# libraz/mygram-db

Hardware: AMD Instinct MI355X
Metric: queries/sec + p50 latency, 10M-doc bigram index, batch=1024 3-term AND (higher is better)
Workload: dtype u32 set algebra + f64 BM25

## Files before the change

mygram-db_amd/csrc/mgx_api.cpp:

```cpp
#include <hip/hip_runtime.h>

#include <dlfcn.h>
#include <pthread.h>

#include <algorithm>
#include <atomic>
#include <chrono>
#include <cmath>
#include <condition_variable>
#include <map>
#include <cstdio>
#include <cstdlib>
#include <cstring>
#include <memory>
#include <mutex>
#include <string>
#include <thread>
#include <tuple>
#include <unordered_map>
#include <vector>

#include "../../include/mygram_gpu.h"
#include "mgx_compile.hpp"
#include "mgx_highlight.hpp"
#include "mgx_host.hpp"
#include "mgx_internal.hpp"
#include "mgx_launch.hpp"
#include "mygram_tools.h"

namespace mgx {

static thread_local std::string g_last_error;
void SetError(const std::string& msg) { g_last_error = msg; }
int Fail(int code, const std::string& msg) {
  g_last_error = msg;
  return code;
}

#define MGX_HIP(expr)                                                                             \
  do {                                                                                            \
    hipError_t e__ = (expr);                                                                      \
    if (e__ != hipSuccess)                                                                        \
      return ::mgx::Fail(MGX_ERR_INTERNAL, std::string(#expr) + ": " + hipGetErrorString(e__));   \
  } while (0)
#define MGX_LAUNCH(expr)                                                                                    \
  do {                                                                                                      \
    int e__ = (expr);                                                                                       \
    if (e__ != 0)                                                                                           \
      return ::mgx::Fail(MGX_ERR_INTERNAL,                                                                  \
                         std::string(#expr) + ": " + hipGetErrorString(static_cast<hipError_t>(e__)));      \
  } while (0)

static std::atomic<int> g_fail_after{-1};
static std::atomic<int> g_fail_count{0};
static hipError_t DeviceMalloc(void** p, size_t n) {
  if (g_fail_after.load(std::memory_order_relaxed) >= 0) {
    if (g_fail_after.load() == 0) {
      if (g_fail_count.fetch_sub(1) > 0) {
        if (g_fail_count.load() <= 0) g_fail_after.store(-1);
        *p = nullptr;
        return hipErrorOutOfMemory;
      }
      g_fail_after.store(-1);
    } else {
      g_fail_after.fetch_sub(1);
    }
  }
  return hipMalloc(p, n);
}

struct Arena {
  struct Chunk {
    char* dev = nullptr;
    char* host = nullptr;
    size_t cap = 0, used = 0;
  };
  std::vector<Chunk> chunks;
  bool mirrored = false;
  size_t chunk_bytes = 4u << 20;
  explicit Arena(bool m) : mirrored(m) {}
  Arena(const Arena&) = delete;
  Arena& operator=(const Arena&) = delete;
  ~Arena() {
    for (Chunk& c : chunks) {
      if (c.dev) (void)hipFree(c.dev);
      if (c.host) (void)hipHostFree(c.host);
    }
  }
  void Reset() {
    for (Chunk& c : chunks) c.used = 0;
  }
  hipError_t Alloc(size_t n, void** dev, void** mirror) {
    n = (std::max<size_t>(n, 16) + 255) & ~static_cast<size_t>(255);
    for (Chunk& c : chunks) {
      if (c.cap - c.used >= n) {
        *dev = c.dev + c.used;
        if (mirror) *mirror = c.host ? c.host + c.used : nullptr;
        c.used += n;
        return hipSuccess;
      }
    }
    Chunk c;
    c.cap = std::max(n, chunk_bytes);
    hipError_t e = DeviceMalloc(reinterpret_cast<void**>(&c.dev), c.cap);
    if (e != hipSuccess) return e;
    if (mirrored) {
      e = hipHostMalloc(reinterpret_cast<void**>(&c.host), c.cap, hipHostMallocDefault);
      if (e != hipSuccess) {
        (void)hipFree(c.dev);
        return e;
      }
    }
    c.used = n;
    *dev = c.dev;
    if (mirror) *mirror = c.host;
    chunks.push_back(c);
    return hipSuccess;
  }
};

struct BatchResources {
  Arena upload{true}, out{false};
  bool uploaded = false;
  void* h_down[3] = {nullptr, nullptr, nullptr};
  size_t h_down_cap[3] = {0, 0, 0};
  hipEvent_t fork_ev = nullptr, join_ev = nullptr;
  hipStream_t stream = nullptr;
  hipEvent_t done_ev = nullptr;
  hipEvent_t main_ev = nullptr;
  bool copy_issued = false;
  void* xchg[4] = {nullptr, nullptr, nullptr, nullptr};
  size_t xchg_cap[4] = {0, 0, 0, 0};
  hipError_t Exchange(int which, size_t bytes, void** out_ptr) {
    if (xchg_cap[which] < bytes) {
      if (xchg[which]) (void)hipFree(xchg[which]);
      xchg[which] = nullptr;
      xchg_cap[which] = 0;
      const size_t cap = bytes + bytes / 4;
      hipError_t e = DeviceMalloc(&xchg[which], cap);
      if (e != hipSuccess) return e;
      xchg_cap[which] = cap;
    }
    *out_ptr = xchg[which];
    return hipSuccess;
  }
  void* cond = nullptr;
  size_t cond_cap = 0;
  hipError_t Conditions(size_t bytes, void** out_ptr) {
    if (cond_cap < bytes) {
      if (cond) (void)hipFree(cond);
      cond = nullptr;
      cond_cap = 0;
      hipError_t e = DeviceMalloc(&cond, bytes);
      if (e != hipSuccess) return e;
      cond_cap = bytes;
    }
    *out_ptr = cond;
    return hipSuccess;
  }
  ~BatchResources() {
    if (cond) (void)hipFree(cond);
    for (void* x : xchg)
      if (x) (void)hipFree(x);
    if (stream) (void)hipStreamDestroy(stream);
    if (done_ev) (void)hipEventDestroy(done_ev);
    if (main_ev) (void)hipEventDestroy(main_ev);
    for (void* h : h_down)
      if (h) (void)hipHostFree(h);
    if (fork_ev) (void)hipEventDestroy(fork_ev);
    if (join_ev) (void)hipEventDestroy(join_ev);
  }
  hipError_t Pinned(int which, size_t bytes, void** out_ptr) {
    if (h_down_cap[which] < bytes) {
      if (h_down[which]) (void)hipHostFree(h_down[which]);
      h_down[which] = nullptr;
      h_down_cap[which] = 0;
      const size_t cap = std::max<size_t>(bytes + bytes / 2, 1u << 16);
      hipError_t e = hipHostMalloc(&h_down[which], cap, hipHostMallocDefault);
      if (e != hipSuccess) return e;
      h_down_cap[which] = cap;
    }
    *out_ptr = h_down[which];
    return hipSuccess;
  }
  void Reset() {
    upload.Reset();
    out.Reset();
    uploaded = false;
    copy_issued = false;
  }
};
static thread_local BatchResources* tl_res = nullptr;
struct ResourceScope {
  BatchResources* prev;
  explicit ResourceScope(BatchResources* r) : prev(tl_res) { tl_res = r; }
  ~ResourceScope() { tl_res = prev; }
};

struct DevBuf {
  void* p = nullptr;
  size_t bytes = 0;
  bool owned = true;
  DevBuf() = default;
  DevBuf(const DevBuf&) = delete;
  DevBuf& operator=(const DevBuf&) = delete;
  DevBuf(DevBuf&& o) noexcept : p(o.p), bytes(o.bytes), owned(o.owned) { o.p = nullptr; o.bytes = 0; }
  DevBuf& operator=(DevBuf&& o) noexcept {
    if (this != &o) {
      Free();
      p = o.p;
      bytes = o.bytes;
      owned = o.owned;
      o.p = nullptr;
      o.bytes = 0;
    }
    return *this;
  }
  ~DevBuf() { Free(); }
  void Free() {
    if (p && owned) (void)hipFree(p);
    p = nullptr;
    bytes = 0;
    owned = true;
  }
  hipError_t Alloc(size_t n) {
    Free();
    bytes = n;
    if (tl_res) {
      owned = false;
      return tl_res->out.Alloc(n, &p, nullptr);
    }
    return DeviceMalloc(&p, n ? n : 16);
  }
  template <typename T>
  T* as() const { return static_cast<T*>(p); }
};

template <typename T>
static hipError_t Upload(DevBuf& b, const T* host, size_t count, size_t pad_count = 0) {
  if (tl_res) {
    b.Free();
    b.bytes = (count + pad_count) * sizeof(T);
    b.owned = false;
    void* mirror = nullptr;
    hipError_t e = tl_res->upload.Alloc(b.bytes, &b.p, &mirror);
    if (e != hipSuccess) return e;
    if (count) std::memcpy(mirror, host, count * sizeof(T));
    if (pad_count) std::memset(static_cast<char*>(mirror) + count * sizeof(T), 0xFF, pad_count * sizeof(T));
    return hipSuccess;
  }
  hipError_t e = b.Alloc((count + pad_count) * sizeof(T));
  if (e != hipSuccess) return e;
  if (pad_count) {
    e = hipMemset(static_cast<char*>(b.p) + count * sizeof(T), 0xFF, pad_count * sizeof(T));
    if (e != hipSuccess) return e;
  }
  if (count) e = hipMemcpy(b.p, host, count * sizeof(T), hipMemcpyHostToDevice);
  return e;
}

}

using mgx::DevBuf;


struct mgx_index {
  int device = 0;
  hipStream_t stream = nullptr;
  hipStream_t side_stream = nullptr;
  std::mutex mu;
  std::mutex pool_mu;
  std::vector<std::unique_ptr<mgx::BatchResources>> single_pool;
  mgx::DevIndex dev{};
  DevBuf d_offsets, d_docids, d_tf, d_doc_len, d_skip_row, d_tile_off, d_gram_bitmaps, d_filter_bitmaps;
  DevBuf d_text, d_text_off;
  uint32_t max_text_bytes = 0;
  DevBuf d_dl8, d_tfnib, d_tf_ovf_pos, d_tf_ovf_val;
  DevBuf d_dev_index;
  std::vector<uint64_t> h_offsets;
  std::vector<uint32_t> h_skip_row;
  std::vector<uint32_t> h_bm_row;
  uint32_t n_filter_rows = 0, filter_cap_rows = 0;
  struct FilterColumn {
    uint32_t value_class = 0, n_values = 0;
    DevBuf d_values, d_null, d_value_ids;
  };
  std::vector<std::unique_ptr<FilterColumn>> filter_columns;
  std::atomic<uint32_t> n_filter_columns{0};
  std::vector<DevBuf> retired_filter_pools;
  uint64_t n_grams = 0;
  bool can_score = false;
  uint64_t words_per_row = 0;
  uint64_t filter_row_stride = 0;
  struct TableKey {
    uint32_t row;
    uint64_t idf, k1, b, avg;
    bool operator==(const TableKey& o) const { return row == o.row && idf == o.idf && k1 == o.k1 && b == o.b && avg == o.avg; }
  };
  struct TableKeyHash {
    size_t operator()(const TableKey& k) const {
      uint64_t h = k.row * 0x9E3779B97F4A7C15ull;
      for (uint64_t v : {k.idf, k.k1, k.b, k.avg}) h = (h ^ v) * 0xFF51AFD7ED558CCDull + (h >> 29);
      return static_cast<size_t>(h);
    }
  };
  std::mutex table_mu;
  std::unordered_map<TableKey, uint32_t, TableKeyHash> table_slot;
  DevBuf d_table_pool;
  uint32_t table_cap = 0, table_used = 0, table_dl = 0;
  hipStream_t table_stream = nullptr;
  hipEvent_t table_ev = nullptr;
  mgx::TableJob* job_ring = nullptr;
  DevBuf d_job_ring;
  uint32_t job_ring_at = 0;
  std::vector<mgx::TableJob> pending_jobs;
  hipEvent_t chain_ev = nullptr;
  std::atomic<int> fifo{1};
  bool table_ev_recorded = false;
  static constexpr uint32_t kJobRing = 4096;
  size_t table_doubles() const { return static_cast<size_t>(mgx::kFastPoolTf + 1) * table_dl; }
  struct NormTable {
    uint64_t k1, b, avg;
    DevBuf d;
  };
  std::vector<std::unique_ptr<NormTable>> norm_tables;
  struct BlockMax {
    uint64_t k1, b, avg;
    double step;
    DevBuf d, d_fine;
  };
  std::vector<std::unique_ptr<BlockMax>> block_max;
  std::unordered_map<std::string, uint64_t> df_cache;
  uint32_t n_bitmap_rows = 0, n_fine_rows = 0;
  std::atomic<uint32_t> live_row{mgx::kNoRow};
  std::atomic<bool> bitmaps_clean{false};
  DevBuf d_doc_map;
  DevBuf d_fine_rows;
// ... 821 lines not shown
  }
}

int mgx_index_invalidate_statistics(mgx_index* idx) {
  if (!idx) return mgx::Fail(MGX_ERR_INVALID_ARGUMENT, "mgx_index_invalidate_statistics: null index");
  MGX_HIP(hipSetDevice(idx->device));
  MGX_HIP(hipDeviceSynchronize());
  std::lock_guard<std::mutex> lock(idx->table_mu);
  idx->table_slot.clear();
  idx->table_used = 0;
  idx->pending_jobs.clear();
  idx->norm_tables.clear();
  idx->block_max.clear();
  idx->df_cache.clear();
  return MGX_OK;
}

int mgx_index_synchronize(mgx_index* idx) {
  if (!idx) return mgx::Fail(MGX_ERR_INVALID_ARGUMENT, "mgx_index_synchronize: null index");
  MGX_HIP(hipSetDevice(idx->device));
  MGX_HIP(hipDeviceSynchronize());
  return MGX_OK;
}

}


struct mgx_batch {
  mgx_index* idx = nullptr;
  std::unique_ptr<mgx::BatchResources> res_owned;
  mgx::BatchResources* res = nullptr;
  uint32_t n_queries = 0;
  std::vector<mgx::QuerySpec> specs;
  struct RouteLaunch {
    mgx::DevBatch dev{};
    DevBuf d_items;
  };
  struct Group {
    std::vector<uint32_t> qids;
    mgx::DevBatch dev{};
    mgx::LdsPlan plan{};
    mgx::WavePlan wplan{};
    RouteLaunch block;
    uint32_t n_items_plain = 0;
    uint32_t n_items_fz = 0;
    RouteLaunch wave;
    DevBuf d_tables;
    mgx::WavePlan wplan_lists{};
    RouteLaunch wave_lists;
    mgx::FastPlan fplan{};
    RouteLaunch fast[mgx::kFastMaxScore];
    uint32_t n_seed_fast[mgx::kFastMaxScore] = {0, 0, 0, 0, 0};
    uint32_t seed_k = 0;
    uint64_t seed_table_docs = 0;
    DevBuf d_has_seed;
    DevBuf d_fast_queries;
    RouteLaunch cand;
    DevBuf d_cand_skip;
    uint32_t cand_leaves = 0, cand_instr = 0, cand_cap = 0;
    RouteLaunch merge;
    uint32_t merge_leaves = 0, merge_instr = 0, merge_ops = 0, merge_cap = 0;
    RouteLaunch page_wave, page_block;
    uint32_t n_page_fz = 0;
    DevBuf d_queries, d_leaves, d_prog, d_score, d_explicit, d_counters, d_ident, d_list_begin;
    std::vector<unsigned long long> h_counters;
  };
  Group score, bitmap;
  Group textdf;
  std::vector<mgx::QuerySpec> df_specs;
  DevBuf d_patterns, d_text_terms, d_text_idf, d_text_df, d_verify_terms, d_verify_prog;
  DevBuf d_text_df_local, d_text_df_known;
  std::vector<uint64_t> h_text_df, h_text_df_local, text_total_docs;
  std::vector<uint64_t> text_df_known;
  std::vector<std::string> text_df_key;
  std::vector<double> h_text_idf;
  DevBuf d_cond_groups, d_conds;
  uint32_t n_cond_groups = 0;
  uint64_t* cond_arena = nullptr;
  bool df_ready = false;
  DevBuf d_cand_keys, d_cand_docs, d_cand_n;
  DevBuf d_export;
  size_t ex_off32 = 0, ex_bytes = 0;
  uint64_t* ex_keys() const { return d_export.as<uint64_t>(); }
  uint64_t* ex_totals(size_t n) const { return d_export.as<uint64_t>() + n * top_stride; }
  uint32_t* ex_docs() const { return reinterpret_cast<uint32_t*>(static_cast<char*>(d_export.p) + ex_off32); }
  uint32_t* ex_counts(size_t n) const { return ex_docs() + n * top_stride; }
  DevBuf d_score_out;
  void* h_score_out = nullptr;
  size_t so_override = 0, so_scores = 0, so_docs = 0, so_n = 0, so_bytes = 0;
  unsigned long long* sc_counters() const { return d_score_out.as<unsigned long long>(); }
  uint64_t* sc_override() const { return reinterpret_cast<uint64_t*>(static_cast<char*>(d_score_out.p) + so_override); }
  double* sc_scores() const { return reinterpret_cast<double*>(static_cast<char*>(d_score_out.p) + so_scores); }
  uint32_t* sc_docs() const { return reinterpret_cast<uint32_t*>(static_cast<char*>(d_score_out.p) + so_docs); }
  uint32_t* sc_n() const { return reinterpret_cast<uint32_t*>(static_cast<char*>(d_score_out.p) + so_n); }
  uint32_t top_stride = 0, page_stride = 0;
  bool merged_shards = false;
  DevBuf d_rbits, d_tile_cnt, d_tile_start, d_totals, d_take, d_out_off, d_reverse;
  mgx_batch* merge_other = nullptr;
  bool merged_away = false;
  hipStream_t merge_stream = nullptr;
  DevBuf d_merge;
  Group page;
  DevBuf d_ptile_cnt, d_ptile_start, d_page_out, d_page_scratch;
  void* h_page_out = nullptr;
  size_t po_totals = 0, po_docs = 0, po_bytes = 0;
  uint32_t doc_page_stride = 0;
  struct Highlight {
    std::vector<mgx::DevHlQuery> queries;
    std::vector<int32_t> of_query;
    DevBuf d_queries, d_terms, d_patterns, d_arena;
    void* h_arena = nullptr;
    size_t bytes = 0;
    uint32_t n_entries = 0;
    bool defer = false;
    std::vector<mgx_highlight_entry> entries;
    bool on() const { return !queries.empty(); }
  };
  Highlight hl;
  bool fetched = false;
  std::vector<mgx_query_result> h_results;
  std::vector<uint32_t> h_docs;
  std::vector<double> h_scores;
  bool executed = false;
  hipStream_t last_stream = nullptr;
  bool timing = false;
  std::vector<std::pair<hipEvent_t, hipEvent_t>> events;
  uint64_t list_bytes = 0;
};

namespace mgx {

constexpr int kSections = 7;
static std::atomic<uint64_t> g_section_us[kSections];
static const char* const kSectionNames[kSections] = {"queries+leaves", "routes", "table uploads", "result blocks",
                                                      "items", "launch order", "descriptors+items"};
struct SectionTimer {
  static bool On() {
    static const bool on = std::getenv("MGX_TRACE_HOST") != nullptr;
    return on;
  }
  std::chrono::steady_clock::time_point t;
  SectionTimer() { if (On()) t = std::chrono::steady_clock::now(); }
  void Mark(int section) {
    if (!On()) return;
    const auto now = std::chrono::steady_clock::now();
    g_section_us[section] += std::chrono::duration_cast<std::chrono::nanoseconds>(now - t).count();
    t = now;
  }
};

using Group = mgx_batch::Group;
using RouteLaunch = mgx_batch::RouteLaunch;

enum class Route : uint8_t {
  kBlock,
  kWave,
  kWaveLists,
  kFast,
  kCand,
  kMerge,
};

static bool EnvZero(const char* name) { return std::getenv(name) && atoi(std::getenv(name)) == 0; }
struct PathSwitches {
  const bool wave = std::getenv("MGX_FORCE_BLOCK_KERNEL") == nullptr;
  const bool fast = wave && !EnvZero("MGX_FAST_PATH"), cand = wave && !EnvZero("MGX_CAND");
  const bool merge = wave && !EnvZero("MGX_MERGE");
};

struct GroupPlan {
  GroupPlan(uint32_t n_, uint32_t mode)
      : n(n_), score_mode(mode == kModeScore), df_mode(mode == kModeTextDf), page_mode(mode == kModeDocPage) {}
  const uint32_t n;
  const bool score_mode, df_mode, page_mode;
  std::vector<DevQuery> dq;
  std::vector<DevLeaf> leaves;
  std::vector<uint32_t> prog;
  std::vector<DevScoreTerm> score;
  std::vector<uint32_t> expl;
  uint32_t max_limit = 1, max_needed = 1;
  std::vector<Route> route;
  std::vector<DevFastQuery> fastq;
  std::vector<uint64_t> wave_tables;
  std::vector<uint32_t> cand_driver;
  std::vector<DevItem> items;
  std::vector<uint32_t> list_begin, item_begin;
  std::vector<DevItem> block, wave, wave_lists, fast[kFastMaxScore], cand, merge;
  std::vector<uint8_t> has_seed;
};

static int LayOutQueries(mgx_batch* b, Group& g, const std::vector<QuerySpec>& specs, GroupPlan& p) {
  std::vector<DevLeaf>& leaves = p.leaves;
  std::vector<uint32_t>& expl = p.expl;
  p.dq.resize(p.n);
  uint32_t max_leaves = 0, max_lds_leaves = 0, max_score = 0, max_stack = 0, max_instr = 0, max_cap = 64;
  for (uint32_t i = 0; i < p.n; ++i) {
    const QuerySpec& s = specs[g.qids[i]];
    DevQuery& q = p.dq[i];
    std::memset(&q, 0, sizeof(q));
    q.leaf_begin = static_cast<uint32_t>(leaves.size());
    q.n_leaves = static_cast<uint32_t>(s.leaves.size());
    q.prog_begin = static_cast<uint32_t>(p.prog.size());
    q.n_instr = static_cast<uint32_t>(s.prog.size());
    q.score_begin = static_cast<uint32_t>(p.score.size());
    q.n_score = static_cast<uint32_t>(s.score.size());
    q.mode = s.mode;
    q.limit = s.limit;
    q.offset = s.offset;
    q.needed = static_cast<uint32_t>(std::min<uint64_t>(static_cast<uint64_t>(s.offset) + s.limit, 0xFFFFFFFFull));
    uint32_t cap = 64;
    if (s.mode == kModeScore)
      while (cap < q.needed && cap < (1u << 30)) cap <<= 1;
    q.cap = cap;
    q.descending = s.reverse;
    q.stack_depth = s.stack_depth;
    q.out_slot = i;
    q.pat_off = s.pat_off;
    q.pat_len = s.pat_len;
    q.vt_begin = s.vt_begin;
    q.vt_count = static_cast<uint32_t>(s.verify_patterns.size());
    q.fz_distance = s.fz_distance;
    q.vp_begin = s.vp_begin;
    q.k1 = s.k1;
    q.b = s.b;
    q.one_minus_b = 1.0 - s.b;
    q.k1_plus_1 = s.k1 + 1.0;
    q.avgdl_clamped = std::max(s.avgdl, 1.0);
    const uint32_t ebase = static_cast<uint32_t>(expl.size());
    uint32_t n_lds = 0;
    for (size_t li = 0; li < s.leaves.size(); ++li) {
      DevLeaf lf = s.leaves[li];
      if (lf.kind == kLeafExplicit) lf.a += ebase;
      bool resident = lf.kind == kLeafList || lf.kind == kLeafExplicit;
      for (const DevScoreTerm& st : s.score) resident = resident || st.leaf == li;
      lf.lds = resident ? n_lds++ : kNoRow;
      leaves.push_back(lf);
    }
    if (n_lds > kMaxLdsLeaves)
      return Fail(MGX_ERR_NOT_IMPLEMENTED,
                  "query " + std::to_string(g.qids[i]) + ": more than 64 sorted-list / scored operands in one query");
    max_lds_leaves = std::max(max_lds_leaves, n_lds);
    p.prog.insert(p.prog.end(), s.prog.begin(), s.prog.end());
    p.score.insert(p.score.end(), s.score.begin(), s.score.end());
    expl.insert(expl.end(), s.explicit_ids.begin(), s.explicit_ids.end());
    while (expl.size() % 4) expl.push_back(0xFFFFFFFFu);
    max_leaves = std::max(max_leaves, q.n_leaves);
    max_score = std::max(max_score, q.n_score);
    max_stack = std::max(max_stack, q.stack_depth);
    max_instr = std::max(max_instr, q.n_instr);
    max_cap = std::max(max_cap, q.cap);
    p.max_limit = std::max(p.max_limit, q.limit);
    p.max_needed = std::max(p.max_needed, q.needed);
    if (!p.df_mode) b->list_bytes += 4 * s.list_postings;
  }
  g.plan = PlanLds(max_leaves, max_lds_leaves, max_score, max_stack, max_instr, max_cap, p.score_mode || p.df_mode);
  return MGX_OK;
}

static bool ResolveFast(mgx_index* idx, const uint64_t* cond_arena, const QuerySpec& s, const DevQuery& q, DevFastQuery* out) {
  DevFastQuery& f = *out;
  for (uint32_t ins : s.prog) {
    const uint32_t op = ins >> 24, arg = ins & 0xFFFFFFu;
    if (op == kOpCount) {
      if (f.n_ops == 0) return false;
      f.ops[f.n_ops - 1].code |= arg << 8;
      continue;
    }
    const DevLeaf& lf = s.leaves[arg];
    if (f.n_ops == static_cast<uint32_t>(kFastMaxOps) || (op == kOpLoad) != (f.n_ops == 0)) return false;
    FastOp o{};
    uint64_t stride = 0;
    if (lf.kind == kLeafGramBitmap) {
      o.base = reinterpret_cast<uint64_t>(idx->dev.gram_bitmaps + static_cast<uint64_t>(lf.b) * idx->dev.gb_row_stride);
      stride = idx->dev.gb_tile_stride * 8;
    } else if (lf.kind == kLeafFilterBitmap) {
      o.base = static_cast<uint64_t>(lf.b) * idx->dev.fb_row_stride * 8;
      stride = idx->dev.fb_tile_stride * 8;
      o.code |= 16u;
    } else if (lf.kind == kLeafCondBitmap) {
      o.base = reinterpret_cast<uint64_t>(cond_arena + static_cast<uint64_t>(lf.b) * idx->dev.fb_row_stride);
      stride = idx->dev.fb_tile_stride * 8;
    } else {
      return false;
    }
    if (stride > 0xFFFFFFFFull) return false;
    o.tile_stride = static_cast<uint32_t>(stride);
    o.code |= (op == kOpLoad || op == kOpOr) ? kFastOr : op == kOpAnd ? kFastAnd : kFastAndNot;
    f.ops[f.n_ops++] = o;
  }
  if (f.n_ops == 0) return false;
  for (size_t t = 0; t < s.score.size(); ++t) {
    const DevLeaf& lf = s.leaves[s.score[t].leaf];
    if (lf.kind != kLeafGramBitmap) return false;
    FastScore& fs = f.score[t];
    fs.nib = reinterpret_cast<uint64_t>(idx->dev.tfnib + static_cast<uint64_t>(lf.b) * idx->dev.nib_row_stride);
    fs.idf = s.score[t].idf;
    fs.gram = lf.a;
    fs.skip_row = lf.row;
  }
  if (s.reverse != 0) {
    double step = 0.0;
    f.blockmax = GetBlockMax(idx, s.k1, s.b, s.avgdl, &step, &f.blockmax_fine);
    if (f.blockmax) {
      f.bm_tile_stride = idx->n_bitmap_rows * 256u;
      f.bmf_tile_stride = idx->n_fine_rows * 1024u;
      double idf_max = 0.0;
      for (size_t t = 0; t < s.score.size(); ++t) idf_max = std::max(idf_max, s.score[t].idf);
      const double wunit = idf_max > 0.0 ? idf_max * (1.0 + 0x1p-40) / 255.0 : 1.0;
      f.bm_inv_unit = 1.0 / (wunit * step);
      f.bm_wpack = f.bm_w4 = f.bm_cint = 0;
      for (size_t t = 0; t < s.score.size(); ++t) {
        const uint32_t w = static_cast<uint32_t>(std::min(255.0, std::ceil(s.score[t].idf / wunit)));
        if (t < 4) f.bm_wpack |= w << (8 * t); else f.bm_w4 = w;
      }
      for (size_t t = 0; t < s.score.size(); ++t) {
        const DevLeaf& lf = s.leaves[s.score[t].leaf];
        FastScore& fs = f.score[t];
        const uint32_t frow = f.blockmax_fine ? idx->h_fine_map[lf.b] : kNoRow;
        fs.bm_mode = frow != kNoRow ? 2u : 1u;
        fs.bm_off = frow != kNoRow ? frow * 1024u : lf.b * 256u;
      }
    }
  }
  f.n_score = static_cast<uint32_t>(s.score.size());
  f.needed = q.needed;
  f.cap = q.cap;
  f.descending = q.descending;
  f.k1 = q.k1;
  f.b = q.b;
  f.one_minus_b = q.one_minus_b;
  f.k1_plus_1 = q.k1_plus_1;
  f.avgdl_clamped = q.avgdl_clamped;
  return true;
}

static void RouteCandMerge(mgx_batch* b, Group& g, const std::vector<QuerySpec>& specs, const PathSwitches& sw,
                           GroupPlan& p) {
  static const uint64_t kMaxPerTile = std::getenv("MGX_CAND_MAX_PER_TILE") ? static_cast<uint64_t>(atoll(std::getenv("MGX_CAND_MAX_PER_TILE"))) : 64ull;
  const mgx_index* idx = b->idx;
  for (uint32_t i = 0; sw.cand && i < p.n; ++i) {
    const QuerySpec& s = specs[g.qids[i]];
    if (p.route[i] == Route::kFast || !s.flat || s.prog.empty()) continue;
    if (p.score_mode && (!s.fast_score_ok || s.score.empty())) continue;
    bool ok = true, counted = false;
    uint32_t driver = kNoLeaf;
    uint64_t best = ~0ull, longest_list = 0;
    for (size_t pc = 0; ok && pc < s.prog.size(); ++pc) {
      const uint32_t op = s.prog[pc] >> 24, arg = s.prog[pc] & 0xFFFFFFu;
      if (op == kOpCount) {
        counted = true;
        continue;
      }
      if ((op == kOpLoad) != (pc == 0) || (op != kOpLoad && op != kOpAnd && op != kOpAndNot)) { ok = false; break; }
      const DevLeaf& lf = s.leaves[arg];
      if (lf.kind != kLeafList && lf.kind != kLeafGramBitmap && !IsFilterKind(lf.kind)) { ok = false; break; }
      if (lf.kind == kLeafList) longest_list = std::max<uint64_t>(longest_list, idx->h_offsets[lf.a + 1] - idx->h_offsets[lf.a]);
      if (op == kOpAndNot || IsFilterKind(lf.kind) || counted) continue;
      const uint64_t sz = idx->h_offsets[lf.a + 1] - idx->h_offsets[lf.a];
      if (sz < best) {
        best = sz;
        driver = arg;
      }
    }
    if (!ok || driver == kNoLeaf || s.leaves[driver].kind != kLeafList) continue;
    for (uint32_t ins : s.prog)
      if ((ins >> 24) == kOpAndNot && (ins & 0xFFFFFFu) == driver) ok = false;
    if (p.score_mode)
      for (const DevScoreTerm& st : s.score)
        ok = ok && st.leaf != kNoLeaf && (s.leaves[st.leaf].kind == kLeafList || s.leaves[st.leaf].kind == kLeafGramBitmap);
    if (!ok) continue;
    DevQuery& q = p.dq[i];
    const bool long_probe = longest_list > 8 * kMaxPerTile * idx->dev.n_tiles;
    if (best > kMaxPerTile * idx->dev.n_tiles || long_probe) {
      uint32_t staged = 0;
      for (size_t li = 0; li < s.leaves.size(); ++li) staged += li != driver ? 1u : 0u;
      if (!p.score_mode || !sw.merge || staged > kMergeMaxOps || q.cap > 256) continue;
      q.pat_off = driver;
      p.route[i] = Route::kMerge;
      g.merge_leaves = std::max(g.merge_leaves, q.n_leaves);
      g.merge_instr = std::max(g.merge_instr, q.n_instr);
      g.merge_ops = std::max(g.merge_ops, staged);
      g.merge_cap = std::max(g.merge_cap, q.cap);
      continue;
    }
    if (p.cand_driver.empty()) p.cand_driver.assign(p.n, kNoLeaf);
    p.cand_driver[i] = driver;
    p.route[i] = Route::kCand;
    g.cand_leaves = std::max(g.cand_leaves, q.n_leaves);
    g.cand_instr = std::max(g.cand_instr, q.n_instr);
    g.cand_cap = std::max(g.cand_cap, q.cap);
  }
  if (CandLdsBytes(g.cand_leaves, g.cand_instr, p.score_mode ? g.cand_cap : 0) > 150 * 1024) {
    for (Route& r : p.route)
      if (r == Route::kCand) r = Route::kBlock;
    p.cand_driver.clear();
  }
  if (MergeLdsBytes(g.merge_leaves, g.merge_instr, g.merge_ops, g.merge_cap) > 150 * 1024)
    for (Route& r : p.route)
      if (r == Route::kMerge) r = Route::kBlock;
}

static int ChooseRoutes(mgx_batch* b, Group& g, const std::vector<QuerySpec>& specs, const PathSwitches& sw,
                        GroupPlan& p) {
  mgx_index* idx = b->idx;
  p.route.assign(p.n, Route::kBlock);
  if (p.score_mode) {
    uint32_t fcap = 64;
    bool have_params = false;
    double pk1 = 0, pb = 0, pavg = 0;
    for (uint32_t i = 0; sw.fast && i < p.n; ++i) {
      const QuerySpec& s = specs[g.qids[i]];
      if (!s.flat || !s.fast_score_ok || s.score.empty() || s.score.size() > static_cast<size_t>(kFastMaxScore)) continue;
      if (p.dq[i].cap > 128) continue;
      if (have_params && (Bits(s.k1) != Bits(pk1) || Bits(s.b) != Bits(pb) || Bits(s.avgdl) != Bits(pavg))) continue;
      DevFastQuery f{};
      if (!ResolveFast(idx, b->cond_arena, s, p.dq[i], &f)) continue;
      if (!have_params) {
        pk1 = s.k1;
        pb = s.b;
        pavg = s.avgdl;
        have_params = true;
      }
      if (p.fastq.empty()) p.fastq.resize(p.n);
      p.fastq[i] = f;
      p.route[i] = Route::kFast;
      fcap = std::max(fcap, f.cap);
    }
    if (have_params) {
      const double* ktab = GetLengthNormTable(idx, pk1, pb, pavg);
      g.fplan = PlanFast(fcap, ktab);
      if (ktab == nullptr || g.fplan.bytes > 64 * 1024)
        for (Route& r : p.route) r = Route::kBlock;
    }

    uint32_t wl = 0, wsc = 0, wi = 0, wc = 64;
    for (uint32_t i = 0; i < p.n; ++i) {
      if (p.route[i] == Route::kFast) continue;
      const QuerySpec& s = specs[g.qids[i]];
      bool ok = sw.wave && s.wave_ok;
      for (const DevScoreTerm& st : s.score)
        ok = ok && (s.leaves[st.leaf].kind == kLeafGramBitmap || s.leaves[st.leaf].kind == kLeafList);
      if (!ok) continue;
      uint64_t tabs[kWaveScoreSlots] = {0, 0, 0};
      for (size_t t = 0; ok && t < s.score.size(); ++t) {
        const DevLeaf& lf = s.leaves[s.score[t].leaf];
        const uint32_t key = lf.kind == kLeafGramBitmap ? lf.b : 0x80000000u | lf.a;
        tabs[t] = GetContributionTable(idx, key, s.score[t].idf, s.k1, s.b, s.avgdl);
        ok = tabs[t] != 0;
      }
      if (!ok) continue;
      if (p.wave_tables.empty()) p.wave_tables.assign(static_cast<size_t>(p.n) * kWaveScoreSlots, 0);
      for (int t = 0; t < kWaveScoreSlots; ++t) p.wave_tables[static_cast<size_t>(i) * kWaveScoreSlots + t] = tabs[t];
      bool lists = false;
      for (const DevLeaf& lf : s.leaves) lists = lists || lf.kind == kLeafList || lf.kind == kLeafExplicit;
      p.route[i] = lists ? Route::kWaveLists : Route::kWave;
      wl = std::max<uint32_t>(wl, p.dq[i].n_leaves);
      wsc = std::max<uint32_t>(wsc, p.dq[i].n_score);
      wi = std::max<uint32_t>(wi, p.dq[i].n_instr);
      wc = std::max<uint32_t>(wc, p.dq[i].cap);
    }
    g.wplan = PlanWave(wl, wsc, wi, wc, idx->dev.max_doc_len, false);
    g.wplan_lists = PlanWave(wl, wsc, wi, wc, idx->dev.max_doc_len, true);
    if (g.wplan_lists.bytes > 160 * 1024)
      for (Route& r : p.route)
        if (r != Route::kFast) r = Route::kBlock;
  }
  if (p.page_mode || p.df_mode) {
    uint32_t wl = 1, wi = 1;
    bool has_list = false;
    for (uint32_t i = 0; i < p.n; ++i) {
      const QuerySpec& s = specs[g.qids[i]];
      if (!(sw.wave && s.wave_ok)) continue;
      p.route[i] = Route::kWave;
      for (const DevLeaf& lf : s.leaves) has_list = has_list || lf.kind == kLeafList || lf.kind == kLeafExplicit;
      wl = std::max<uint32_t>(wl, p.dq[i].n_leaves);
      wi = std::max<uint32_t>(wi, p.dq[i].n_instr);
    }
    g.wplan = WavePlan{wl, 0, wi, 0, 0, has_list ? 1u : 0u, 0};
  }
  g.cand_leaves = g.cand_instr = g.cand_cap = 0;
  g.merge_leaves = g.merge_instr = g.merge_ops = g.merge_cap = 0;
  if (p.score_mode || p.page_mode) RouteCandMerge(b, g, specs, sw, p);
  if (g.plan.bytes > 160 * 1024)
    return Fail(MGX_ERR_NOT_IMPLEMENTED, "query shape exceeds the 160 KiB LDS of a CU");
  for (uint32_t i = 0; i < p.n; ++i)
    if (specs[g.qids[i]].fz_op && g.plan.bytes + kFzLdsBytes > 160 * 1024)
      return Fail(MGX_ERR_NOT_IMPLEMENTED, "query shape with the fuzzy text filter exceeds the 160 KiB LDS of a CU");
  return MGX_OK;
}

static int UploadTables(mgx_batch* b, Group& g, const GroupPlan& p, SectionTimer& sec) {
  const uint32_t n = p.n;
  MGX_HIP(Upload(g.d_queries, p.dq.data(), p.dq.size()));
  MGX_HIP(Upload(g.d_leaves, p.leaves.data(), p.leaves.size()));
  MGX_HIP(Upload(g.d_prog, p.prog.data(), p.prog.size()));
  MGX_HIP(Upload(g.d_score, p.score.data(), p.score.size()));
  MGX_HIP(Upload(g.d_explicit, p.expl.data(), p.expl.size(), 4));
  sec.Mark(2);
  if (p.score_mode) {
    const size_t max_limit = p.max_limit;
    b->so_override = static_cast<size_t>(n) * 9 * 8;
    b->so_scores = b->so_override + static_cast<size_t>(n) * 8;
    b->so_docs = b->so_scores + static_cast<size_t>(n) * max_limit * 8;
    b->so_n = b->so_docs + static_cast<size_t>(n) * max_limit * 4;
    b->so_bytes = b->so_n + static_cast<size_t>(n) * 4;
    MGX_HIP(b->d_score_out.Alloc(b->so_bytes));
    MGX_HIP(b->res->Pinned(0, b->so_bytes, &b->h_score_out));
  } else if (p.page_mode) {
    const size_t max_limit = p.max_limit;
    b->doc_page_stride = p.max_limit;
    b->po_totals = static_cast<size_t>(n) * 8 * 8;
    b->po_docs = b->po_totals + static_cast<size_t>(n) * 8;
    b->po_bytes = b->po_docs + static_cast<size_t>(n) * max_limit * 4;
    MGX_HIP(b->d_page_out.Alloc(b->po_bytes));
    MGX_HIP(b->res->Pinned(1, b->po_bytes, &b->h_page_out));
    const size_t tiles = b->idx->dev.n_tiles;
    MGX_HIP(b->d_ptile_cnt.Alloc(static_cast<size_t>(n) * tiles * 4));
    MGX_HIP(b->d_ptile_start.Alloc(static_cast<size_t>(n) * tiles * 8));
  } else {
    MGX_HIP(g.d_counters.Alloc(static_cast<size_t>(n) * 9 * sizeof(unsigned long long)));
  }
  g.h_counters.assign(static_cast<size_t>(n) * 8, 0);
  std::vector<uint32_t> ident(n);
  for (uint32_t i = 0; i < n; ++i) ident[i] = i;
  MGX_HIP(Upload(g.d_ident, ident.data(), n));
  return MGX_OK;
}

static void CutItems(const mgx_batch* b, const Group& g, const std::vector<QuerySpec>& specs, GroupPlan& p) {
  static const double kMatchesPerUnit = std::getenv("MGX_ITEM_MATCHES") ? atof(std::getenv("MGX_ITEM_MATCHES")) : 256.0;
  static const double kItemCost = std::getenv("MGX_ITEM_COST") ? atof(std::getenv("MGX_ITEM_COST")) : 192.0;
  static const uint32_t kMaxTiles = std::getenv("MGX_MAX_ITEM_TILES") ? static_cast<uint32_t>(atoi(std::getenv("MGX_MAX_ITEM_TILES"))) : static_cast<uint32_t>(kMaxTilesPerItem);
  static const uint64_t want_items = std::getenv("MGX_WANT_ITEMS") ? static_cast<uint64_t>(atoll(std::getenv("MGX_WANT_ITEMS"))) : 4ull * 768ull;
  static const uint32_t kSeedTiles = std::getenv("MGX_SEED_TILES") ? static_cast<uint32_t>(atoi(std::getenv("MGX_SEED_TILES"))) : 16u;
  const uint32_t n = p.n, n_tiles = b->idx->dev.n_tiles;
  p.list_begin.assign(n + 1, 0);
  p.item_begin.assign(n + 1, 0);
  uint32_t n_lists = 0;
  for (uint32_t i = 0; i < n; ++i) {
    const QuerySpec& s = specs[g.qids[i]];
    const Route route = p.route[i];
    p.item_begin[i] = static_cast<uint32_t>(p.items.size());
    const bool fast = route == Route::kFast;
    const double per_tile = 1.0 + (p.score_mode || p.df_mode ? s.est_density * kTileDocs / (fast ? kMatchesPerUnit / 2 : kMatchesPerUnit) : 0.0);
    const double fast_scale = std::min(4.0, std::max(2.0, static_cast<double>(n_tiles) / 150.0));
    uint32_t tiles = static_cast<uint32_t>((fast ? fast_scale * kItemCost : kItemCost) / per_tile);
    tiles = std::max<uint32_t>(8, std::min<uint32_t>(tiles, fast ? 2 * kMaxTiles : kMaxTiles)) & ~7u;
    if (p.score_mode) {
      const uint64_t cap = std::max<uint64_t>(8, (static_cast<uint64_t>(n_tiles) * n / want_items + 7) & ~7ull);
      tiles = static_cast<uint32_t>(std::min<uint64_t>(tiles, cap));
    }
    if (p.score_mode && route == Route::kBlock) tiles = 8;
    p.list_begin[i] = n_lists;
    if (route == Route::kCand) {
      p.items.push_back(DevItem{i, p.cand_driver[i], 0, n_lists++});
      continue;
    }
    uint32_t t0 = 0;
    const uint32_t seed_tiles = std::min<uint32_t>(kSeedTiles, (n_tiles / 8) & ~7u);
    if (fast && seed_tiles && n_tiles > 4 * seed_tiles) {
      p.items.push_back(DevItem{i, 0, seed_tiles, n_lists++});
      t0 = seed_tiles;
    }
    for (uint32_t t = t0; t < n_tiles; t += tiles) {
      DevItem it{i, t, std::min(tiles, n_tiles - t), n_lists++};
      p.items.push_back(it);
    }
  }
  p.list_begin[n] = n_lists;
  p.item_begin[n] = static_cast<uint32_t>(p.items.size());
}

static int ScheduleItems(const mgx_batch* b, Group& g, const std::vector<QuerySpec>& specs, GroupPlan& p) {
  static const uint32_t kSortTiles = std::getenv("MGX_SORT_TILES") ? static_cast<uint32_t>(atoi(std::getenv("MGX_SORT_TILES"))) : 16u;
  static const bool kXcdAffinity = std::getenv("MGX_XCD_AFFINITY") ? atoi(std::getenv("MGX_XCD_AFFINITY")) != 0 : true;
  static const double kHeavyDensity = std::getenv("MGX_HEAVY_DENSITY") ? atof(std::getenv("MGX_HEAVY_DENSITY")) : 0.05;
  static const double kSqueezeEnv = std::getenv("MGX_HEAVY_SQUEEZE") ? atof(std::getenv("MGX_HEAVY_SQUEEZE")) : -1.0;
  const uint32_t n = p.n, n_tiles = b->idx->dev.n_tiles;
  const bool deal = kXcdAffinity && p.score_mode;
  std::vector<uint32_t> order(n);
  for (uint32_t i = 0; i < n; ++i) order[i] = i;
  if (deal) {
    std::vector<uint32_t> heavy(n, 0);
    for (uint32_t i = 0; i < n; ++i) {
      uint64_t best = 0;
      for (const DevLeaf& lf : specs[g.qids[i]].leaves) {
        if (lf.kind != kLeafGramBitmap && lf.kind != kLeafList) continue;
        const uint64_t sz = b->idx->h_offsets[lf.a + 1] - b->idx->h_offsets[lf.a];
        if (sz > best) {
          best = sz;
          heavy[i] = lf.a;
        }
      }
    }
    std::stable_sort(order.begin(), order.end(), [&](uint32_t x, uint32_t y) { return heavy[x] < heavy[y]; });
  }
  const uint32_t n_bands = n_tiles / kSortTiles + 1;
  const double kHeavySqueeze = kSqueezeEnv >= 0.0 ? kSqueezeEnv : 0.6 + 0.4 * std::min(1.0, n_tiles / 600.0);
  auto band_of = [&](const DevItem& it) {
    const Route route = p.route[it.query];
    if (route == Route::kCand) return 0u;
    const uint32_t band = it.tile_begin / kSortTiles;
    if (p.score_mode && route == Route::kFast && specs[g.qids[it.query]].est_density >= kHeavyDensity)
      return static_cast<uint32_t>(band * kHeavySqueeze);
    return band;
  };
  std::vector<uint32_t> band_at(n_bands + 1, 0);
  for (const DevItem& it : p.items) band_at[band_of(it) + 1]++;
  for (uint32_t k = 0; k < n_bands; ++k) band_at[k + 1] += band_at[k];
  std::vector<DevItem> sorted(p.items.size());
  {
    std::vector<uint32_t> cur(band_at.begin(), band_at.end() - 1);
    for (uint32_t oi = 0; oi < n; ++oi) {
      const uint32_t i = order[oi];
      for (uint32_t k = p.item_begin[i]; k < p.item_begin[i + 1]; ++k) sorted[cur[band_of(p.items[k])]++] = p.items[k];
    }
  }
  if (deal) {
    for (uint32_t k = 0; k < n_bands; ++k) {
      const size_t lo = band_at[k], m = band_at[k + 1] - lo, per = (m + 7) / 8;
      size_t w = lo;
      for (size_t r = 0; r < per; ++r)
        for (size_t x = 0; x < 8; ++x)
          if (x * per + r < m) p.items[w++] = sorted[lo + x * per + r];
    }
  } else {
    p.items.swap(sorted);
  }
  p.has_seed.assign(n, 0);
  for (int pass = 0; pass < 2; ++pass) {
    for (const DevItem& it : p.items) {
      const Route route = p.route[it.query];
      const bool seed = route == Route::kFast && it.list == p.list_begin[it.query] && it.tile_begin == 0 &&
                        p.list_begin[it.query + 1] - p.list_begin[it.query] > 1 && it.n_tiles <= 16;
      if (seed != (pass == 0)) continue;
      switch (route) {
        case Route::kBlock: p.block.push_back(it); break;
        case Route::kWave: p.wave.push_back(it); break;
        case Route::kWaveLists: p.wave_lists.push_back(it); break;
        case Route::kFast: p.fast[p.fastq[it.query].n_score - 1].push_back(it); break;
        case Route::kCand: p.cand.push_back(it); break;
        case Route::kMerge: p.merge.push_back(it); break;
      }
      if (seed && p.fastq[it.query].blockmax != 0) p.has_seed[it.query] = 1;
    }
    if (pass == 0)
      for (int t = 0; t < kFastMaxScore; ++t) g.n_seed_fast[t] = static_cast<uint32_t>(p.fast[t].size());
  }
  g.seed_k = 0;
  g.seed_table_docs = 0;
  for (uint32_t i = 0; p.score_mode && i < n; ++i) {
    const QuerySpec& sp = specs[g.qids[i]];
    if (sp.reverse != 0 && p.dq[i].needed != 0 && p.dq[i].needed <= 128u) {
      g.seed_k = std::max(g.seed_k, p.dq[i].needed);
      g.seed_table_docs = std::max<uint64_t>(g.seed_table_docs, sp.total_docs);
    }
  }
  if (g.seed_k) MGX_HIP(Upload(g.d_has_seed, p.has_seed.data(), p.has_seed.size()));
  return MGX_OK;
}

static hipError_t MakeRoute(RouteLaunch& r, const DevBatch& base, const std::vector<DevItem>& items) {
  r.dev = base;
  r.dev.n_items = static_cast<uint32_t>(items.size());
  const hipError_t e = Upload(r.d_items, items.data(), items.size());
  r.dev.items = r.d_items.as<DevItem>();
  return e;
}

static int UploadItems(mgx_batch* b, Group& g, const std::vector<QuerySpec>& specs, GroupPlan& p) {
  const uint32_t n = p.n;
  std::vector<uint8_t> listlike(n, 0);
  for (uint32_t i = 0; i < n; ++i) {
    for (const DevLeaf& lf : specs[g.qids[i]].leaves)
      if (lf.kind == kLeafList || lf.kind == kLeafExplicit || lf.kind == kLeafRange) listlike[i] = 1;
    if (specs[g.qids[i]].fz_op) listlike[i] = 2;
  }
  std::stable_partition(p.block.begin(), p.block.end(), [&](const DevItem& it) { return listlike[it.query] == 0; });
  if (std::find(listlike.begin(), listlike.end(), 2) != listlike.end())
    std::stable_partition(p.block.begin(), p.block.end(), [&](const DevItem& it) { return listlike[it.query] != 2; });
  g.n_items_plain = g.n_items_fz = 0;
  for (const DevItem& it : p.block) {
    g.n_items_plain += listlike[it.query] == 0 ? 1u : 0u;
    g.n_items_fz += listlike[it.query] == 2 ? 1u : 0u;
  }
  DevBatch& d = g.dev;
  d.queries = g.d_queries.as<DevQuery>();
  d.leaves = g.d_leaves.as<DevLeaf>();
  d.prog = g.d_prog.as<uint32_t>();
  d.score_terms = g.d_score.as<DevScoreTerm>();
  d.explicit_pool = g.d_explicit.as<uint32_t>();
  d.patterns = b->d_patterns.as<uint8_t>();
  d.text_terms = b->d_text_terms.as<DevTextTerm>();
  d.text_idf = b->d_text_idf.as<double>();
  d.verify_terms = b->d_verify_terms.as<DevTextTerm>();
  d.verify_prog = b->d_verify_prog.as<uint32_t>();
  d.n_queries = n;
  d.counters = p.score_mode  ? b->sc_counters()
               : p.page_mode ? b->d_page_out.as<unsigned long long>()
                             : g.d_counters.as<unsigned long long>();
  if (p.page_mode) {
    d.tile_cnt = b->d_ptile_cnt.as<uint32_t>();
    d.tile_start = b->d_ptile_start.as<uint64_t>();
    d.totals = reinterpret_cast<const uint64_t*>(static_cast<const char*>(b->d_page_out.p) + b->po_totals);
    d.page_docs = reinterpret_cast<uint32_t*>(static_cast<char*>(b->d_page_out.p) + b->po_docs);
    d.page_stride = b->doc_page_stride;
  }
  d.bounds = p.score_mode ? d.counters + static_cast<size_t>(n) * 8 : nullptr;
#ifdef MGX_ABLATION
  d.debug_skip = std::getenv("MGX_DEBUG_SKIP") ? static_cast<uint32_t>(atoi(std::getenv("MGX_DEBUG_SKIP"))) : 0u;
#endif
  if (p.score_mode) {
    const size_t n_lists = p.list_begin[n], max_needed = p.max_needed;
    d.cand_stride = b->top_stride = p.max_needed;
    b->page_stride = p.max_limit;
    MGX_HIP(b->d_cand_keys.Alloc(n_lists * max_needed * 8));
    MGX_HIP(b->d_cand_docs.Alloc(n_lists * max_needed * 4));
    MGX_HIP(b->d_cand_n.Alloc(n_lists * 4));
    {
      const size_t elems = static_cast<size_t>(n) * max_needed + n;
      b->ex_off32 = elems * 8;
      b->ex_bytes = (elems * 12 + 7) / 8 * 8;
      MGX_HIP(b->d_export.Alloc(b->ex_bytes));
    }
    d.cand_keys = b->d_cand_keys.as<uint64_t>();
    d.cand_docs = b->d_cand_docs.as<uint32_t>();
    d.cand_n = b->d_cand_n.as<uint32_t>();
  } else if (!p.df_mode && !p.page_mode) {
    const size_t tiles = b->idx->dev.n_tiles;
    MGX_HIP(b->d_rbits.Alloc(static_cast<size_t>(n) * tiles * kWordsPerTile * 8));
    MGX_HIP(b->d_tile_cnt.Alloc(static_cast<size_t>(n) * tiles * 4));
    MGX_HIP(b->d_tile_start.Alloc(static_cast<size_t>(n) * tiles * 8));
    MGX_HIP(b->d_totals.Alloc(static_cast<size_t>(n) * 8));
    MGX_HIP(b->d_take.Alloc(static_cast<size_t>(n) * 8));
    MGX_HIP(b->d_out_off.Alloc(static_cast<size_t>(n) * 8));
    std::vector<uint32_t> rev(n);
    for (uint32_t i = 0; i < n; ++i) rev[i] = specs[g.qids[i]].deep_score ? 0u : specs[g.qids[i]].reverse;
    MGX_HIP(Upload(b->d_reverse, rev.data(), n));
    d.rbits = b->d_rbits.as<uint64_t>();
    d.tile_cnt = b->d_tile_cnt.as<uint32_t>();
  }
  if (p.score_mode && !p.wave_tables.empty()) {
    MGX_HIP(Upload(g.d_tables, p.wave_tables.data(), p.wave_tables.size()));
    d.wave_tables = g.d_tables.as<uint64_t>();
  }
  if (!p.fastq.empty()) MGX_HIP(Upload(g.d_fast_queries, p.fastq.data(), p.fastq.size()));
  d.fast_queries = g.d_fast_queries.as<DevFastQuery>();
  d.dev_index = b->idx->d_dev_index.as<DevIndex>();
  d.cond_bitmaps = b->cond_arena;
  for (int t = 0; t < kFastMaxScore; ++t) MGX_HIP(MakeRoute(g.fast[t], d, p.fast[t]));
  MGX_HIP(MakeRoute(g.wave_lists, d, p.wave_lists));
  MGX_HIP(MakeRoute(g.cand, d, p.cand));
  MGX_HIP(MakeRoute(g.merge, d, p.merge));
  if (p.page_mode && !p.cand.empty()) {
    std::vector<uint8_t> skip(n, 0);
    for (uint32_t i = 0; i < n; ++i) skip[i] = p.route[i] == Route::kCand ? 1 : 0;
    MGX_HIP(Upload(g.d_cand_skip, skip.data(), skip.size()));
  }
  MGX_HIP(MakeRoute(g.block, d, p.block));
  MGX_HIP(MakeRoute(g.wave, d, p.wave));
  MGX_HIP(Upload(g.d_list_begin, p.list_begin.data(), p.list_begin.size()));
  if (p.page_mode) {
    std::vector<DevItem> pw, pb;
    for (uint32_t i = 0; i < n; ++i)
      if (p.route[i] != Route::kCand && !specs[g.qids[i]].fz_op)
        (p.route[i] == Route::kWave ? pw : pb).push_back(DevItem{i, 0, 0, 0});
    g.n_page_fz = 0;
    for (uint32_t i = 0; i < n; ++i)
      if (specs[g.qids[i]].fz_op) {
        pb.push_back(DevItem{i, 0, 0, 0});
        ++g.n_page_fz;
      }
    MGX_HIP(MakeRoute(g.page_wave, d, pw));
    MGX_HIP(MakeRoute(g.page_block, d, pb));
  }
  return MGX_OK;
}

static int UploadGroup(mgx_batch* b, Group& g, uint32_t mode, const std::vector<QuerySpec>& specs) {
  GroupPlan p(static_cast<uint32_t>(g.qids.size()), mode);
  if (p.n == 0) return MGX_OK;
  const PathSwitches sw;
  SectionTimer sec;
  if (const int rc = LayOutQueries(b, g, specs, p)) return rc;
  sec.Mark(0);
  if (const int rc = ChooseRoutes(b, g, specs, sw, p)) return rc;
  sec.Mark(1);
  if (const int rc = UploadTables(b, g, p, sec)) return rc;
  sec.Mark(3);
  CutItems(b, g, specs, p);
  sec.Mark(4);
  if (const int rc = ScheduleItems(b, g, specs, p)) return rc;
  sec.Mark(5);
  if (const int rc = UploadItems(b, g, specs, p)) return rc;
  sec.Mark(6);
  if (std::getenv("MGX_VERBOSE")) {
    size_t fast_queries = 0;
    for (Route r : p.route) fast_queries += r == Route::kFast ? 1 : 0;
    fprintf(stderr,
            "[mgx] %s group: %u queries; fast path %zu items (%zu queries, lds %u B, ring %u), wave kernel %zu items "
            "(lds %u B, lists %zu), block kernel %zu items (lds %u B), candidate-driven %zu queries, list merge %zu "
            "items\n",
            p.score_mode ? "score" : p.page_mode ? "docid-page" : p.df_mode ? "df" : "bitmap", p.n,
            p.fast[0].size() + p.fast[1].size() + p.fast[2].size() + p.fast[3].size() + p.fast[4].size(), fast_queries,
            g.fplan.bytes, g.fplan.ring, p.wave.size() + p.wave_lists.size(), g.wplan.bytes, p.wave_lists.size(),
            p.block.size(), g.plan.bytes, p.cand.size(), p.merge.size());
  }
  return MGX_OK;
}

static CompileView ViewOf(const mgx_index* idx) {
  CompileView v;
  v.offsets = idx->h_offsets.data();
  v.skip_row = idx->h_skip_row.data();
  v.bm_row = idx->h_bm_row.data();
  v.n_grams = idx->n_grams;
  v.n_docs = idx->dev.n_docs;
  v.first_doc_id = idx->dev.first_doc_id;
  v.has_text = idx->dev.text != nullptr;
  v.can_score = idx->can_score;
  v.n_filter_rows = idx->n_filter_rows;
  v.n_filter_columns = idx->n_filter_columns.load(std::memory_order_acquire);
  v.live_row = idx->live_row.load(std::memory_order_relaxed);
  v.bitmaps_clean = idx->bitmaps_clean.load(std::memory_order_relaxed);
  return v;
}

static int CompileRange(const CompileView& view, const mgx_query* queries, std::vector<QuerySpec>* specs, uint32_t a, uint32_t b) {
  for (uint32_t i = a; i < b; ++i) {
    (*specs)[i].Clear();
    if (const int rc = CompileQuery(view, queries[i], &(*specs)[i])) return Fail(rc, "query " + std::to_string(i) + ": " + g_last_error);
  }
  return MGX_OK;
}

struct CompilePool {
  std::mutex mu, gate;
  std::condition_variable cv_work, cv_done;
  std::vector<std::thread> helpers;
  const CompileView* view = nullptr;
  const mgx_query* queries = nullptr;
  std::vector<QuerySpec>* specs = nullptr;
  uint32_t next = 0, end = 0, pending = 0;
  int rc = MGX_OK;
  std::string error;
  bool stop = false;
  static constexpr uint32_t kChunk = 64;

  void Run(std::unique_lock<std::mutex>& lock) {
    while (next < end) {
      const uint32_t a = next, b = std::min(end, a + kChunk);
      next = b;
      lock.unlock();
      const int local = CompileRange(*view, queries, specs, a, b);
      lock.lock();
      if (local && rc == MGX_OK) {
        rc = local;
        error = g_last_error;
      }
      pending -= b - a;
    }
  }
  void Helper() {
    std::unique_lock<std::mutex> lock(mu);
    for (;;) {
      cv_work.wait(lock, [&] { return stop || next < end; });
      if (stop) return;
      Run(lock);
      if (pending == 0) cv_done.notify_all();
    }
  }
  CompilePool() {
    const int n = std::getenv("MGX_COMPILE_THREADS") ? atoi(std::getenv("MGX_COMPILE_THREADS")) : 3;
    for (int i = 0; i < n; ++i)
      helpers.emplace_back([this] {
        pthread_setname_np(pthread_self(), "mgx-compile");
        Helper();
      });
  }
  ~CompilePool() {
    {
      std::lock_guard<std::mutex> lock(mu);
      stop = true;
    }
    cv_work.notify_all();
    for (auto& t : helpers) t.join();
  }
};

static int CompileAll(const mgx_index* idx, const mgx_query* queries, uint32_t n, std::vector<QuerySpec>* specs) {
  static thread_local CompilePool pool;
  const CompileView view = ViewOf(idx);
  std::unique_lock<std::mutex> gate(pool.gate, std::try_to_lock);
  if (n < 4 * CompilePool::kChunk || pool.helpers.empty() || !gate.owns_lock()) return CompileRange(view, queries, specs, 0, n);
  std::unique_lock<std::mutex> lock(pool.mu);
  pool.view = &view;
  pool.queries = queries;
  pool.specs = specs;
  pool.next = 0;
  pool.end = pool.pending = n;
  pool.rc = MGX_OK;
  pool.cv_work.notify_all();
  pool.Run(lock);
  pool.cv_done.wait(lock, [&] { return pool.pending == 0; });
  pool.end = 0;
  if (pool.rc) SetError(pool.error);
  return pool.rc;
}

static int LayOutConditions(mgx_batch* b) {
  mgx_index* idx = b->idx;
  size_t n_refs = 0;
  for (const QuerySpec& s : b->specs) n_refs += s.conds.size();
  if (n_refs == 0) return MGX_OK;
  using Key = std::tuple<uint32_t, uint32_t, uint64_t, uint64_t, uint32_t, uint32_t>;
  std::map<Key, uint32_t> rows;
  for (QuerySpec& s : b->specs)
    for (DevLeaf& lf : s.leaves) {
      if (lf.kind != kLeafCondBitmap) continue;
      const mgx_condition& c = s.conds[lf.a];
      const Key key{c.column_id, c.op, c.literal_bits, Bits(c.eq_epsilon), c.null_matches ? 1u : 0u, c.never_matches ? 1u : 0u};
      lf.b = rows.emplace(key, static_cast<uint32_t>(rows.size())).first->second;
      lf.a = 0;
    }
  const uint64_t row_bytes = idx->dev.fb_row_stride * sizeof(uint64_t);
  if (idx->dev.fb_row_stride % kCondBlockWords != 0)
    return Fail(MGX_ERR_INTERNAL, "filter row stride is not a multiple of the condition pass's block");
  if (rows.size() * row_bytes > MGX_CONDITION_ARENA_MAX_BYTES)
    return Fail(MGX_ERR_OUT_OF_RANGE, "the batch holds " + std::to_string(rows.size()) + " distinct conditions of " +
                                          std::to_string(row_bytes) + " bytes each: more than the " +
                                          std::to_string(MGX_CONDITION_ARENA_MAX_BYTES) +
                                          " bytes (MGX_CONDITION_ARENA_MAX_BYTES) a batch's condition arena may take");
  void* arena = nullptr;
  MGX_HIP(b->res->Conditions(rows.size() * row_bytes, &arena));
  b->cond_arena = static_cast<uint64_t*>(arena);
  std::vector<DevCondition> conds;
  std::vector<DevCondGroup> groups;
  conds.reserve(rows.size());
  {
    std::lock_guard<std::mutex> lock(idx->mu);
    uint32_t last_column = 0;
    for (const auto& kv : rows) {
      const uint32_t column = std::get<0>(kv.first);
      if (groups.empty() || column != last_column) {
        last_column = column;
        const mgx_index::FilterColumn& col = *idx->filter_columns[column];
        DevCondGroup g{};
        g.values = col.d_values.as<uint64_t>();
        g.is_null = col.d_null.as<uint8_t>();
        g.value_class = col.value_class;
        g.cond_begin = g.cond_end = static_cast<uint32_t>(conds.size());
        groups.push_back(g);
      }
      DevCondition d{};
      d.literal = std::get<2>(kv.first);
      __builtin_memcpy(&d.eq_epsilon, &std::get<3>(kv.first), 8);
      d.op = std::get<1>(kv.first);
      d.null_matches = std::get<4>(kv.first);
      d.never_matches = std::get<5>(kv.first);
      d.row = kv.second;
      conds.push_back(d);
      groups.back().cond_end = static_cast<uint32_t>(conds.size());
    }
  }
  if (groups.size() > 65535) return Fail(MGX_ERR_OUT_OF_RANGE, "conditions on more than 65535 columns in one batch");
  MGX_HIP(Upload(b->d_conds, conds.data(), conds.size()));
  MGX_HIP(Upload(b->d_cond_groups, groups.data(), groups.size()));
  b->n_cond_groups = static_cast<uint32_t>(groups.size());
  return MGX_OK;
}

static int NumberTextTerms(mgx_batch* b, std::string* pool, std::vector<DevTextTerm>* tts) {
  mgx_index* idx = b->idx;
  const CompileView view = ViewOf(idx);
  std::map<std::pair<std::string, uint64_t>, uint32_t> seen;
  for (QuerySpec& s : b->specs) {
    for (const QuerySpec::TextTerm& tt : s.text_terms) {
      const auto ins = seen.emplace(std::make_pair(tt.pattern, s.total_docs), static_cast<uint32_t>(tts->size()));
      const uint32_t id = ins.first->second;
      if (s.deep_score) s.deep_grams[tt.score_index] = kDeepText | id;
      else s.score[tt.score_index].text_term = id;
      if (!ins.second) continue;
      const DevTextTerm d{static_cast<uint32_t>(pool->size()), static_cast<uint32_t>(tt.pattern.size())};
      *pool += tt.pattern;
      tts->push_back(d);
      b->text_total_docs.push_back(s.total_docs);
      std::string ckey = tt.pattern + '\0' + std::to_string(s.total_docs);
      uint64_t known = ~0ull;
      {
        std::lock_guard<std::mutex> lock(idx->table_mu);
        const auto hit = idx->df_cache.find(ckey);
        if (hit != idx->df_cache.end()) known = hit->second;
      }
      b->text_df_known.push_back(tt.grams.empty() ? 0ull : known);
      b->text_df_key.push_back(std::move(ckey));
      QuerySpec ds;
      if (const int rc = CompileTextDf(view, tt.grams, tt.grams.empty() || known != ~0ull, d.pat_off, d.pat_len, &ds)) return rc;
      b->df_specs.push_back(std::move(ds));
    }
  }
  return MGX_OK;
}

static void PoolVerifyPatterns(mgx_batch* b, std::string* pool, std::vector<DevTextTerm>* vts, std::vector<uint32_t>* vprog) {
  for (QuerySpec& s : b->specs) {
    s.vt_begin = static_cast<uint32_t>(vts->size());
    s.vp_begin = static_cast<uint32_t>(vprog->size());
    vprog->insert(vprog->end(), s.verify_prog.begin(), s.verify_prog.end());
    for (const std::string& pat : s.verify_patterns) {
      vts->push_back(DevTextTerm{static_cast<uint32_t>(pool->size()), static_cast<uint32_t>(pat.size())});
      *pool += pat;
    }
  }
}

static int PrepareInto(mgx_batch* b, mgx_index* idx, std::vector<QuerySpec>&& specs) {
  ResourceScope scope(b->res);
  b->idx = idx;
  b->n_queries = static_cast<uint32_t>(specs.size());
  b->specs = std::move(specs);
  for (uint32_t i = 0; i < b->n_queries; ++i) {
    const uint32_t m = b->specs[i].mode;
    (m == kModeScore ? b->score : m == kModeDocPage ? b->page : b->bitmap).qids.push_back(i);
  }
  MGX_HIP(hipSetDevice(idx->device));
  if (const int rc = LayOutConditions(b)) return rc;
  std::string pool;
  std::vector<DevTextTerm> tts, vts;
  std::vector<uint32_t> vprog;
  if (const int rc = NumberTextTerms(b, &pool, &tts)) return rc;
  PoolVerifyPatterns(b, &pool, &vts, &vprog);
  if (!vprog.empty()) MGX_HIP(Upload(b->d_verify_prog, vprog.data(), vprog.size()));
  if (!vts.empty()) MGX_HIP(Upload(b->d_verify_terms, vts.data(), vts.size()));
  if (!pool.empty()) MGX_HIP(Upload(b->d_patterns, reinterpret_cast<const uint8_t*>(pool.data()), pool.size(), 16));
  const uint32_t n_tt = static_cast<uint32_t>(tts.size());
  if (n_tt != 0) {
    MGX_HIP(Upload(b->d_text_terms, tts.data(), tts.size()));
    MGX_HIP(b->d_text_idf.Alloc(static_cast<size_t>(n_tt) * sizeof(double)));
    MGX_HIP(b->d_text_df.Alloc(static_cast<size_t>(n_tt) * sizeof(uint64_t)));
    MGX_HIP(b->d_text_df_local.Alloc(static_cast<size_t>(n_tt) * sizeof(uint64_t)));
    MGX_HIP(Upload(b->d_text_df_known, b->text_df_known.data(), b->text_df_known.size()));
    b->h_text_df.assign(n_tt, 0);
    b->h_text_df_local.assign(n_tt, 0);
    b->h_text_idf.assign(n_tt, 0.0);
    for (uint32_t i = 0; i < n_tt; ++i) b->textdf.qids.push_back(i);
  }
  int rc = UploadGroup(b, b->score, kModeScore, b->specs);
  if (rc) return rc;
  rc = UploadGroup(b, b->bitmap, kModeBitmap, b->specs);
  if (rc) return rc;
  rc = UploadGroup(b, b->textdf, kModeTextDf, b->df_specs);
  if (rc) return rc;
  rc = UploadGroup(b, b->page, kModeDocPage, b->specs);
  if (rc) return rc;
  b->h_results.assign(b->n_queries, mgx_query_result{});
  return MGX_OK;
}

static int PrepareFromSpecs(mgx_index* idx, std::vector<QuerySpec>&& specs, mgx_batch** out) {
  auto b = std::make_unique<mgx_batch>();
  b->res_owned = std::make_unique<BatchResources>();
  b->res = b->res_owned.get();
  int rc = PrepareInto(b.get(), idx, std::move(specs));
  if (rc) return rc;
  *out = b.release();
  return MGX_OK;
}

static void ResetBatch(mgx_batch* b) {
  std::unique_ptr<BatchResources> owned = std::move(b->res_owned);
  BatchResources* res = b->res;
  for (auto& ev : b->events) {
    (void)hipEventDestroy(ev.first);
    (void)hipEventDestroy(ev.second);
  }
  const bool timing = b->timing;
  b->~mgx_batch();
  new (b) mgx_batch();
  b->res_owned = std::move(owned);
  b->res = res;
  b->timing = timing;
  if (res) res->Reset();
}

static int IssueResultCopy(mgx_batch* b, hipStream_t s) {
  if (!b->res) return MGX_OK;
  if (!b->page.qids.empty())
    MGX_HIP(hipMemcpyAsync(b->h_page_out, b->d_page_out.p, b->po_bytes, hipMemcpyDeviceToHost, s));
  if (!b->score.qids.empty())
    MGX_HIP(hipMemcpyAsync(b->h_score_out, b->d_score_out.p, b->so_bytes, hipMemcpyDeviceToHost, s));
  if (!b->res->done_ev) {
    MGX_HIP(hipEventCreateWithFlags(&b->res->done_ev, hipEventDisableTiming));
  }
  MGX_HIP(hipEventRecord(b->res->done_ev, s));
  b->res->copy_issued = true;
  return MGX_OK;
}

static int BatchStream(mgx_batch* b, void* hip_stream, hipStream_t* out) {
  (void)b;
  *out = static_cast<hipStream_t>(hip_stream);
  return MGX_OK;
}

static int EnsureUploaded(mgx_batch* b, hipStream_t s) {
  if (!b->res || b->res->uploaded) return MGX_OK;
  for (const Arena::Chunk& c : b->res->upload.chunks)
    if (c.used) MGX_HIP(hipMemcpyAsync(c.dev, c.host, c.used, hipMemcpyHostToDevice, s));
  b->res->uploaded = true;
  return MGX_OK;
}

static int CountDfImpl(mgx_batch* b, hipStream_t s) {
  mgx_index* idx = b->idx;
  mgx_batch::Group& g = b->textdf;
  if (g.qids.empty()) return MGX_OK;
  MGX_HIP(hipSetDevice(idx->device));
  {
    int rc = EnsureUploaded(b, s);
    if (rc) return rc;
  }
  MGX_HIP(hipMemsetAsync(g.d_counters.p, 0, g.d_counters.bytes, s));
  MGX_LAUNCH(LaunchWaveCount(idx->dev, g.wave.dev, g.wplan, true, s));
  MGX_LAUNCH(LaunchTileEval(kModeTextDf, idx->dev, g.block.dev, g.plan, s, g.n_items_plain));
  MGX_LAUNCH(LaunchGatherDf(g.d_counters.as<unsigned long long>(), b->d_text_df_known.as<uint64_t>(),
                            static_cast<uint32_t>(g.qids.size()), b->d_text_df_local.as<uint64_t>(),
                            b->d_text_df.as<uint64_t>(), s));
  return MGX_OK;
}

struct SeedGather {
  int world = 1;
  mgx_gather_fn fn = nullptr;
  void* user = nullptr;
};
static int SeedBoundExchange(mgx_batch* b, mgx_batch::Group& g, const SeedGather& sg, hipStream_t s);

static int ForkSide(mgx_batch* b, hipStream_t s) {
  if (!b->res->fork_ev) {
    MGX_HIP(hipEventCreateWithFlags(&b->res->fork_ev, hipEventDisableTiming));
    MGX_HIP(hipEventCreateWithFlags(&b->res->join_ev, hipEventDisableTiming));
  }
  MGX_HIP(hipEventRecord(b->res->fork_ev, s));
  MGX_HIP(hipStreamWaitEvent(b->idx->side_stream, b->res->fork_ev, 0));
  return MGX_OK;
}

static int RunHighlight(mgx_batch* b, hipStream_t s, bool merged, const mgx_index* mapped, const mgx_index* plain) {
  mgx_batch::Highlight& h = b->hl;
  DevHlBatch hb{};
  hb.queries = h.d_queries.as<DevHlQuery>();
  hb.n_queries = static_cast<uint32_t>(h.queries.size());
  hb.n_entries = h.n_entries;
  hb.terms = h.d_terms.as<DevHlTerm>();
  hb.patterns = h.d_patterns.as<uint8_t>();
  hb.arena = h.d_arena.as<uint8_t>();
  auto source = [](const mgx_index* ix, bool with_map) {
    DevHlSource src{};
    if (!ix) return src;
    src.text = ix->dev.text;
    src.text_off = ix->dev.text_off;
    src.doc_map = with_map ? ix->d_doc_map.as<uint32_t>() : nullptr;
    src.first_doc_id = ix->dev.first_doc_id;
    src.n_docs = ix->dev.n_docs;
    return src;
  };
  hb.mapped = source(mapped, true);
  hb.plain = source(plain, false);
  hb.merged = merged ? 1u : 0u;
  MGX_LAUNCH(LaunchHighlight(hb, s));
  MGX_HIP(hipMemcpyAsync(h.h_arena, h.d_arena.p, h.bytes, hipMemcpyDeviceToHost, s));
  return MGX_OK;
}

static int ExecuteImpl(mgx_batch* b, hipStream_t s, const SeedGather* sg = nullptr) {
  mgx_index* idx = b->idx;
  MGX_HIP(hipSetDevice(idx->device));
  {
    int rc = EnsureUploaded(b, s);
    if (rc) return rc;
  }
  MGX_LAUNCH(LaunchFilterCompareBatch(b->d_cond_groups.as<DevCondGroup>(), b->n_cond_groups, b->d_conds.as<DevCondition>(),
                                      idx->dev.n_docs, idx->dev.fb_row_stride, b->cond_arena, s));
  b->merged_shards = false;
  b->merge_other = nullptr;
  b->merged_away = false;
  {
    std::lock_guard<std::mutex> lock(idx->table_mu);
    MGX_HIP(FlushTableJobs(idx));
    if (idx->table_ev_recorded) MGX_HIP(hipStreamWaitEvent(s, idx->table_ev, 0));
  }
  hipEvent_t ev0 = nullptr, ev1 = nullptr;
  if (b->timing) {
    MGX_HIP(hipEventCreate(&ev0));
    MGX_HIP(hipEventCreate(&ev1));
  }
  bool timed = false;
  if (!b->textdf.qids.empty()) {
    if (!b->df_ready) {
      int rc = CountDfImpl(b, s);
      if (rc) return rc;
    }
    b->df_ready = false;
    const size_t n_tt = b->h_text_df.size();
    MGX_HIP(hipMemcpyAsync(b->h_text_df.data(), b->d_text_df.p, n_tt * sizeof(uint64_t), hipMemcpyDeviceToHost, s));
    MGX_HIP(hipMemcpyAsync(b->h_text_df_local.data(), b->d_text_df_local.p, n_tt * sizeof(uint64_t),
                           hipMemcpyDeviceToHost, s));
    MGX_HIP(hipStreamSynchronize(s));
    {
      std::lock_guard<std::mutex> lock(idx->table_mu);
      for (size_t i = 0; i < n_tt; ++i)
        if (b->text_df_known[i] == ~0ull && idx->df_cache.size() < (1u << 20))
          idx->df_cache.emplace(b->text_df_key[i], b->h_text_df_local[i]);
    }
    for (size_t i = 0; i < n_tt; ++i) {
      const uint64_t total = b->text_total_docs[i];
      const uint64_t dfc = std::min<uint64_t>(b->h_text_df[i], total);
      const double nn = static_cast<double>(total), df = static_cast<double>(dfc);
      b->h_text_idf[i] = total == 0 ? 0.0 : std::log((nn - df + 0.5) / (df + 0.5) + 1.0);
    }
    MGX_HIP(hipMemcpyAsync(b->d_text_idf.p, b->h_text_idf.data(), n_tt * sizeof(double), hipMemcpyHostToDevice, s));
  }
  if (!b->score.qids.empty()) {
    mgx_batch::Group& g = b->score;
    size_t clear_bytes = b->so_override;
#ifdef MGX_ABLATION
    if (std::getenv("MGX_KEEP_BOUNDS")) clear_bytes = b->score.qids.size() * 8 * 8;
#endif
    MGX_HIP(hipMemsetAsync(b->d_score_out.p, 0, clear_bytes, s));
    if (b->timing) {
      MGX_HIP(hipEventRecord(ev0, s));
    }
    static const bool kChainEnv = !(std::getenv("MGX_CHAIN") && atoi(std::getenv("MGX_CHAIN")) == 0);
    const bool kChain = kChainEnv && idx->fifo.load(std::memory_order_relaxed) != 0;
    if (kChain && b->res_owned) {
      if (!b->res->main_ev) MGX_HIP(hipEventCreateWithFlags(&b->res->main_ev, hipEventDisableTiming));
      std::lock_guard<std::mutex> lock(idx->table_mu);
      if (idx->chain_ev && idx->chain_ev != b->res->main_ev) MGX_HIP(hipStreamWaitEvent(s, idx->chain_ev, 0));
    }
    uint32_t n_fast = 0;
    for (int t = 0; t < kFastMaxScore; ++t) n_fast += g.fast[t].dev.n_items;
    const bool main_work = n_fast != 0 || g.wave.dev.n_items != 0 || g.merge.dev.n_items != 0;
    const bool side_work = g.block.dev.n_items != 0 || g.wave_lists.dev.n_items != 0 || g.cand.dev.n_items != 0;
    hipStream_t side = s;
    if (main_work && side_work) {
      if (const int rc = ForkSide(b, s)) return rc;
      side = idx->side_stream;
// ... 151 lines not shown
  m->page_off.resize(n);
  m->page_n.resize(n);
  std::vector<uint64_t> take[2], off[2], soff[2], koff[2], n2[2], toff[2];
  for (int k = 0; k < 2; ++k) {
    take[k].assign(n, 0);
    off[k].assign(n, 0);
    soff[k].assign(n, 0);
    koff[k].assign(n, 0);
    n2[k].assign(n, 0);
    toff[k].assign(n, 0);
  }
  std::vector<DevMergeRun> runs(n);
  std::vector<uint64_t> run_start(n + 1);
  std::vector<uint32_t> terms;
  std::vector<double> idfs;
  uint64_t at[2] = {0, 0}, n_scores = 0, n_keys = 0, pages = 0, elems = 0;
  for (size_t i = 0; i < n; ++i) {
    const QuerySpec& sp = a->specs[g.qids[i]];
    const uint64_t t = a->merged_away ? 0 : tot[0][i] + tot[1][i];
    uint64_t lo = 0, hi = 0;
    if (sp.deep_score) {
      lo = std::min<uint64_t>(sp.offset, t);
      hi = sp.limit == 0 ? t : std::min<uint64_t>(lo + sp.limit, t);
    } else {
      hi = sp.limit == 0 ? t : std::min<uint64_t>(t, sp.limit);
    }
    m->total[i] = n_side == 2 ? t : g.h_counters[i * 8 + 4];
    m->page_off[i] = pages;
    m->page_n[i] = hi - lo;
    pages += hi - lo;
    DevMergeRun& r = runs[i];
    r.kind = sp.deep_score ? kMergeScore : sp.reverse ? kMergeDocDesc : kMergeDocAsc;
    r.descending = sp.reverse ? 1u : 0u;
    r.lo = static_cast<uint32_t>(lo);
    r.hi = static_cast<uint32_t>(hi);
    r.out_off = m->page_off[i];
    for (int k = 0; k < n_side; ++k) {
      take[k][i] = hi == lo ? 0 : sp.deep_score ? tot[k][i] : std::min<uint64_t>(tot[k][i], hi);
      off[k][i] = at[k];
      at[k] += take[k][i];
      if (sp.deep_score && take[k][i] != 0) {
        const QuerySpec& ks = side[k]->specs[g.qids[i]];
        soff[k][i] = n_scores;
        n_scores += take[k][i];
        n2[k][i] = 2048;
        while (n2[k][i] < take[k][i]) n2[k][i] <<= 1;
        koff[k][i] = n_keys;
        n_keys += n2[k][i];
        toff[k][i] = terms.size();
        const std::vector<double> ki = DeepIdfs(side[k], ks);
        terms.insert(terms.end(), ks.deep_grams.begin(), ks.deep_grams.end());
        idfs.insert(idfs.end(), ki.begin(), ki.end());
      }
    }
    r.a_n = static_cast<uint32_t>(take[0][i]);
    r.b_n = static_cast<uint32_t>(take[1][i]);
    run_start[i] = elems;
    elems += take[0][i] + take[1][i];
  }
  run_start[n] = elems;
  if (elems == 0) return MGX_OK;
  if (elems > 0xFFFFFFFFull || pages > 0xFFFFFFFFull || n_keys > 0xFFFFFFFFull)
    return Fail(MGX_ERR_OUT_OF_RANGE, "batch result exceeds 2^32 doc ids");
  for (size_t i = 0; i < n; ++i) {
    DevMergeRun& r = runs[i];
    r.a_off = r.kind == kMergeScore ? koff[0][i] : off[0][i];
    r.b_off = r.kind == kMergeScore ? koff[1][i] : at[0] + off[1][i];
  }
  const uint64_t o_start = Align8(n * sizeof(DevMergeRun));
  const uint64_t o_terms = o_start + (n + 1) * 8;
  const uint64_t o_idfs = Align8(o_terms + terms.size() * 4);
  const uint64_t up_bytes = o_idfs + idfs.size() * 8;
  const uint64_t o_docs = Align8(up_bytes);
  const uint64_t o_scores = Align8(o_docs + (at[0] + at[1]) * 4);
  const uint64_t o_keys = o_scores + n_scores * 8;
  const uint64_t o_dprime = o_keys + n_keys * 8;
  const uint64_t o_pdocs = Align8(o_dprime + n_keys * 4);
  const uint64_t o_pscores = Align8(o_pdocs + pages * 4);
  const uint64_t bytes = o_pscores + pages * 8;
  if (a->d_merge.bytes < bytes) MGX_HIP(a->d_merge.Alloc(bytes));
  char* base = static_cast<char*>(a->d_merge.p);
  std::vector<char> up(up_bytes);
  std::memcpy(up.data(), runs.data(), n * sizeof(DevMergeRun));
  std::memcpy(up.data() + o_start, run_start.data(), (n + 1) * 8);
  if (!terms.empty()) std::memcpy(up.data() + o_terms, terms.data(), terms.size() * 4);
  if (!idfs.empty()) std::memcpy(up.data() + o_idfs, idfs.data(), idfs.size() * 8);
  MGX_HIP(hipMemcpyAsync(base, up.data(), up_bytes, hipMemcpyHostToDevice, s));
  uint32_t* docs = reinterpret_cast<uint32_t*>(base + o_docs);
  double* scores = reinterpret_cast<double*>(base + o_scores);
  uint64_t* keys = reinterpret_cast<uint64_t*>(base + o_keys);
  uint32_t* dprime = reinterpret_cast<uint32_t*>(base + o_dprime);
  uint32_t* pdocs = reinterpret_cast<uint32_t*>(base + o_pdocs);
  double* pscores = reinterpret_cast<double*>(base + o_pscores);
  std::vector<uint64_t> out_off[2];
  for (int k = 0; k < n_side; ++k) {
    mgx_batch* x = side[k];
    out_off[k] = off[k];
    if (k == 1)
      for (uint64_t& o : out_off[k]) o += at[0];
    MGX_HIP(hipMemcpyAsync(x->d_take.p, take[k].data(), n * 8, hipMemcpyHostToDevice, s));
    MGX_HIP(hipMemcpyAsync(x->d_out_off.p, out_off[k].data(), n * 8, hipMemcpyHostToDevice, s));
    if (at[k])
      MGX_LAUNCH(LaunchExpand(x->bitmap.dev.rbits, x->d_tile_start.as<uint64_t>(), x->d_totals.as<uint64_t>(),
                              x->d_take.as<uint64_t>(), x->d_out_off.as<uint64_t>(), x->d_reverse.as<uint32_t>(),
                              static_cast<uint32_t>(n), x->idx->dev.n_tiles, x->idx->dev.first_doc_id, docs, s));
  }
  const uint32_t* d_terms = reinterpret_cast<const uint32_t*>(base + o_terms);
  const double* d_idfs = reinterpret_cast<const double*>(base + o_idfs);
  for (size_t i = 0; i < n; ++i)
    for (int k = 0; k < n_side; ++k) {
      if (n2[k][i] == 0) continue;
      mgx_batch* x = side[k];
      const QuerySpec& ks = x->specs[g.qids[i]];
      MGX_LAUNCH(LaunchScoreCandidatesMixed(x->idx->dev, docs + out_off[k][i], take[k][i], d_terms + toff[k][i],
                                            d_idfs + toff[k][i], static_cast<uint32_t>(ks.deep_grams.size()),
                                            x->d_patterns.as<uint8_t>(), x->d_text_terms.as<DevTextTerm>(), ks.k1,
                                            ks.b, ks.avgdl, scores + soff[k][i], s));
    }
  if (n_side == 2)
    for (int k = 0; k < 2; ++k) {
      const mgx_index* ix = side[k]->idx;
      if (ix->d_doc_map.p && at[k])
        MGX_LAUNCH(LaunchRemapDocs(docs + (k == 0 ? 0 : at[0]), at[k], ix->d_doc_map.as<uint32_t>(), ix->dev.first_doc_id,
                                   ix->dev.n_docs, s));
    }
  for (size_t i = 0; i < n; ++i)
    for (int k = 0; k < n_side; ++k) {
      if (n2[k][i] == 0) continue;
      const int rc = SortRun(docs + out_off[k][i], scores + soff[k][i], take[k][i], n2[k][i], runs[i].descending,
                             keys + koff[k][i], dprime + koff[k][i], s);
      if (rc) return rc;
    }
  MGX_LAUNCH(LaunchRankMerge(reinterpret_cast<const DevMergeRun*>(base), reinterpret_cast<const uint64_t*>(base + o_start),
                             static_cast<uint32_t>(n), elems, docs, keys, dprime, pdocs, pscores, s));
  m->docs.resize(pages);
  if (pages) MGX_HIP(hipMemcpyAsync(m->docs.data(), pdocs, pages * 4, hipMemcpyDeviceToHost, s));
  if (pages && n_keys) {
    m->scores.resize(pages);
    MGX_HIP(hipMemcpyAsync(m->scores.data(), pscores, pages * 8, hipMemcpyDeviceToHost, s));
  }
  MGX_HIP(hipStreamSynchronize(s));
  return MGX_OK;
}

static int FetchImpl(mgx_batch* b, mgx_result_view* out) {
  mgx_index* idx = b->idx;
  MGX_HIP(hipSetDevice(idx->device));
  hipStream_t s = b->last_stream;
  const uint32_t* page_n = nullptr;
  const uint32_t* page_docs = nullptr;
  const double* page_scores = nullptr;
  const unsigned long long* override_tot = nullptr;
  if (b->res && b->res->copy_issued) {
    static const bool spin = std::getenv("MGX_WAIT_POLICY") != nullptr && std::string(std::getenv("MGX_WAIT_POLICY")) == "spin";
    if (spin) {
      MGX_HIP(hipEventSynchronize(b->res->done_ev));
    } else {
      for (;;) {
        const hipError_t q = hipEventQuery(b->res->done_ev);
        if (q == hipSuccess) break;
        if (q != hipErrorNotReady) return Fail(MGX_ERR_INTERNAL, std::string("hipEventQuery: ") + hipGetErrorString(q));
        std::this_thread::sleep_for(std::chrono::microseconds(20));
      }
    }
  } else {
    if (!b->page.qids.empty())
      MGX_HIP(hipMemcpyAsync(b->h_page_out, b->d_page_out.p, b->po_bytes, hipMemcpyDeviceToHost, s));
    if (!b->score.qids.empty())
      MGX_HIP(hipMemcpyAsync(b->h_score_out, b->d_score_out.p, b->so_bytes, hipMemcpyDeviceToHost, s));
    MGX_HIP(hipStreamSynchronize(s));
  }
  if (!b->score.qids.empty()) {
    mgx_batch::Group& g = b->score;
    const size_t n = g.qids.size();
    const char* h = static_cast<const char*>(b->h_score_out);
    const unsigned long long* hc = reinterpret_cast<const unsigned long long*>(h);
    for (size_t i = 0; i < n * 8; ++i) g.h_counters[i] = hc[i];
    override_tot = reinterpret_cast<const unsigned long long*>(h + b->so_override);
    page_scores = reinterpret_cast<const double*>(h + b->so_scores);
    page_docs = reinterpret_cast<const uint32_t*>(h + b->so_docs);
    page_n = reinterpret_cast<const uint32_t*>(h + b->so_n);
  }
  BitmapPages bm;
  if (!b->bitmap.qids.empty()) {
    int rc = FetchBitmapPages(b, &bm);
    if (rc) return rc;
  }
  const uint32_t* dp_docs = nullptr;
  const unsigned long long* dp_totals = nullptr;
  if (!b->page.qids.empty()) {
    const char* h = static_cast<const char*>(b->h_page_out);
    const unsigned long long* hc = reinterpret_cast<const unsigned long long*>(h);
    for (size_t i = 0; i < b->page.qids.size() * 8; ++i) b->page.h_counters[i] = hc[i];
    dp_docs = reinterpret_cast<const uint32_t*>(h + b->po_docs);
    dp_totals = reinterpret_cast<const unsigned long long*>(h + b->po_totals);
  }
  std::vector<uint32_t> pos_in_group(b->n_queries, 0);
  for (size_t i = 0; i < b->score.qids.size(); ++i) pos_in_group[b->score.qids[i]] = static_cast<uint32_t>(i);
  for (size_t i = 0; i < b->bitmap.qids.size(); ++i) pos_in_group[b->bitmap.qids[i]] = static_cast<uint32_t>(i);
  for (size_t i = 0; i < b->page.qids.size(); ++i) pos_in_group[b->page.qids[i]] = static_cast<uint32_t>(i);
  uint64_t n_out = 0;
  for (uint32_t qi = 0; qi < b->n_queries; ++qi) {
    mgx_query_result& r = b->h_results[qi];
    const uint32_t gi = pos_in_group[qi];
    const bool sc = b->specs[qi].mode == kModeScore, pg = b->specs[qi].mode == kModeDocPage;
    const unsigned long long* c =
        (sc ? b->score : pg ? b->page : b->bitmap).h_counters.data() + static_cast<size_t>(gi) * 8;
    r.total_candidates = c[0];
    r.after_intersection = c[1];
    r.after_not = c[2];
    r.after_filters = c[3];
    r.total = c[4];
    if (sc && b->merged_shards) r.total = override_tot[gi];
    if (pg && b->merged_shards) r.total = dp_totals[gi];
    if (!sc && !pg) r.total = bm.total[gi];
    r.n_docs = sc   ? page_n[gi]
               : pg ? static_cast<uint32_t>(std::min<uint64_t>(r.total, b->specs[qi].limit))
                    : static_cast<uint32_t>(bm.page_n[gi]);
    r.docs_begin = static_cast<uint32_t>(n_out);
    n_out += r.n_docs;
  }
  if (n_out > 0xFFFFFFFFull) return Fail(MGX_ERR_OUT_OF_RANGE, "batch result exceeds 2^32 doc ids");
  b->h_docs.resize(n_out);
  b->h_scores.assign(n_out, 0.0);
  for (uint32_t qi = 0; qi < b->n_queries; ++qi) {
    const mgx_query_result& r = b->h_results[qi];
    if (r.n_docs == 0) continue;
    const uint32_t gi = pos_in_group[qi];
    const uint32_t mode = b->specs[qi].mode;
    uint32_t* dst = b->h_docs.data() + r.docs_begin;
    if (mode == kModeScore) {
      std::memcpy(dst, page_docs + static_cast<size_t>(gi) * b->page_stride, r.n_docs * sizeof(uint32_t));
      std::memcpy(b->h_scores.data() + r.docs_begin, page_scores + static_cast<size_t>(gi) * b->page_stride,
                  r.n_docs * sizeof(double));
    } else if (mode == kModeDocPage) {
      std::memcpy(dst, dp_docs + static_cast<size_t>(gi) * b->doc_page_stride, r.n_docs * sizeof(uint32_t));
    } else {
      std::memcpy(dst, bm.docs.data() + bm.page_off[gi], r.n_docs * sizeof(uint32_t));
      if (b->specs[qi].deep_score)
        std::memcpy(b->h_scores.data() + r.docs_begin, bm.scores.data() + bm.page_off[gi], r.n_docs * sizeof(double));
    }
  }
  out->n_queries = b->n_queries;
  out->queries = b->h_results.data();
  out->docs = b->h_docs.data();
  out->scores = b->h_scores.data();
  b->fetched = true;
  return MGX_OK;
}

}

extern "C" {

int mgx_batch_prepare(mgx_index* idx, const mgx_query* queries, uint32_t n_queries, mgx_batch** out) {
  if (out) *out = nullptr;
  if (!idx || !out || (n_queries && !queries))
    return mgx::Fail(MGX_ERR_INVALID_ARGUMENT, "mgx_batch_prepare: null argument");
  try {
    std::vector<mgx::QuerySpec> specs(n_queries);
    const int rc = mgx::CompileAll(idx, queries, n_queries, &specs);
    if (rc) return rc;
    return mgx::PrepareFromSpecs(idx, std::move(specs), out);
  } catch (const std::exception& e) {
    return mgx::Fail(MGX_ERR_INTERNAL, std::string("mgx_batch_prepare: ") + e.what());
  }
}

int mgx_batch_reset(mgx_batch* batch, const mgx_query* queries, uint32_t n_queries) {
  if (!batch || (n_queries && !queries)) return mgx::Fail(MGX_ERR_INVALID_ARGUMENT, "mgx_batch_reset: null argument");
  try {
    mgx_index* idx = batch->idx;
    std::vector<mgx::QuerySpec> specs = std::move(batch->specs);
    specs.resize(n_queries);
    int rc = MGX_OK;
    static const bool kTrace = std::getenv("MGX_TRACE_HOST") != nullptr;
    const auto t0 = std::chrono::steady_clock::now();
    rc = mgx::CompileAll(idx, queries, n_queries, &specs);
    const auto t1 = std::chrono::steady_clock::now();
    MGX_HIP(hipSetDevice(idx->device));
    mgx::ResetBatch(batch);
    if (rc) return rc;
    rc = mgx::PrepareInto(batch, idx, std::move(specs));
    if (kTrace) {
      static std::atomic<uint64_t> n{0};
      static std::atomic<uint64_t> us_compile{0}, us_into{0};
      const auto t2 = std::chrono::steady_clock::now();
      us_compile += std::chrono::duration_cast<std::chrono::microseconds>(t1 - t0).count();
      us_into += std::chrono::duration_cast<std::chrono::microseconds>(t2 - t1).count();
      static const uint64_t period = std::max(1, atoi(std::getenv("MGX_TRACE_HOST")) > 1 ? atoi(std::getenv("MGX_TRACE_HOST")) : 64);
      if (++n % period == 0) {
        const double per = static_cast<double>(period);
        fprintf(stderr, "[mgx] reset x%llu: CompileQuery loop %.3f ms, reset + PrepareInto %.3f ms per batch\n",
                static_cast<unsigned long long>(period), us_compile.exchange(0) / (per * 1e3), us_into.exchange(0) / (per * 1e3));
        for (int k = 0; k < mgx::kSections; ++k)
          fprintf(stderr, "[mgx]   %-24s %.3f ms\n", mgx::kSectionNames[k], mgx::g_section_us[k].exchange(0) / (per * 1e6));
      }
    }
    return rc;
  } catch (const std::exception& e) {
    return mgx::Fail(MGX_ERR_INTERNAL, std::string("mgx_batch_reset: ") + e.what());
  }
}

int mgx_batch_stream(mgx_batch* batch, void** hip_stream) {
  if (hip_stream) *hip_stream = nullptr;
  if (!batch || !hip_stream || !batch->res) return mgx::Fail(MGX_ERR_INVALID_ARGUMENT, "mgx_batch_stream: null argument");
  if (!batch->res->stream) {
    MGX_HIP(hipSetDevice(batch->idx->device));
    MGX_HIP(hipStreamCreateWithFlags(&batch->res->stream, hipStreamNonBlocking));
  }
  *hip_stream = batch->res->stream;
  return MGX_OK;
}

int mgx_batch_execute(mgx_batch* batch, void* hip_stream) {
// ... 1182 lines not shown
```

mygram-db_amd/csrc/shim/mygram_shim.cpp:

```cpp
#include "mygram_shim.hpp"

#include "../mgx_highlight.hpp"
#include "../mgx_text.hpp"

#include <algorithm>
#include <atomic>
#include <charconv>
#include <chrono>
#include <cstring>
#include <cmath>
#include <cstdio>
#include <cstdlib>
#include <condition_variable>
#include <deque>
#include <functional>
#include <future>
#include <iterator>
#include <map>
#include <mutex>
#include <thread>
#include <unordered_map>

#include <pthread.h>

// ... 2507 lines not shown
    return out;
  }
  mgx_batch* batch = nullptr;
  int rc = mgx_batch_prepare(im->dev, mq.data(), static_cast<uint32_t>(mq.size()), &batch);
  if (rc != MGX_OK) return MakeUnexpected(MakeError(static_cast<ErrorCode>(rc), mgx_last_error()));
  std::unique_ptr<mgx_batch, void (*)(mgx_batch*)> guard(batch, mgx_batch_destroy);
  HighlightRequests hreq;
  {
    const Error he = AttachHighlight(index, delta.get(), queries, plans, batch, &hreq);
    if (he.code() != ErrorCode::kSuccess) return MakeUnexpected(he);
  }
  if (delta) {
    mgx_batch* dbatch = nullptr;
    rc = mgx_batch_prepare(delta->impl()->dev, dq.data(), static_cast<uint32_t>(dq.size()), &dbatch);
    if (rc != MGX_OK) return MakeUnexpected(MakeError(static_cast<ErrorCode>(rc), mgx_last_error()));
    std::unique_ptr<mgx_batch, void (*)(mgx_batch*)> dguard(dbatch, mgx_batch_destroy);
    void* stream = nullptr;
    rc = mgx_batch_stream(batch, &stream);
    if (rc == MGX_OK) rc = RunWithDelta(batch, dbatch, stream);
    if (rc != MGX_OK) return MakeUnexpected(MakeError(static_cast<ErrorCode>(rc), mgx_last_error()));
    mgx_result_view dv{};
    rc = mgx_batch_fetch(batch, &v);
    if (rc == MGX_OK) rc = mgx_batch_fetch(dbatch, &dv);
    if (rc != MGX_OK) return MakeUnexpected(MakeError(static_cast<ErrorCode>(rc), mgx_last_error()));
    Collect(plans, v, &out, &dv);
    rc = CollectSnippets(queries, plans, batch, v, &out);
    if (rc != MGX_OK) return MakeUnexpected(MakeError(static_cast<ErrorCode>(rc), mgx_last_error()));
    return out;
  }
  rc = mgx_batch_execute(batch, nullptr);
  if (rc != MGX_OK) return MakeUnexpected(MakeError(static_cast<ErrorCode>(rc), mgx_last_error()));
  rc = mgx_batch_fetch(batch, &v);
  if (rc != MGX_OK) return MakeUnexpected(MakeError(static_cast<ErrorCode>(rc), mgx_last_error()));
  Collect(plans, v, &out);
  rc = CollectSnippets(queries, plans, batch, v, &out);
  if (rc != MGX_OK) return MakeUnexpected(MakeError(static_cast<ErrorCode>(rc), mgx_last_error()));
  return out;
}

namespace {
Error FacetOne(const index::Index& index, const BatchQuery& query, const std::string& column, bool* found,
               std::vector<storage::FilterValue>* dict, std::vector<uint64_t>* counts, uint64_t* matched) {
  index.FlushPendingFilterColumns();
  index::Index::Impl* im = index.impl();
  uint32_t device_column = 0;
  *found = false;
  *matched = 0;
  {
    std::lock_guard<std::mutex> lock(im->filter_mu);
    const index::Index::Impl::FilterColumn* col = im->ResolveColumn(column);
    if (col != nullptr) {
      *found = true;
      device_column = col->device_id;
      *dict = col->dict;
    }
  }
  BatchQuery q = query;
  q.sort_by_score = false;
  q.limit = 0;
  q.offset = 0;
  if (q.terms.empty() && !q.ast) {
    auto all = std::make_shared<query::QueryNode>(query::NodeType::NOT);
    all->children.push_back(std::make_unique<query::QueryNode>(std::string()));
    q.ast = std::move(all);
  }
  PlannedQuery plan;
  PlanQuery(index, q, index.Bm25DocCount(), index.Bm25AvgDocLength(), &plan);
  if (plan.error != ErrorCode::kSuccess) return MakeError(plan.error, plan.error_message);
  counts->assign(std::max<size_t>(dict->size(), 1), 0);
  if (plan.on_device && *found) {
    if (mgx_facet_counts(im->dev, &plan.q, device_column, counts->data(), matched) != MGX_OK)
      return MakeError(ErrorCode::kInternalError, mgx_last_error());
  }
  return Error{ErrorCode::kSuccess, ""};
}
}

Expected<FacetOutput, Error> ExecuteFacet(const index::Index& index, const BatchQuery& query, const std::string& column) {
  index.Finalize();
  index::Index::Impl* im = index.impl();
  if (!im->dev) return MakeUnexpected(MakeError(ErrorCode::kInternalError, im->last_error));
  {
    const std::string merr = index.ApplyMutations();
    if (!merr.empty()) return MakeUnexpected(MakeError(ErrorCode::kInternalError, merr));
  }
  const std::shared_ptr<index::Index> delta = DeltaOf(index);
  if (delta && !query.filters.empty())
    return MakeUnexpected(MakeError(ErrorCode::kNotImplemented,
                                    "BatchQuery::filters (raw bitmap ids) belong to one device index: a table with a delta takes filter_conditions"));
  bool found = false, dfound = false;
  std::vector<storage::FilterValue> dict, ddict;
  std::vector<uint64_t> counts, dcounts;
  FacetOutput out;
  Error e = FacetOne(index, query, column, &found, &dict, &counts, &out.matched_documents);
  if (e.code() != ErrorCode::kSuccess) return MakeUnexpected(e);
  if (delta) {
    uint64_t dmatched = 0;
    e = FacetOne(*delta, query, column, &dfound, &ddict, &dcounts, &dmatched);
    if (e.code() != ErrorCode::kSuccess) return MakeUnexpected(e);
    out.matched_documents += dmatched;
    if (dfound) {
      std::vector<storage::FilterValue> merged;
      std::vector<uint64_t> mcounts;
      size_t i = 0, j = 0;
      const size_t ni = found ? dict.size() : 0;
      while (i < ni || j < ddict.size()) {
        if (j == ddict.size() || (i < ni && dict[i] < ddict[j])) {
          merged.push_back(dict[i]);
          mcounts.push_back(counts[i]);
          ++i;
        } else if (i == ni || ddict[j] < dict[i]) {
          merged.push_back(ddict[j]);
          mcounts.push_back(dcounts[j]);
          ++j;
        } else {
          merged.push_back(dict[i]);
          mcounts.push_back(counts[i] + dcounts[j]);
          ++i;
          ++j;
        }
      }
      dict.swap(merged);
      counts.swap(mcounts);
      found = true;
    }
  }
  if (!found)
    return MakeUnexpected(MakeError(ErrorCode::kIndexNotFound, "Facet column \"" + column + "\" not found"));
  std::vector<size_t> order;
  for (size_t v = 0; v < dict.size(); ++v)
    if (counts[v] > 0) order.push_back(v);
  std::stable_sort(order.begin(), order.end(), [&](size_t a, size_t b) { return counts[a] > counts[b]; });
  out.total_values = order.size();
  const size_t first = std::min<size_t>(query.offset, order.size());
  const size_t last = std::min<size_t>(order.size(), first + static_cast<size_t>(query.limit));
  for (size_t k = first; k < last; ++k) {
    out.value_counts.emplace_back(storage::SerializeFilterValue(dict[order[k]]), counts[order[k]]);
    out.display.push_back(storage::FilterValueToDisplayString(dict[order[k]]));
  }
  return out;
}


struct BatchExecutor::Impl {
  using clock = std::chrono::steady_clock;
  const index::Index& index;
  Options opt;
  uint64_t total_docs = 0;
  double avgdl = 0.0;
  enum State { kFree, kFilling, kPlanning, kPlanned, kCompiling, kCompiled, kEnqueued, kFailed };
  struct Slot {
    mgx_batch* batch = nullptr;
    std::vector<BatchQuery> queries;
    std::vector<PlannedQuery> plans;
    std::vector<mgx_query> mq;
    std::shared_ptr<index::Index::Impl::Handles> handles;
    std::shared_ptr<index::Index> delta, dbatch_index;
    std::vector<PlannedQuery> dplans;
    std::vector<mgx_query> dq;
    HighlightRequests hreq;
    mgx_batch* dbatch = nullptr;
    uint64_t total_docs = 0;
    double avgdl = 0.0;
    uint64_t ticket = 0;
    State state = kFree;
    size_t chunks_left = 0;
    Error error{ErrorCode::kSuccess, ""};
    Timing timing;
    clock::time_point t_submit, t_planned, t_compiled;
  };
  struct Chunk {
    Slot* slot;
    size_t begin, end;
  };
  static constexpr size_t kChunk = 64;
  std::vector<Slot> slots;
  uint64_t next_ticket = 1, next_compile = 1, next_enqueue = 1;
  std::vector<std::thread> workers;
  std::vector<std::thread> dispatchers;
  std::mutex mu;
  std::condition_variable cv_work, cv_state;
  std::deque<Chunk> chunks;
  bool stop = false;
  bool enqueuing = false;
  bool comm_poisoned = false;
  std::string poison_message;

  Impl(const index::Index& ix, Options o) : index(ix), opt(o) {}

  Slot* ByTicket(uint64_t ticket) {
    for (auto& s : slots)
      if (s.state != kFree && s.state != kFilling && s.ticket == ticket) return &s;
    return nullptr;
  }

  void Compile(Slot* slot) {
    index::Index::Impl* im = index.impl();
    static const bool kTrace = std::getenv("MGX_TRACE_HOST") != nullptr;
    const auto t_in = clock::now();
    slot->mq.clear();
    for (const auto& p : slot->plans) {
      if (p.error != ErrorCode::kSuccess) {
        slot->error = MakeError(p.error, p.error_message);
        return;
      }
      if (p.on_device) slot->mq.push_back(p.q);
    }
    slot->timing.device_queries = static_cast<uint32_t>(slot->mq.size());
    slot->dq.clear();
    if (slot->delta) {
      for (const auto& p : slot->dplans) {
        if (p.error != ErrorCode::kSuccess) {
          slot->error = MakeError(p.error, p.error_message);
          return;
        }
        if (p.on_device) slot->dq.push_back(p.q);
      }
    }
    if (slot->mq.empty()) return;
    if (kTrace) {
      static std::atomic<uint64_t> n{0}, us{0};
      us += std::chrono::duration_cast<std::chrono::microseconds>(clock::now() - t_in).count();
      if (++n % 64 == 0) fprintf(stderr, "[shim] gather of the planned queries: %.3f ms per batch\n", us.exchange(0) / 64e3);
    }
    int rc;
    {
      std::shared_ptr<index::Index::Impl::Handles> cur;
      {
        std::lock_guard<std::mutex> il(im->mu);
        cur = im->handles;
      }
      if (slot->batch && slot->handles != cur) {
        mgx_batch_destroy(slot->batch);
        slot->batch = nullptr;
      }
      slot->handles = std::move(cur);
    }
    if (!slot->batch)
      rc = mgx_batch_prepare(im->dev, slot->mq.data(), static_cast<uint32_t>(slot->mq.size()), &slot->batch);
    else
      rc = mgx_batch_reset(slot->batch, slot->mq.data(), static_cast<uint32_t>(slot->mq.size()));
    if (rc != MGX_OK) {
      slot->error = MakeError(static_cast<ErrorCode>(rc), mgx_last_error());
      return;
    }
    slot->error = AttachHighlight(index, slot->delta.get(), slot->queries, slot->plans, slot->batch, &slot->hreq);
    if (slot->error.code() != ErrorCode::kSuccess) return;
    if (slot->dbatch && slot->dbatch_index != slot->delta) {
      mgx_batch_destroy(slot->dbatch);
      slot->dbatch = nullptr;
      slot->dbatch_index.reset();
    }
    if (!slot->delta) return;
    if (!slot->dbatch) {
      rc = mgx_batch_prepare(slot->delta->impl()->dev, slot->dq.data(), static_cast<uint32_t>(slot->dq.size()), &slot->dbatch);
      if (rc == MGX_OK) slot->dbatch_index = slot->delta;
    } else {
      rc = mgx_batch_reset(slot->dbatch, slot->dq.data(), static_cast<uint32_t>(slot->dq.size()));
    }
    if (rc != MGX_OK) slot->error = MakeError(static_cast<ErrorCode>(rc), mgx_last_error());
  }

  void EnqueueReady(std::unique_lock<std::mutex>& lock) {
    if (enqueuing) return;
    enqueuing = true;
    for (;;) {
      Slot* slot = ByTicket(next_enqueue);
      if (!slot || (slot->state != kCompiled && slot->state != kFailed)) break;
      if (opt.comm && comm_poisoned && slot->state == kCompiled) {
        slot->error = MakeError(ErrorCode::kInternalError, "the table's communicator was aborted after an earlier failure: " + poison_message);
        slot->state = kFailed;
      } else if (opt.comm && slot->state == kFailed && !comm_poisoned) {
        comm_poisoned = true;
        poison_message = slot->error.message();
        (void)mgx_comm_abort(opt.comm);
      }
      if (slot->state == kCompiled && !slot->mq.empty()) {
        lock.unlock();
        const auto t0 = clock::now();
        void* stream = nullptr;
        int rc = mgx_batch_stream(slot->batch, &stream);
        mgx_comm* comm = opt.comm;
        if (rc == MGX_OK && slot->delta) {
          rc = RunWithDelta(slot->batch, slot->dbatch, stream);
        } else {
          static const bool kTrace = std::getenv("MGX_TRACE_HOST") != nullptr;
          const auto e0 = clock::now();
          if (rc == MGX_OK && comm) rc = mgx_batch_exchange_df(slot->batch, comm, stream);
          const auto e1 = clock::now();
          if (rc == MGX_OK)
            rc = comm ? mgx_batch_execute_sharded(slot->batch, comm, stream) : mgx_batch_execute(slot->batch, stream);
          const auto e2 = clock::now();
          if (rc == MGX_OK && comm) rc = mgx_batch_exchange(slot->batch, comm, stream);
          if (kTrace) {
            static std::atomic<uint64_t> n{0}, a{0}, b{0}, c{0};
            a += std::chrono::duration_cast<std::chrono::nanoseconds>(e1 - e0).count();
            b += std::chrono::duration_cast<std::chrono::nanoseconds>(e2 - e1).count();
            c += std::chrono::duration_cast<std::chrono::nanoseconds>(clock::now() - e2).count();
            if (++n % 64 == 0)
              fprintf(stderr, "[shim] enqueue per batch: exchange_df %.1f us, execute %.1f us, exchange %.1f us\n",
                      a.exchange(0) / 64e3, b.exchange(0) / 64e3, c.exchange(0) / 64e3);
          }
        }
        if (rc != MGX_OK) slot->error = MakeError(static_cast<ErrorCode>(rc), mgx_last_error());
        slot->timing.enqueue_ms = std::chrono::duration<double, std::milli>(clock::now() - t0).count();
        lock.lock();
        if (rc != MGX_OK && comm && !comm_poisoned) {
          comm_poisoned = true;
          poison_message = slot->error.message();
          (void)mgx_comm_abort(comm);
        }
      }
      slot->state = slot->error.code() == ErrorCode::kSuccess && slot->state == kCompiled ? kEnqueued : kFailed;
      ++next_enqueue;
      cv_state.notify_all();
    }
    enqueuing = false;
  }

  void Work() {
    std::unique_lock<std::mutex> lock(mu);
    for (;;) {
      cv_work.wait(lock, [&] { return stop || !chunks.empty(); });
      if (stop) return;
      const Chunk c = chunks.front();
      chunks.pop_front();
      lock.unlock();
      for (size_t i = c.begin; i < c.end; ++i) {
        c.slot->plans[i].Reset();
        PlanQuery(index, c.slot->queries[i], c.slot->total_docs, c.slot->avgdl, &c.slot->plans[i]);
        if (c.slot->delta) {
          c.slot->dplans[i].Reset();
          if (c.slot->plans[i].error == ErrorCode::kSuccess)
            PlanForDelta(*c.slot->delta, c.slot->queries[i], c.slot->total_docs, c.slot->avgdl, c.slot->plans[i],
                         &c.slot->dplans[i]);
        }
      }
      lock.lock();
      if (--c.slot->chunks_left != 0) continue;
      c.slot->t_planned = clock::now();
      c.slot->state = kPlanned;
      cv_state.notify_all();
    }
  }

  void Dispatch() {
    std::unique_lock<std::mutex> lock(mu);
    for (;;) {
      Slot* slot = nullptr;
      cv_state.wait(lock, [&] {
        slot = ByTicket(next_compile);
        return stop || (slot && slot->state == kPlanned);
      });
      if (stop) return;
      slot->state = kCompiling;
      ++next_compile;
      lock.unlock();
      const auto t_begin = clock::now();
      Compile(slot);
      slot->t_compiled = clock::now();
      slot->timing.plan_ms = std::chrono::duration<double, std::milli>(slot->t_planned - slot->t_submit).count();
      slot->timing.compile_ms = std::chrono::duration<double, std::milli>(slot->t_compiled - t_begin).count();
      lock.lock();
      slot->state = slot->error.code() == ErrorCode::kSuccess ? kCompiled : kFailed;
      EnqueueReady(lock);
    }
  }
};

BatchExecutor::BatchExecutor(const index::Index& index, Options options) : impl_(std::make_unique<Impl>(index, options)) {
  index.Finalize();
  impl_->total_docs = index.Bm25DocCount();
  impl_->avgdl = index.Bm25AvgDocLength();
  impl_->slots.resize(static_cast<size_t>(std::max(1, options.depth)));
  for (int t = 0; t < std::max(1, options.planner_threads); ++t)
    impl_->workers.emplace_back([this] {
      pthread_setname_np(pthread_self(), "mgx-plan");
      impl_->Work();
    });
  static const int kDispatchers = std::getenv("MGX_DISPATCHERS") ? atoi(std::getenv("MGX_DISPATCHERS")) : 3;
  const int n_dispatchers = std::max(1, std::min(kDispatchers, std::max(1, options.depth)));
  for (int t = 0; t < n_dispatchers; ++t)
    impl_->dispatchers.emplace_back([this] {
      pthread_setname_np(pthread_self(), "mgx-dispatch");
      impl_->Dispatch();
    });
}

BatchExecutor::~BatchExecutor() {
  {
    std::unique_lock<std::mutex> lock(impl_->mu);
    impl_->cv_state.wait(lock, [&] {
      for (auto& s : impl_->slots)
        if (s.state == Impl::kPlanning || s.state == Impl::kPlanned || s.state == Impl::kCompiling ||
            s.state == Impl::kCompiled)
          return false;
      return true;
    });
    impl_->stop = true;
  }
  impl_->cv_work.notify_all();
  impl_->cv_state.notify_all();
  for (auto& w : impl_->workers) w.join();
  for (auto& d : impl_->dispatchers) d.join();
  for (auto& s : impl_->slots) {
    if (s.state == Impl::kEnqueued && s.batch && !s.mq.empty()) {
      mgx_result_view v{};
      (void)mgx_batch_fetch(s.batch, &v);
    }
    if (s.dbatch) mgx_batch_destroy(s.dbatch);
    if (s.batch) mgx_batch_destroy(s.batch);
  }
}

Expected<uint64_t, Error> BatchExecutor::Submit(std::vector<BatchQuery>&& queries) {
  index::Index::Impl* im = impl_->index.impl();
  if (!im->dev) return MakeUnexpected(MakeError(ErrorCode::kInternalError, im->last_error));
  index::MutationStep step;
  bool mutable_table = false;
  {
    std::lock_guard<std::mutex> il(im->mu);
    step = index::NextMutationStep(im->mut, false);
    mutable_table = im->mut.active;
  }
  if (step == index::MutationStep::kInstall) {
    if (impl_->opt.comm)
      return MakeUnexpected(MakeError(ErrorCode::kNotImplemented, "a sharded table (Options::comm) is static"));
    std::unique_lock<std::mutex> lock(impl_->mu);
    impl_->cv_state.wait(lock, [&] {
      for (auto& s : impl_->slots)
        if (s.state == Impl::kPlanning || s.state == Impl::kPlanned || s.state == Impl::kCompiling || s.state == Impl::kCompiled)
          return false;
      return true;
    });
  }
  if (step != index::MutationStep::kNothing) {
    const std::string merr = impl_->index.ApplyMutations();
    if (!merr.empty()) return MakeUnexpected(MakeError(ErrorCode::kInternalError, merr));
  }
  if (mutable_table) {
    impl_->total_docs = impl_->index.Bm25DocCount();
    impl_->avgdl = impl_->index.Bm25AvgDocLength();
  }
  if (impl_->opt.comm && AnyHighlight(queries))
    return MakeUnexpected(MakeError(ErrorCode::kNotImplemented,
                                    "highlight on a sharded table (Options::comm) is not implemented: the page's texts "
                                    "live on other ranks"));
  Impl::Slot* slot = nullptr;
  {
    std::lock_guard<std::mutex> lock(impl_->mu);
    for (auto& s : impl_->slots)
      if (s.state == Impl::kFree) {
        slot = &s;
        break;
      }
    if (!slot)
      return MakeUnexpected(MakeError(ErrorCode::kInvalidArgument,
                                      "BatchExecutor: every slot holds an unfetched batch (Wait for one first)"));
    slot->state = Impl::kFilling;
  }
  slot->queries.swap(queries);
  slot->plans.resize(slot->queries.size());
  slot->total_docs = impl_->total_docs;
  slot->avgdl = impl_->avgdl;
  slot->delta = DeltaOf(impl_->index);
  if (slot->delta) slot->dplans.resize(slot->queries.size());
  slot->error = Error{ErrorCode::kSuccess, ""};
  slot->timing = Timing{};
  slot->t_submit = Impl::clock::now();
  const size_t n = slot->queries.size();
  std::lock_guard<std::mutex> lock(impl_->mu);
  slot->ticket = impl_->next_ticket++;
  slot->state = Impl::kPlanning;
  slot->chunks_left = std::max<size_t>(1, (n + Impl::kChunk - 1) / Impl::kChunk);
  if (n == 0) impl_->chunks.push_back(Impl::Chunk{slot, 0, 0});
  for (size_t a = 0; a < n; a += Impl::kChunk) impl_->chunks.push_back(Impl::Chunk{slot, a, std::min(n, a + Impl::kChunk)});
  impl_->cv_work.notify_all();
  return slot->ticket;
}

Expected<uint64_t, Error> BatchExecutor::Submit(const std::vector<BatchQuery>& queries) {
  return Submit(std::vector<BatchQuery>(queries));
}

Expected<std::vector<BatchResult>, Error> BatchExecutor::Wait(uint64_t ticket, Timing* timing) {
  std::vector<BatchResult> out;
  const Error e = WaitInto(ticket, &out, timing);
  if (e.code() != ErrorCode::kSuccess) return MakeUnexpected(e);
  return out;
}

Error BatchExecutor::Warm(const std::vector<BatchQuery>& sample, int rounds) {
  const size_t depth = impl_->slots.size();
  std::vector<uint64_t> tickets;
  std::vector<BatchResult> sink;
  for (int r = 0; r < std::max(1, rounds); ++r) {
    tickets.clear();
    for (size_t k = 0; k < depth; ++k) {
      auto t = Submit(sample);
      if (!t) return t.error();
      tickets.push_back(*t);
    }
    for (uint64_t t : tickets) {
      const Error e = WaitInto(t, &sink);
      if (e.code() != ErrorCode::kSuccess) return e;
    }
  }
  return Error{ErrorCode::kSuccess, ""};
}

Error BatchExecutor::WaitInto(uint64_t ticket, std::vector<BatchResult>* results, Timing* timing) {
  std::vector<BatchResult>& out = *results;
  std::unique_lock<std::mutex> lock(impl_->mu);
  Impl::Slot* s = ticket ? impl_->ByTicket(ticket) : nullptr;
  if (!s) return MakeError(ErrorCode::kInvalidArgument, "BatchExecutor::Wait: unknown ticket");
  impl_->cv_state.wait(lock, [&] { return s->state == Impl::kEnqueued || s->state == Impl::kFailed; });
  if (s->state == Impl::kFailed) {
    const Error e = s->error;
    s->state = Impl::kFree;
    return e;
  }
  lock.unlock();
  mgx_result_view v{}, dv{};
  const auto t0 = Impl::clock::now();
  if (!s->mq.empty()) {
    int rc = mgx_batch_fetch(s->batch, &v);
    if (rc == MGX_OK && s->delta) rc = mgx_batch_fetch(s->dbatch, &dv);
    if (rc != MGX_OK) {
      const Error e = MakeError(static_cast<ErrorCode>(rc), mgx_last_error());
      lock.lock();
      s->state = Impl::kFree;
      return e;
    }
  }
  Collect(s->plans, v, &out, s->delta ? &dv : nullptr);
  if (!s->mq.empty()) {
    const int rc = CollectSnippets(s->queries, s->plans, s->batch, v, &out);
    if (rc != MGX_OK) {
      const Error e = MakeError(static_cast<ErrorCode>(rc), mgx_last_error());
      lock.lock();
      s->state = Impl::kFree;
      return e;
    }
  }
  s->timing.wait_ms = std::chrono::duration<double, std::milli>(Impl::clock::now() - t0).count();
  if (timing) *timing = s->timing;
  lock.lock();
  s->state = Impl::kFree;
  return Error{ErrorCode::kSuccess, ""};
}


struct MicroBatcher::Impl {
  using clock = std::chrono::steady_clock;
  struct Waiter {
    std::mutex mu;
    std::condition_variable cv;
    bool done = false;
    Expected<BatchResult, Error> result{MakeUnexpected(MakeError(ErrorCode::kInternalError, "unanswered"))};
  };
  struct InFlight {
    uint64_t ticket = 0;
    std::vector<Waiter*> waiters;
    Error submit_error{ErrorCode::kSuccess, ""};
  };
  Options opt;
  BatchExecutor executor;
  std::mutex mu;
  std::condition_variable cv_pending, cv_inflight, cv_room;
  std::vector<BatchQuery> pending;
  std::vector<Waiter*> pending_waiters;
  clock::time_point first_arrival;
  std::deque<InFlight> inflight;
  Stats stats;
  bool stop = false;
  std::thread former, completer;

  Impl(const index::Index& index, Options o) : opt(o), executor(index, o.executor) {}

  static void Answer(Waiter* w, Expected<BatchResult, Error>&& r) {
    std::lock_guard<std::mutex> lock(w->mu);
    w->result = std::move(r);
    w->done = true;
    w->cv.notify_one();
  }

  void Form() {
    std::unique_lock<std::mutex> lock(mu);
    for (;;) {
      cv_pending.wait(lock, [&] { return stop || !pending.empty(); });
      if (pending.empty()) return;
      const auto deadline = first_arrival + opt.max_delay;
      const bool full = cv_pending.wait_until(lock, deadline, [&] { return stop || pending.size() >= opt.max_batch; });
      cv_room.wait(lock, [&] { return inflight.size() < static_cast<size_t>(std::max(1, opt.executor.depth)); });
      InFlight f;
      std::vector<BatchQuery> batch;
      const size_t take = std::min(pending.size(), opt.max_batch);
      batch.assign(std::make_move_iterator(pending.begin()), std::make_move_iterator(pending.begin() + take));
      f.waiters.assign(pending_waiters.begin(), pending_waiters.begin() + take);
      pending.erase(pending.begin(), pending.begin() + take);
      pending_waiters.erase(pending_waiters.begin(), pending_waiters.begin() + take);
      if (!pending.empty()) first_arrival = clock::now();
      ++stats.batches;
      stats.queries += take;
      ++(full && take == opt.max_batch ? stats.closed_full : stats.closed_by_delay);
      lock.unlock();
      auto t = executor.Submit(std::move(batch));
      lock.lock();
      if (t) f.ticket = *t; else f.submit_error = t.error();
      inflight.push_back(std::move(f));
      cv_inflight.notify_one();
    }
  }

// ... 69 lines not shown
```

mygram-db_amd/csrc/shim/mygram_shim.hpp:

```cpp
#pragma once

#include <chrono>
#include <cstdint>
#include <memory>
#include <optional>
#include <string>
#include <unordered_map>
#include <string_view>
#include <utility>
#include <variant>
#include <vector>

#include "../../../include/mygram_gpu.h"

namespace mygram::utils {

enum class ErrorCode : std::uint16_t {
  kSuccess = 0,
  kInvalidArgument = 2,
  kOutOfRange = 3,
  kNotImplemented = 4,
  kInternalError = 5,
  kQueryInvalidSort = 3007,
  kIndexNotFound = 4000,
// ... 162 lines not shown
}

namespace mygramdb::storage {
class DocumentStore {
 public:
  explicit DocumentStore(const index::Index& index) : index_(&index) {}
  [[nodiscard]] const index::Index& index() const { return *index_; }
  [[nodiscard]] bool IsStoreTextsEnabled() const { return true; }
  [[nodiscard]] size_t Size() const;

 private:
  const index::Index* index_;
};
}

namespace mygramdb::index {

struct BM25Params {
  double k1 = 1.2;
  double b = 0.75;
};

struct ScoredDoc {
  DocId doc_id;
  double score;
};

class BM25Scorer {
 public:
  static double ComputeIDF(uint64_t total_docs, uint64_t doc_freq);
  static mygram::utils::Expected<std::vector<ScoredDoc>, mygram::utils::Error> ScoreDocuments(
      const std::vector<DocId>& candidates, const std::vector<std::string>& search_terms,
      const std::vector<uint64_t>& term_doc_freqs, const Index& index, uint64_t total_docs, double avg_doc_length,
      const BM25Params& params);
  static mygram::utils::Expected<std::vector<ScoredDoc>, mygram::utils::Error> ScoreDocuments(
      const std::vector<DocId>& candidates, const std::vector<std::string>& search_terms,
      const std::vector<uint64_t>& term_doc_freqs, const storage::DocumentStore& doc_store, uint64_t total_docs,
      double avg_doc_length, const BM25Params& params) {
    return ScoreDocuments(candidates, search_terms, term_doc_freqs, doc_store.index(), total_docs, avg_doc_length, params);
  }
};

}

namespace mygramdb::query {

using DocId = storage::DocId;
enum class SortOrder : uint8_t { ASC, DESC };
enum class FilterOp : uint8_t { EQ, NE, GT, GTE, LT, LTE };
struct FilterCondition {
  std::string column;
  FilterOp op = FilterOp::EQ;
  std::string value;
};

enum class NodeType : uint8_t { AND, OR, NOT, TERM };
struct QueryNode {
  NodeType type;
  std::string term;
  std::vector<std::unique_ptr<QueryNode>> children;
  explicit QueryNode(std::string term_value) : type(NodeType::TERM), term(std::move(term_value)) {}
  explicit QueryNode(NodeType node_type) : type(node_type) {}
};

struct HighlightOptions {
  std::string open_tag = "<em>";
  std::string close_tag = "</em>";
  uint32_t snippet_length = 100;
  uint32_t max_fragments = 3;
};
struct HighlightResult {
  std::string snippet;
};
class Highlighter {
 public:
  static HighlightResult Generate(std::string_view normalized_text, const std::vector<std::string>& search_terms,
                                  const HighlightOptions& options);
  static std::vector<std::pair<uint32_t, uint32_t>> FindMatchPositions(std::string_view normalized_text,
                                                                       const std::vector<std::string>& search_terms);
};

class ResultSorter {
 public:
  static std::vector<DocId> SortByScore(const index::Index& index, const std::vector<DocId>& results,
                                        const std::vector<double>& scores, SortOrder order, uint32_t limit,
                                        uint32_t offset);
  static std::vector<DocId> SortByScore(const std::vector<DocId>& results, const std::vector<double>& scores,
                                        SortOrder order, uint32_t limit, uint32_t offset);
};

}

namespace mygramdb::search_pipeline {

using DocId = storage::DocId;

struct BatchQuery {
  std::vector<std::string> terms;
  std::shared_ptr<const query::QueryNode> ast;
  std::vector<std::string> not_terms;
  std::vector<std::pair<uint32_t, bool>> filters;
  std::vector<query::FilterCondition> filter_conditions;
  uint32_t fuzzy_max_distance = 0;
  bool sort_by_score = false;
  bool verify_text = false;
  query::SortOrder order = query::SortOrder::DESC;
  uint32_t limit = 100;
  uint32_t offset = 0;
  index::BM25Params bm25;
  std::optional<query::HighlightOptions> highlight;
};

std::vector<std::string> BuildHighlightTerms(const std::vector<std::string>& search_terms, const index::Index* index);

struct BatchResult {
  std::vector<DocId> results;
  std::vector<double> scores;
  uint64_t total = 0;
  size_t total_candidates = 0, after_intersection = 0, after_not = 0, after_filters = 0;
  bool empty_term_detected = false;
  std::vector<std::string> snippets;
};

mygram::utils::Expected<std::vector<BatchResult>, mygram::utils::Error> ExecuteBatch(
    const index::Index& index, const std::vector<BatchQuery>& queries);

struct FacetOutput {
  uint64_t matched_documents = 0;
  uint64_t total_values = 0;
  std::vector<std::pair<std::string, uint64_t>> value_counts;
  std::vector<std::string> display;
};
mygram::utils::Expected<FacetOutput, mygram::utils::Error> ExecuteFacet(const index::Index& index, const BatchQuery& query,
                                                                        const std::string& column);

class BatchExecutor {
 public:
  struct Options {
    int depth = 2;
    int planner_threads = 4;
    mgx_comm* comm = nullptr;
  };
  struct Timing {
    double plan_ms = 0, compile_ms = 0, enqueue_ms = 0, wait_ms = 0;
    uint32_t device_queries = 0;
  };
  BatchExecutor(const index::Index& index, Options options);
  explicit BatchExecutor(const index::Index& index) : BatchExecutor(index, Options{}) {}
  ~BatchExecutor();
  BatchExecutor(const BatchExecutor&) = delete;
  BatchExecutor& operator=(const BatchExecutor&) = delete;
  mygram::utils::Expected<uint64_t, mygram::utils::Error> Submit(const std::vector<BatchQuery>& queries);
  mygram::utils::Expected<uint64_t, mygram::utils::Error> Submit(std::vector<BatchQuery>&& queries);
  mygram::utils::Expected<std::vector<BatchResult>, mygram::utils::Error> Wait(uint64_t ticket, Timing* timing = nullptr);
  mygram::utils::Error Warm(const std::vector<BatchQuery>& sample, int rounds = 2);
  mygram::utils::Error WaitInto(uint64_t ticket, std::vector<BatchResult>* results, Timing* timing = nullptr);

 private:
  struct Impl;
  std::unique_ptr<Impl> impl_;
};

class MicroBatcher {
 public:
  struct Options {
    size_t max_batch = 1024;
    std::chrono::microseconds max_delay{200};
    BatchExecutor::Options executor;
  };
  struct Stats {
    uint64_t batches = 0, queries = 0;
    uint64_t closed_full = 0, closed_by_delay = 0;
  };
  MicroBatcher(const index::Index& index, Options options);
  ~MicroBatcher();
  MicroBatcher(const MicroBatcher&) = delete;
  MicroBatcher& operator=(const MicroBatcher&) = delete;
  [[nodiscard]] mygram::utils::Expected<BatchResult, mygram::utils::Error> Search(BatchQuery query);
  [[nodiscard]] Stats GetStats() const;

 private:
  struct Impl;
  std::unique_ptr<Impl> impl_;
};

}
```

mygram-db_amd/csrc/shim/shim_capi.cpp:

```cpp
#include <algorithm>
#include <chrono>
#include <cstring>
#include <memory>
#include <mutex>
#include <string>
#include <unordered_map>
#include <vector>

#include "../../../include/mygram_shim_c.h"
#include "mygram_shim.hpp"

using mygramdb::index::Index;
using mygramdb::search_pipeline::BatchExecutor;
using mygramdb::search_pipeline::BatchQuery;
using mygramdb::search_pipeline::MicroBatcher;

struct mgxs_table {
  std::unique_ptr<Index> index;
};
struct mgxs_executor {
  std::unique_ptr<BatchExecutor> ex;
  std::vector<BatchQuery> queries;
  std::vector<mygramdb::search_pipeline::BatchResult> results;
  std::mutex limits_mu;
  std::unordered_map<uint64_t, uint32_t> limits;
};

struct mgxs_batcher {
  std::unique_ptr<MicroBatcher> mb;
};

namespace {
thread_local std::string g_err;
int Fail(int code, const std::string& msg) {
  g_err = msg;
  return code;
}
}

extern "C" {

const char* mgxs_last_error(void) { return g_err.c_str(); }

int mgxs_table_adopt(mgx_columns* columns, mgx_index* device_index, int ngram_size, int kanji_ngram_size,
                     int cross_boundary_ngrams, mgxs_table** out) {
  if (out) *out = nullptr;
  if (!columns || !device_index || !out) return Fail(MGX_ERR_INVALID_ARGUMENT, "mgxs_table_adopt: null argument");
  try {
    auto t = std::make_unique<mgxs_table>();
    t->index = Index::Adopt(columns, device_index, ngram_size, kanji_ngram_size, cross_boundary_ngrams != 0);
    if (!t->index->LastError().empty()) return Fail(MGX_ERR_INTERNAL, t->index->LastError());
    *out = t.release();
    return MGX_OK;
  } catch (const std::exception& e) {
    return Fail(MGX_ERR_INTERNAL, e.what());
  }
}

int mgxs_table_from_dump(const uint8_t* data, uint64_t len, const char* table_name, int device, mgxs_table** out) {
  if (out) *out = nullptr;
  if (!data || !out) return Fail(MGX_ERR_INVALID_ARGUMENT, "mgxs_table_from_dump: null argument");
  try {
    std::string err;
    auto t = std::make_unique<mgxs_table>();
    t->index = Index::FromDump(data, len, table_name ? table_name : "", &err, device);
    if (!t->index) return Fail(MGX_ERR_INVALID_ARGUMENT, err);
    *out = t.release();
    return MGX_OK;
  } catch (const std::exception& e) {
    return Fail(MGX_ERR_INTERNAL, e.what());
  }
}

int mgxs_table_set_global_stats(mgxs_table* table, uint64_t total_docs, double avg_doc_length,
                                const uint64_t* global_posting_sizes, uint64_t n_grams) {
  if (!table || (n_grams && !global_posting_sizes))
    return Fail(MGX_ERR_INVALID_ARGUMENT, "mgxs_table_set_global_stats: null argument");
  try {
    const std::string err = table->index->SetGlobalStats(
        total_docs, avg_doc_length, std::vector<uint64_t>(global_posting_sizes, global_posting_sizes + n_grams));
    return err.empty() ? MGX_OK : Fail(MGX_ERR_INVALID_ARGUMENT, err);
  } catch (const std::exception& e) {
    return Fail(MGX_ERR_INTERNAL, e.what());
  }
}

int mgxs_table_set_normalization(mgxs_table* table, int nfkc, const char* width, int lower) {
  if (!table || !width) return Fail(MGX_ERR_INVALID_ARGUMENT, "mgxs_table_set_normalization: null argument");
  try {
    table->index->SetNormalization(nfkc != 0, width, lower != 0);
    return MGX_OK;
  } catch (const std::exception& e) {
    return Fail(MGX_ERR_INTERNAL, e.what());
  }
}

int mgxs_normalize_uses_icu(void) { return mygram::utils::NormalizeTextUsesIcu() ? 1 : 0; }

int mgxs_normalize_text(const char* text, size_t len, int nfkc, const char* width, int lower, char* out, size_t cap,
                        size_t* out_len) {
  if ((len && !text) || !width || !out_len || (cap && !out))
    return Fail(MGX_ERR_INVALID_ARGUMENT, "mgxs_normalize_text: null argument");
  try {
    const std::string r = mygram::utils::NormalizeText(std::string_view(text ? text : "", len), nfkc != 0, width, lower != 0);
    *out_len = r.size();
    if (r.size() > cap) return Fail(MGX_ERR_OUT_OF_RANGE, "mgxs_normalize_text: output buffer too small (*out_len holds the size)");
    if (!r.empty()) std::memcpy(out, r.data(), r.size());
    return MGX_OK;
  } catch (const std::exception& e) {
    return Fail(MGX_ERR_INTERNAL, e.what());
  }
}

int mgxs_table_set_absent_grams(mgxs_table* table, uint64_t n, const char* const* grams, const uint64_t* sizes) {
  if (!table || (n && (!grams || !sizes))) return Fail(MGX_ERR_INVALID_ARGUMENT, "mgxs_table_set_absent_grams: null argument");
  try {
    std::unordered_map<std::string, uint64_t> m;
    for (uint64_t i = 0; i < n; ++i) m.emplace(grams[i], sizes[i]);
    table->index->SetAbsentGrams(std::move(m));
    return MGX_OK;
  } catch (const std::exception& e) {
    return Fail(MGX_ERR_INTERNAL, e.what());
  }
}

void mgxs_table_destroy(mgxs_table* table) { delete table; }

int mgxs_executor_create_sharded(mgxs_table* table, int depth, int planner_threads, mgx_comm* comm, mgxs_executor** out) {
  if (out) *out = nullptr;
  if (!table || !out) return Fail(MGX_ERR_INVALID_ARGUMENT, "mgxs_executor_create_sharded: null argument");
  try {
    auto e = std::make_unique<mgxs_executor>();
    BatchExecutor::Options o;
    o.depth = depth > 0 ? depth : 2;
    o.planner_threads = planner_threads > 0 ? planner_threads : 1;
    o.comm = comm;
    e->ex = std::make_unique<BatchExecutor>(*table->index, o);
    *out = e.release();
    return MGX_OK;
  } catch (const std::exception& e) {
    return Fail(MGX_ERR_INTERNAL, e.what());
  }
}

int mgxs_executor_create(mgxs_table* table, int depth, int planner_threads, mgxs_executor** out) {
  return mgxs_executor_create_sharded(table, depth, planner_threads, nullptr, out);
}

void mgxs_executor_destroy(mgxs_executor* ex) { delete ex; }

namespace {
void FillQueries(std::vector<BatchQuery>* out, uint32_t n_queries, const uint32_t* n_terms, const char* const* terms,
                 uint32_t limit, uint32_t offset, int sort_by_score, int descending) {
  out->resize(n_queries);
  size_t at = 0;
  for (uint32_t i = 0; i < n_queries; ++i) {
    BatchQuery& q = (*out)[i];
    q.terms.resize(n_terms[i]);
    for (uint32_t t = 0; t < n_terms[i]; ++t) q.terms[t].assign(terms[at++]);
    q.ast.reset();
    q.not_terms.clear();
    q.filters.clear();
    q.fuzzy_max_distance = 0;
    q.verify_text = false;
    q.bm25 = mygramdb::index::BM25Params{};
    q.sort_by_score = sort_by_score != 0;
    q.order = descending ? mygramdb::query::SortOrder::DESC : mygramdb::query::SortOrder::ASC;
    q.limit = limit;
    q.offset = offset;
  }
}
}

int mgxs_executor_warm(mgxs_executor* ex, uint32_t n_queries, const uint32_t* n_terms, const char* const* terms,
                       uint32_t limit, uint32_t offset, int sort_by_score, int descending, int rounds) {
  if (!ex || (n_queries && (!n_terms || !terms))) return Fail(MGX_ERR_INVALID_ARGUMENT, "mgxs_executor_warm: null argument");
  try {
    std::vector<BatchQuery> sample;
    FillQueries(&sample, n_queries, n_terms, terms, limit, offset, sort_by_score, descending);
    const auto e = ex->ex->Warm(sample, rounds);
    if (e.code() != mygram::utils::ErrorCode::kSuccess) return Fail(static_cast<int>(e.code()), e.message());
    return MGX_OK;
  } catch (const std::exception& e) {
    return Fail(MGX_ERR_INTERNAL, e.what());
  }
}

int mgxs_submit(mgxs_executor* ex, uint32_t n_queries, const uint32_t* n_terms, const char* const* terms,
                uint32_t limit, uint32_t offset, int sort_by_score, int descending, uint64_t* ticket) {
  if (ticket) *ticket = 0;
  if (!ex || !ticket || (n_queries && (!n_terms || !terms)))
    return Fail(MGX_ERR_INVALID_ARGUMENT, "mgxs_submit: null argument");
  try {
    FillQueries(&ex->queries, n_queries, n_terms, terms, limit, offset, sort_by_score, descending);
    auto r = ex->ex->Submit(std::move(ex->queries));
    if (!r) return Fail(static_cast<int>(r.error().code()), r.error().message());
    *ticket = *r;
    {
      std::lock_guard<std::mutex> lock(ex->limits_mu);
      ex->limits[*r] = limit;
    }
    return MGX_OK;
  } catch (const std::exception& e) {
    return Fail(MGX_ERR_INTERNAL, e.what());
  }
}

int mgxs_wait(mgxs_executor* ex, uint64_t ticket, uint64_t* totals, uint32_t* n_docs, uint32_t* docs, double* scores,
              double* timing_ms) {
  if (!ex || !totals || !n_docs || !docs) return Fail(MGX_ERR_INVALID_ARGUMENT, "mgxs_wait: null argument");
  try {
    BatchExecutor::Timing tm;
    uint32_t limit = 0;
    {
      std::lock_guard<std::mutex> lock(ex->limits_mu);
      const auto lim = ex->limits.find(ticket);
      if (lim != ex->limits.end()) {
        limit = lim->second;
        ex->limits.erase(lim);
      }
    }
    const auto err = ex->ex->WaitInto(ticket, &ex->results, &tm);
    if (err.code() != mygram::utils::ErrorCode::kSuccess) return Fail(static_cast<int>(err.code()), err.message());
    const auto& res = ex->results;
    for (size_t i = 0; i < res.size(); ++i) {
      totals[i] = res[i].total;
      const size_t n = res[i].results.size();
      n_docs[i] = static_cast<uint32_t>(n);
      for (size_t k = 0; k < n && k < limit; ++k) {
        docs[i * limit + k] = res[i].results[k];
        if (scores) scores[i * limit + k] = k < res[i].scores.size() ? res[i].scores[k] : 0.0;
      }
    }
    if (timing_ms) {
      timing_ms[0] = tm.plan_ms;
      timing_ms[1] = tm.compile_ms;
      timing_ms[2] = tm.enqueue_ms;
      timing_ms[3] = tm.wait_ms;
      timing_ms[4] = static_cast<double>(tm.device_queries);
    }
    return MGX_OK;
  } catch (const std::exception& e) {
    return Fail(MGX_ERR_INTERNAL, e.what());
  }
}

namespace {
using mygramdb::query::FilterCondition;
using mygramdb::query::FilterOp;
using mygramdb::storage::FilterValue;

BatchQuery MakeQuery(uint32_t n_terms, const char* const* terms, uint32_t n_not, const char* const* not_terms,
                     uint32_t n_cond, const char* const* cond_columns, const uint32_t* cond_ops,
                     const char* const* cond_values, int sort_by_score, int descending, uint32_t limit, uint32_t offset) {
  BatchQuery q;
  for (uint32_t t = 0; t < n_terms; ++t) q.terms.emplace_back(terms[t]);
  for (uint32_t t = 0; t < n_not; ++t) q.not_terms.emplace_back(not_terms[t]);
  for (uint32_t c = 0; c < n_cond; ++c)
    q.filter_conditions.push_back(FilterCondition{cond_columns[c], static_cast<FilterOp>(cond_ops[c]), cond_values[c]});
  q.sort_by_score = sort_by_score != 0;
  q.order = descending ? mygramdb::query::SortOrder::DESC : mygramdb::query::SortOrder::ASC;
  q.limit = limit;
  q.offset = offset;
  return q;
}
}

int mgxs_table_add_filter_column(mgxs_table* table, const char* name, int value_type, uint64_t n, const void* values,
                                 const char* const* strings, const uint8_t* is_null) {
  if (!table || !name || (n && !values && !strings)) return Fail(MGX_ERR_INVALID_ARGUMENT, "mgxs_table_add_filter_column: null argument");
  if (value_type < 1 || value_type > 12) return Fail(MGX_ERR_INVALID_ARGUMENT, "mgxs_table_add_filter_column: value_type is 1..12");
  try {
    std::vector<FilterValue> v(n);
    const int64_t* si = static_cast<const int64_t*>(values);
    const uint64_t* ui = static_cast<const uint64_t*>(values);
    const double* di = static_cast<const double*>(values);
    for (uint64_t i = 0; i < n; ++i) {
      if (is_null && is_null[i]) continue;
      switch (value_type) {
        case 1: v[i] = si[i] != 0; break;
        case 2: v[i] = static_cast<int8_t>(si[i]); break;
        case 3: v[i] = static_cast<uint8_t>(ui[i]); break;
        case 4: v[i] = static_cast<int16_t>(si[i]); break;
        case 5: v[i] = static_cast<uint16_t>(ui[i]); break;
        case 6: v[i] = static_cast<int32_t>(si[i]); break;
        case 7: v[i] = static_cast<uint32_t>(ui[i]); break;
        case 8: v[i] = static_cast<int64_t>(si[i]); break;
        case 9: v[i] = static_cast<uint64_t>(ui[i]); break;
        case 10: v[i] = mygramdb::storage::TimeValue{si[i]}; break;
        case 11: v[i] = std::string(strings[i]); break;
        default: v[i] = di[i]; break;
      }
    }
    const std::string err = table->index->AddFilterColumn(name, v);
    return err.empty() ? MGX_OK : Fail(MGX_ERR_INVALID_ARGUMENT, err);
  } catch (const std::exception& e) {
    return Fail(MGX_ERR_INTERNAL, e.what());
  }
}

namespace {
mygramdb::storage::FilterMap MakeFilterMap(uint32_t n, const char* const* names, const int* types, const void* values,
                                           const char* const* strings) {
  mygramdb::storage::FilterMap m;
  const int64_t* si = static_cast<const int64_t*>(values);
  const uint64_t* ui = static_cast<const uint64_t*>(values);
  const double* di = static_cast<const double*>(values);
  for (uint32_t i = 0; i < n; ++i) {
    FilterValue v;
    switch (types[i]) {
      case 1: v = si[i] != 0; break;
      case 2: v = static_cast<int8_t>(si[i]); break;
      case 3: v = static_cast<uint8_t>(ui[i]); break;
      case 4: v = static_cast<int16_t>(si[i]); break;
      case 5: v = static_cast<uint16_t>(ui[i]); break;
      case 6: v = static_cast<int32_t>(si[i]); break;
      case 7: v = static_cast<uint32_t>(ui[i]); break;
      case 8: v = static_cast<int64_t>(si[i]); break;
      case 9: v = static_cast<uint64_t>(ui[i]); break;
      case 10: v = mygramdb::storage::TimeValue{si[i]}; break;
      case 11: v = std::string(strings[i]); break;
      case 12: v = di[i]; break;
      default: break;
    }
    m[names[i]] = std::move(v);
  }
  return m;
}
}

int mgxs_table_add_document(mgxs_table* table, uint32_t doc_id, const char* text, size_t len, uint32_t n_filters,
                            const char* const* names, const int* types, const void* values, const char* const* strings) {
  if (!table || (len && !text)) return Fail(MGX_ERR_INVALID_ARGUMENT, "mgxs_table_add_document: null argument");
  try {
    const size_t stats_before = table->index->GetMutationStats().delta_documents;
    const std::string_view t(text ? text : "", len);
    if (n_filters) table->index->AddDocument(doc_id, t, MakeFilterMap(n_filters, names, types, values, strings));
    else table->index->AddDocument(doc_id, t);
    if (table->index->GetMutationStats().delta_documents == stats_before)
      return Fail(MGX_ERR_INVALID_ARGUMENT, table->index->LastError());
    return MGX_OK;
  } catch (const std::exception& e) {
    return Fail(MGX_ERR_INTERNAL, e.what());
  }
}

int mgxs_table_update_document(mgxs_table* table, uint32_t doc_id, const char* old_text, size_t old_len, const char* new_text,
                               size_t new_len, int with_filters, uint32_t n_filters, const char* const* names,
// ... 236 lines not shown
```

Before: 1.063 million.

## Move group planning into reusable plan module and submit queries as flat term buffers

Moves query layout, fast-route resolution, item cutting and scheduling out of the API file into a separate planning module. GroupPlan now lives in per-batch resources with scratch vectors (order, band_at, sorted, keys) so allocations are reused across batches, and a block-max memo is added. The C submit path packs terms into a flat byte buffer, and worker threads build BatchQuery objects from it in parallel instead of on the submitting thread. The aim is to cut host-side planning and allocation cost per batch, at the price of a larger code movement that could subtly change scheduling behaviour.

```diff
diff --git a/mygram-db_amd/csrc/mgx_api.cpp b/mygram-db_amd/csrc/mgx_api.cpp
--- a/mygram-db_amd/csrc/mgx_api.cpp
+++ b/mygram-db_amd/csrc/mgx_api.cpp
@@ -22,6 +22,7 @@
 
 #include "../../include/mygram_gpu.h"
 #include "mgx_compile.hpp"
+#include "mgx_plan.hpp"
 #include "mgx_highlight.hpp"
 #include "mgx_host.hpp"
 #include "mgx_internal.hpp"
@@ -129,6 +130,8 @@
   hipEvent_t done_ev = nullptr;
   hipEvent_t main_ev = nullptr;
   bool copy_issued = false;
+  std::chrono::steady_clock::time_point t_recorded;
+  double done_after_us = 0.0;
   void* xchg[4] = {nullptr, nullptr, nullptr, nullptr};
   size_t xchg_cap[4] = {0, 0, 0, 0};
   hipError_t Exchange(int which, size_t bytes, void** out_ptr) {
@@ -183,6 +186,7 @@
     *out_ptr = h_down[which];
     return hipSuccess;
   }
+  GroupPlan plans[4];
   void Reset() {
     upload.Reset();
     out.Reset();
@@ -1310,15 +1314,6 @@
 using Group = mgx_batch::Group;
 using RouteLaunch = mgx_batch::RouteLaunch;
 
-enum class Route : uint8_t {
-  kBlock,
-  kWave,
-  kWaveLists,
-  kFast,
-  kCand,
-  kMerge,
-};
-
 static bool EnvZero(const char* name) { return std::getenv(name) && atoi(std::getenv(name)) == 0; }
 struct PathSwitches {
   const bool wave = std::getenv("MGX_FORCE_BLOCK_KERNEL") == nullptr;
@@ -1326,170 +1321,28 @@
   const bool merge = wave && !EnvZero("MGX_MERGE");
 };
 
-struct GroupPlan {
-  GroupPlan(uint32_t n_, uint32_t mode)
-      : n(n_), score_mode(mode == kModeScore), df_mode(mode == kModeTextDf), page_mode(mode == kModeDocPage) {}
-  const uint32_t n;
-  const bool score_mode, df_mode, page_mode;
-  std::vector<DevQuery> dq;
-  std::vector<DevLeaf> leaves;
-  std::vector<uint32_t> prog;
-  std::vector<DevScoreTerm> score;
-  std::vector<uint32_t> expl;
-  uint32_t max_limit = 1, max_needed = 1;
-  std::vector<Route> route;
-  std::vector<DevFastQuery> fastq;
-  std::vector<uint64_t> wave_tables;
-  std::vector<uint32_t> cand_driver;
-  std::vector<DevItem> items;
-  std::vector<uint32_t> list_begin, item_begin;
-  std::vector<DevItem> block, wave, wave_lists, fast[kFastMaxScore], cand, merge;
-  std::vector<uint8_t> has_seed;
-};
-
-static int LayOutQueries(mgx_batch* b, Group& g, const std::vector<QuerySpec>& specs, GroupPlan& p) {
-  std::vector<DevLeaf>& leaves = p.leaves;
-  std::vector<uint32_t>& expl = p.expl;
-  p.dq.resize(p.n);
-  uint32_t max_leaves = 0, max_lds_leaves = 0, max_score = 0, max_stack = 0, max_instr = 0, max_cap = 64;
-  for (uint32_t i = 0; i < p.n; ++i) {
-    const QuerySpec& s = specs[g.qids[i]];
-    DevQuery& q = p.dq[i];
-    std::memset(&q, 0, sizeof(q));
-    q.leaf_begin = static_cast<uint32_t>(leaves.size());
-    q.n_leaves = static_cast<uint32_t>(s.leaves.size());
-    q.prog_begin = static_cast<uint32_t>(p.prog.size());
-    q.n_instr = static_cast<uint32_t>(s.prog.size());
-    q.score_begin = static_cast<uint32_t>(p.score.size());
-    q.n_score = static_cast<uint32_t>(s.score.size());
-    q.mode = s.mode;
-    q.limit = s.limit;
-    q.offset = s.offset;
-    q.needed = static_cast<uint32_t>(std::min<uint64_t>(static_cast<uint64_t>(s.offset) + s.limit, 0xFFFFFFFFull));
-    uint32_t cap = 64;
-    if (s.mode == kModeScore)
-      while (cap < q.needed && cap < (1u << 30)) cap <<= 1;
-    q.cap = cap;
-    q.descending = s.reverse;
-    q.stack_depth = s.stack_depth;
-    q.out_slot = i;
-    q.pat_off = s.pat_off;
-    q.pat_len = s.pat_len;
-    q.vt_begin = s.vt_begin;
-    q.vt_count = static_cast<uint32_t>(s.verify_patterns.size());
-    q.fz_distance = s.fz_distance;
-    q.vp_begin = s.vp_begin;
-    q.k1 = s.k1;
-    q.b = s.b;
-    q.one_minus_b = 1.0 - s.b;
-    q.k1_plus_1 = s.k1 + 1.0;
-    q.avgdl_clamped = std::max(s.avgdl, 1.0);
-    const uint32_t ebase = static_cast<uint32_t>(expl.size());
-    uint32_t n_lds = 0;
-    for (size_t li = 0; li < s.leaves.size(); ++li) {
-      DevLeaf lf = s.leaves[li];
-      if (lf.kind == kLeafExplicit) lf.a += ebase;
-      bool resident = lf.kind == kLeafList || lf.kind == kLeafExplicit;
-      for (const DevScoreTerm& st : s.score) resident = resident || st.leaf == li;
-      lf.lds = resident ? n_lds++ : kNoRow;
-      leaves.push_back(lf);
-    }
-    if (n_lds > kMaxLdsLeaves)
-      return Fail(MGX_ERR_NOT_IMPLEMENTED,
-                  "query " + std::to_string(g.qids[i]) + ": more than 64 sorted-list / scored operands in one query");
-    max_lds_leaves = std::max(max_lds_leaves, n_lds);
-    p.prog.insert(p.prog.end(), s.prog.begin(), s.prog.end());
-    p.score.insert(p.score.end(), s.score.begin(), s.score.end());
-    expl.insert(expl.end(), s.explicit_ids.begin(), s.explicit_ids.end());
-    while (expl.size() % 4) expl.push_back(0xFFFFFFFFu);
-    max_leaves = std::max(max_leaves, q.n_leaves);
-    max_score = std::max(max_score, q.n_score);
-    max_stack = std::max(max_stack, q.stack_depth);
-    max_instr = std::max(max_instr, q.n_instr);
-    max_cap = std::max(max_cap, q.cap);
-    p.max_limit = std::max(p.max_limit, q.limit);
-    p.max_needed = std::max(p.max_needed, q.needed);
-    if (!p.df_mode) b->list_bytes += 4 * s.list_postings;
-  }
-  g.plan = PlanLds(max_leaves, max_lds_leaves, max_score, max_stack, max_instr, max_cap, p.score_mode || p.df_mode);
-  return MGX_OK;
-}
-
-static bool ResolveFast(mgx_index* idx, const uint64_t* cond_arena, const QuerySpec& s, const DevQuery& q, DevFastQuery* out) {
-  DevFastQuery& f = *out;
-  for (uint32_t ins : s.prog) {
-    const uint32_t op = ins >> 24, arg = ins & 0xFFFFFFu;
-    if (op == kOpCount) {
-      if (f.n_ops == 0) return false;
-      f.ops[f.n_ops - 1].code |= arg << 8;
-      continue;
-    }
-    const DevLeaf& lf = s.leaves[arg];
-    if (f.n_ops == static_cast<uint32_t>(kFastMaxOps) || (op == kOpLoad) != (f.n_ops == 0)) return false;
-    FastOp o{};
-    uint64_t stride = 0;
-    if (lf.kind == kLeafGramBitmap) {
-      o.base = reinterpret_cast<uint64_t>(idx->dev.gram_bitmaps + static_cast<uint64_t>(lf.b) * idx->dev.gb_row_stride);
-      stride = idx->dev.gb_tile_stride * 8;
-    } else if (lf.kind == kLeafFilterBitmap) {
-      o.base = static_cast<uint64_t>(lf.b) * idx->dev.fb_row_stride * 8;
-      stride = idx->dev.fb_tile_stride * 8;
-      o.code |= 16u;
-    } else if (lf.kind == kLeafCondBitmap) {
-      o.base = reinterpret_cast<uint64_t>(cond_arena + static_cast<uint64_t>(lf.b) * idx->dev.fb_row_stride);
-      stride = idx->dev.fb_tile_stride * 8;
-    } else {
-      return false;
-    }
-    if (stride > 0xFFFFFFFFull) return false;
-    o.tile_stride = static_cast<uint32_t>(stride);
-    o.code |= (op == kOpLoad || op == kOpOr) ? kFastOr : op == kOpAnd ? kFastAnd : kFastAndNot;
-    f.ops[f.n_ops++] = o;
-  }
-  if (f.n_ops == 0) return false;
-  for (size_t t = 0; t < s.score.size(); ++t) {
-    const DevLeaf& lf = s.leaves[s.score[t].leaf];
-    if (lf.kind != kLeafGramBitmap) return false;
-    FastScore& fs = f.score[t];
-    fs.nib = reinterpret_cast<uint64_t>(idx->dev.tfnib + static_cast<uint64_t>(lf.b) * idx->dev.nib_row_stride);
-    fs.idf = s.score[t].idf;
-    fs.gram = lf.a;
-    fs.skip_row = lf.row;
-  }
-  if (s.reverse != 0) {
-    double step = 0.0;
-    f.blockmax = GetBlockMax(idx, s.k1, s.b, s.avgdl, &step, &f.blockmax_fine);
-    if (f.blockmax) {
-      f.bm_tile_stride = idx->n_bitmap_rows * 256u;
-      f.bmf_tile_stride = idx->n_fine_rows * 1024u;
-      double idf_max = 0.0;
-      for (size_t t = 0; t < s.score.size(); ++t) idf_max = std::max(idf_max, s.score[t].idf);
-      const double wunit = idf_max > 0.0 ? idf_max * (1.0 + 0x1p-40) / 255.0 : 1.0;
-      f.bm_inv_unit = 1.0 / (wunit * step);
-      f.bm_wpack = f.bm_w4 = f.bm_cint = 0;
-      for (size_t t = 0; t < s.score.size(); ++t) {
-        const uint32_t w = static_cast<uint32_t>(std::min(255.0, std::ceil(s.score[t].idf / wunit)));
-        if (t < 4) f.bm_wpack |= w << (8 * t); else f.bm_w4 = w;
-      }
-      for (size_t t = 0; t < s.score.size(); ++t) {
-        const DevLeaf& lf = s.leaves[s.score[t].leaf];
-        FastScore& fs = f.score[t];
-        const uint32_t frow = f.blockmax_fine ? idx->h_fine_map[lf.b] : kNoRow;
-        fs.bm_mode = frow != kNoRow ? 2u : 1u;
-        fs.bm_off = frow != kNoRow ? frow * 1024u : lf.b * 256u;
-      }
-    }
-  }
-  f.n_score = static_cast<uint32_t>(s.score.size());
-  f.needed = q.needed;
-  f.cap = q.cap;
-  f.descending = q.descending;
-  f.k1 = q.k1;
-  f.b = q.b;
-  f.one_minus_b = q.one_minus_b;
-  f.k1_plus_1 = q.k1_plus_1;
-  f.avgdl_clamped = q.avgdl_clamped;
-  return true;
+static const uint8_t* BlockMaxOfIndex(void* user, double k1, double b, double avgdl, double* step, const uint8_t** fine) {
+  return GetBlockMax(static_cast<mgx_index*>(user), k1, b, avgdl, step, fine);
+}
+static PlanView PlanViewOf(const mgx_batch* b) {
+  mgx_index* idx = b->idx;
+  PlanView v;
+  v.offsets = idx->h_offsets.data();
+  v.fine_map = idx->h_fine_map.data();
+  v.n_tiles = idx->dev.n_tiles;
+  v.gram_bitmaps = reinterpret_cast<uint64_t>(idx->dev.gram_bitmaps);
+  v.gb_row_stride = idx->dev.gb_row_stride;
+  v.gb_tile_stride = idx->dev.gb_tile_stride;
+  v.fb_row_stride = idx->dev.fb_row_stride;
+  v.fb_tile_stride = idx->dev.fb_tile_stride;
+  v.tfnib = reinterpret_cast<uint64_t>(idx->dev.tfnib);
+  v.nib_row_stride = idx->dev.nib_row_stride;
+  v.cond_arena = reinterpret_cast<uint64_t>(b->cond_arena);
+  v.n_bitmap_rows = idx->n_bitmap_rows;
+  v.n_fine_rows = idx->n_fine_rows;
+  v.block_max = BlockMaxOfIndex;
+  v.block_max_user = idx;
+  return v;
 }
 
 static void RouteCandMerge(mgx_batch* b, Group& g, const std::vector<QuerySpec>& specs, const PathSwitches& sw,
@@ -1559,33 +1412,14 @@
 }
 
 static int ChooseRoutes(mgx_batch* b, Group& g, const std::vector<QuerySpec>& specs, const PathSwitches& sw,
-                        GroupPlan& p) {
+                        const PlanView& view, GroupPlan& p) {
   mgx_index* idx = b->idx;
-  p.route.assign(p.n, Route::kBlock);
+  uint32_t fcap = 64;
+  double fparams[3] = {0, 0, 0};
+  const bool have_params = ChooseFastRoutes(view, g.qids, specs, sw.fast, p, &fcap, fparams);
   if (p.score_mode) {
-    uint32_t fcap = 64;
-    bool have_params = false;
-    double pk1 = 0, pb = 0, pavg = 0;
-    for (uint32_t i = 0; sw.fast && i < p.n; ++i) {
-      const QuerySpec& s = specs[g.qids[i]];
-      if (!s.flat || !s.fast_score_ok || s.score.empty() || s.score.size() > static_cast<size_t>(kFastMaxScore)) continue;
-      if (p.dq[i].cap > 128) continue;
-      if (have_params && (Bits(s.k1) != Bits(pk1) || Bits(s.b) != Bits(pb) || Bits(s.avgdl) != Bits(pavg))) continue;
-      DevFastQuery f{};
-      if (!ResolveFast(idx, b->cond_arena, s, p.dq[i], &f)) continue;
-      if (!have_params) {
-        pk1 = s.k1;
-        pb = s.b;
-        pavg = s.avgdl;
-        have_params = true;
-      }
-      if (p.fastq.empty()) p.fastq.resize(p.n);
-      p.fastq[i] = f;
-      p.route[i] = Route::kFast;
-      fcap = std::max(fcap, f.cap);
-    }
     if (have_params) {
-      const double* ktab = GetLengthNormTable(idx, pk1, pb, pavg);
+      const double* ktab = GetLengthNormTable(idx, fparams[0], fparams[1], fparams[2]);
       g.fplan = PlanFast(fcap, ktab);
       if (ktab == nullptr || g.fplan.bytes > 64 * 1024)
         for (Route& r : p.route) r = Route::kBlock;
@@ -1685,139 +1519,6 @@
   return MGX_OK;
 }
 
-static void CutItems(const mgx_batch* b, const Group& g, const std::vector<QuerySpec>& specs, GroupPlan& p) {
-  static const double kMatchesPerUnit = std::getenv("MGX_ITEM_MATCHES") ? atof(std::getenv("MGX_ITEM_MATCHES")) : 256.0;
-  static const double kItemCost = std::getenv("MGX_ITEM_COST") ? atof(std::getenv("MGX_ITEM_COST")) : 192.0;
-  static const uint32_t kMaxTiles = std::getenv("MGX_MAX_ITEM_TILES") ? static_cast<uint32_t>(atoi(std::getenv("MGX_MAX_ITEM_TILES"))) : static_cast<uint32_t>(kMaxTilesPerItem);
-  static const uint64_t want_items = std::getenv("MGX_WANT_ITEMS") ? static_cast<uint64_t>(atoll(std::getenv("MGX_WANT_ITEMS"))) : 4ull * 768ull;
-  static const uint32_t kSeedTiles = std::getenv("MGX_SEED_TILES") ? static_cast<uint32_t>(atoi(std::getenv("MGX_SEED_TILES"))) : 16u;
-  const uint32_t n = p.n, n_tiles = b->idx->dev.n_tiles;
-  p.list_begin.assign(n + 1, 0);
-  p.item_begin.assign(n + 1, 0);
-  uint32_t n_lists = 0;
-  for (uint32_t i = 0; i < n; ++i) {
-    const QuerySpec& s = specs[g.qids[i]];
-    const Route route = p.route[i];
-    p.item_begin[i] = static_cast<uint32_t>(p.items.size());
-    const bool fast = route == Route::kFast;
-    const double per_tile = 1.0 + (p.score_mode || p.df_mode ? s.est_density * kTileDocs / (fast ? kMatchesPerUnit / 2 : kMatchesPerUnit) : 0.0);
-    const double fast_scale = std::min(4.0, std::max(2.0, static_cast<double>(n_tiles) / 150.0));
-    uint32_t tiles = static_cast<uint32_t>((fast ? fast_scale * kItemCost : kItemCost) / per_tile);
-    tiles = std::max<uint32_t>(8, std::min<uint32_t>(tiles, fast ? 2 * kMaxTiles : kMaxTiles)) & ~7u;
-    if (p.score_mode) {
-      const uint64_t cap = std::max<uint64_t>(8, (static_cast<uint64_t>(n_tiles) * n / want_items + 7) & ~7ull);
-      tiles = static_cast<uint32_t>(std::min<uint64_t>(tiles, cap));
-    }
-    if (p.score_mode && route == Route::kBlock) tiles = 8;
-    p.list_begin[i] = n_lists;
-    if (route == Route::kCand) {
-      p.items.push_back(DevItem{i, p.cand_driver[i], 0, n_lists++});
-      continue;
-    }
-    uint32_t t0 = 0;
-    const uint32_t seed_tiles = std::min<uint32_t>(kSeedTiles, (n_tiles / 8) & ~7u);
-    if (fast && seed_tiles && n_tiles > 4 * seed_tiles) {
-      p.items.push_back(DevItem{i, 0, seed_tiles, n_lists++});
-      t0 = seed_tiles;
-    }
-    for (uint32_t t = t0; t < n_tiles; t += tiles) {
-      DevItem it{i, t, std::min(tiles, n_tiles - t), n_lists++};
-      p.items.push_back(it);
-    }
-  }
-  p.list_begin[n] = n_lists;
-  p.item_begin[n] = static_cast<uint32_t>(p.items.size());
-}
-
-static int ScheduleItems(const mgx_batch* b, Group& g, const std::vector<QuerySpec>& specs, GroupPlan& p) {
-  static const uint32_t kSortTiles = std::getenv("MGX_SORT_TILES") ? static_cast<uint32_t>(atoi(std::getenv("MGX_SORT_TILES"))) : 16u;
-  static const bool kXcdAffinity = std::getenv("MGX_XCD_AFFINITY") ? atoi(std::getenv("MGX_XCD_AFFINITY")) != 0 : true;
-  static const double kHeavyDensity = std::getenv("MGX_HEAVY_DENSITY") ? atof(std::getenv("MGX_HEAVY_DENSITY")) : 0.05;
-  static const double kSqueezeEnv = std::getenv("MGX_HEAVY_SQUEEZE") ? atof(std::getenv("MGX_HEAVY_SQUEEZE")) : -1.0;
-  const uint32_t n = p.n, n_tiles = b->idx->dev.n_tiles;
-  const bool deal = kXcdAffinity && p.score_mode;
-  std::vector<uint32_t> order(n);
-  for (uint32_t i = 0; i < n; ++i) order[i] = i;
-  if (deal) {
-    std::vector<uint32_t> heavy(n, 0);
-    for (uint32_t i = 0; i < n; ++i) {
-      uint64_t best = 0;
-      for (const DevLeaf& lf : specs[g.qids[i]].leaves) {
-        if (lf.kind != kLeafGramBitmap && lf.kind != kLeafList) continue;
-        const uint64_t sz = b->idx->h_offsets[lf.a + 1] - b->idx->h_offsets[lf.a];
-        if (sz > best) {
-          best = sz;
-          heavy[i] = lf.a;
-        }
-      }
-    }
-    std::stable_sort(order.begin(), order.end(), [&](uint32_t x, uint32_t y) { return heavy[x] < heavy[y]; });
-  }
-  const uint32_t n_bands = n_tiles / kSortTiles + 1;
-  const double kHeavySqueeze = kSqueezeEnv >= 0.0 ? kSqueezeEnv : 0.6 + 0.4 * std::min(1.0, n_tiles / 600.0);
-  auto band_of = [&](const DevItem& it) {
-    const Route route = p.route[it.query];
-    if (route == Route::kCand) return 0u;
-    const uint32_t band = it.tile_begin / kSortTiles;
-    if (p.score_mode && route == Route::kFast && specs[g.qids[it.query]].est_density >= kHeavyDensity)
-      return static_cast<uint32_t>(band * kHeavySqueeze);
-    return band;
-  };
-  std::vector<uint32_t> band_at(n_bands + 1, 0);
-  for (const DevItem& it : p.items) band_at[band_of(it) + 1]++;
-  for (uint32_t k = 0; k < n_bands; ++k) band_at[k + 1] += band_at[k];
-  std::vector<DevItem> sorted(p.items.size());
-  {
-    std::vector<uint32_t> cur(band_at.begin(), band_at.end() - 1);
-    for (uint32_t oi = 0; oi < n; ++oi) {
-      const uint32_t i = order[oi];
-      for (uint32_t k = p.item_begin[i]; k < p.item_begin[i + 1]; ++k) sorted[cur[band_of(p.items[k])]++] = p.items[k];
-    }
-  }
-  if (deal) {
-    for (uint32_t k = 0; k < n_bands; ++k) {
-      const size_t lo = band_at[k], m = band_at[k + 1] - lo, per = (m + 7) / 8;
-      size_t w = lo;
-      for (size_t r = 0; r < per; ++r)
-        for (size_t x = 0; x < 8; ++x)
-          if (x * per + r < m) p.items[w++] = sorted[lo + x * per + r];
-    }
-  } else {
-    p.items.swap(sorted);
-  }
-  p.has_seed.assign(n, 0);
-  for (int pass = 0; pass < 2; ++pass) {
-    for (const DevItem& it : p.items) {
-      const Route route = p.route[it.query];
-      const bool seed = route == Route::kFast && it.list == p.list_begin[it.query] && it.tile_begin == 0 &&
-                        p.list_begin[it.query + 1] - p.list_begin[it.query] > 1 && it.n_tiles <= 16;
-      if (seed != (pass == 0)) continue;
-      switch (route) {
-        case Route::kBlock: p.block.push_back(it); break;
-        case Route::kWave: p.wave.push_back(it); break;
-        case Route::kWaveLists: p.wave_lists.push_back(it); break;
-        case Route::kFast: p.fast[p.fastq[it.query].n_score - 1].push_back(it); break;
-        case Route::kCand: p.cand.push_back(it); break;
-        case Route::kMerge: p.merge.push_back(it); break;
-      }
-      if (seed && p.fastq[it.query].blockmax != 0) p.has_seed[it.query] = 1;
-    }
-    if (pass == 0)
-      for (int t = 0; t < kFastMaxScore; ++t) g.n_seed_fast[t] = static_cast<uint32_t>(p.fast[t].size());
-  }
-  g.seed_k = 0;
-  g.seed_table_docs = 0;
-  for (uint32_t i = 0; p.score_mode && i < n; ++i) {
-    const QuerySpec& sp = specs[g.qids[i]];
-    if (sp.reverse != 0 && p.dq[i].needed != 0 && p.dq[i].needed <= 128u) {
-      g.seed_k = std::max(g.seed_k, p.dq[i].needed);
-      g.seed_table_docs = std::max<uint64_t>(g.seed_table_docs, sp.total_docs);
-    }
-  }
-  if (g.seed_k) MGX_HIP(Upload(g.d_has_seed, p.has_seed.data(), p.has_seed.size()));
-  return MGX_OK;
-}
-
 static hipError_t MakeRoute(RouteLaunch& r, const DevBatch& base, const std::vector<DevItem>& items) {
   r.dev = base;
   r.dev.n_items = static_cast<uint32_t>(items.size());
@@ -1936,19 +1637,25 @@
 }
 
 static int UploadGroup(mgx_batch* b, Group& g, uint32_t mode, const std::vector<QuerySpec>& specs) {
-  GroupPlan p(static_cast<uint32_t>(g.qids.size()), mode);
-  if (p.n == 0) return MGX_OK;
+  if (g.qids.empty()) return MGX_OK;
+  GroupPlan local;
+  GroupPlan& p = b->res ? b->res->plans[mode == kModeScore ? 0 : mode == kModeBitmap ? 1 : mode == kModeTextDf ? 2 : 3] : local;
+  p.Begin(static_cast<uint32_t>(g.qids.size()), mode);
   const PathSwitches sw;
+  const PlanView view = PlanViewOf(b);
   SectionTimer sec;
-  if (const int rc = LayOutQueries(b, g, specs, p)) return rc;
+  QueryMaxima mx;
+  if (const int rc = LayOutQueries(g.qids, specs, p, &mx, &b->list_bytes)) return rc;
+  g.plan = PlanLds(mx.leaves, mx.lds_leaves, mx.score, mx.stack, mx.instr, mx.cap, p.score_mode || p.df_mode);
   sec.Mark(0);
-  if (const int rc = ChooseRoutes(b, g, specs, sw, p)) return rc;
+  if (const int rc = ChooseRoutes(b, g, specs, sw, view, p)) return rc;
   sec.Mark(1);
   if (const int rc = UploadTables(b, g, p, sec)) return rc;
   sec.Mark(3);
-  CutItems(b, g, specs, p);
+  CutItems(view, g.qids, specs, p);
   sec.Mark(4);
-  if (const int rc = ScheduleItems(b, g, specs, p)) return rc;
+  ScheduleItems(view, g.qids, specs, p, g.n_seed_fast, &g.seed_k, &g.seed_table_docs);
+  if (g.seed_k) MGX_HIP(Upload(g.d_has_seed, p.has_seed.data(), p.has_seed.size()));
   sec.Mark(5);
   if (const int rc = UploadItems(b, g, specs, p)) return rc;
   sec.Mark(6);
@@ -2233,11 +1940,33 @@
     (void)hipEventDestroy(ev.second);
   }
   const bool timing = b->timing;
+  std::vector<mgx_query_result> h_results = std::move(b->h_results);
+  std::vector<uint32_t> h_docs = std::move(b->h_docs);
+  std::vector<double> h_scores = std::move(b->h_scores);
+  mgx_batch::Group* const groups[4] = {&b->score, &b->bitmap, &b->textdf, &b->page};
+  std::vector<uint32_t> qids[4];
+  std::vector<unsigned long long> h_counters[4];
+  for (int k = 0; k < 4; ++k) {
+    qids[k] = std::move(groups[k]->qids);
+    h_counters[k] = std::move(groups[k]->h_counters);
+  }
   b->~mgx_batch();
   new (b) mgx_batch();
   b->res_owned = std::move(owned);
   b->res = res;
   b->timing = timing;
+  h_results.clear();
+  h_docs.clear();
+  h_scores.clear();
+  b->h_results = std::move(h_results);
+  b->h_docs = std::move(h_docs);
+  b->h_scores = std::move(h_scores);
+  for (int k = 0; k < 4; ++k) {
+    qids[k].clear();
+    h_counters[k].clear();
+    groups[k]->qids = std::move(qids[k]);
+    groups[k]->h_counters = std::move(h_counters[k]);
+  }
   if (res) res->Reset();
 }
 
@@ -2251,6 +1980,7 @@
     MGX_HIP(hipEventCreateWithFlags(&b->res->done_ev, hipEventDisableTiming));
   }
   MGX_HIP(hipEventRecord(b->res->done_ev, s));
+  b->res->t_recorded = std::chrono::steady_clock::now();
   b->res->copy_issued = true;
   return MGX_OK;
 }
@@ -2708,16 +2438,33 @@
   const double* page_scores = nullptr;
   const unsigned long long* override_tot = nullptr;
   if (b->res && b->res->copy_issued) {
-    static const bool spin = std::getenv("MGX_WAIT_POLICY") != nullptr && std::string(std::getenv("MGX_WAIT_POLICY")) == "spin";
+    static const std::string policy = std::getenv("MGX_WAIT_POLICY") ? std::getenv("MGX_WAIT_POLICY") : "";
+    static const bool spin = policy == "spin", nap_only = policy == "nap";
     if (spin) {
       MGX_HIP(hipEventSynchronize(b->res->done_ev));
     } else {
+      using clock = std::chrono::steady_clock;
+      constexpr double kPollLeadUs = 120.0, kPollMaxUs = 250.0;
+      const double expect_us = nap_only ? 0.0 : b->res->done_after_us;
+      bool polling = false;
+      clock::time_point poll_begin;
       for (;;) {
         const hipError_t q = hipEventQuery(b->res->done_ev);
         if (q == hipSuccess) break;
         if (q != hipErrorNotReady) return Fail(MGX_ERR_INTERNAL, std::string("hipEventQuery: ") + hipGetErrorString(q));
-        std::this_thread::sleep_for(std::chrono::microseconds(20));
+        const clock::time_point now = clock::now();
+        const double since_us = std::chrono::duration<double, std::micro>(now - b->res->t_recorded).count();
+        if (expect_us > 0.0 && since_us >= expect_us - kPollLeadUs && !polling) {
+          polling = true;
+          poll_begin = now;
+        }
+        if (polling && std::chrono::duration<double, std::micro>(now - poll_begin).count() < kPollMaxUs)
+          std::this_thread::yield();
+        else
+          std::this_thread::sleep_for(std::chrono::microseconds(20));
       }
+      const double took_us = std::chrono::duration<double, std::micro>(clock::now() - b->res->t_recorded).count();
+      b->res->done_after_us = b->res->done_after_us > 0.0 ? 0.75 * b->res->done_after_us + 0.25 * took_us : took_us;
     }
   } else {
     if (!b->page.qids.empty())
diff --git a/mygram-db_amd/csrc/mgx_plan.cpp b/mygram-db_amd/csrc/mgx_plan.cpp
--- /dev/null
+++ b/mygram-db_amd/csrc/mgx_plan.cpp
@@ -0,0 +1,384 @@
+#include "mgx_plan.hpp"
+
+#include <algorithm>
+#include <cmath>
+#include <cstdlib>
+#include <cstring>
+#include <string>
+
+#include "mgx_host.hpp"
+
+namespace mgx {
+
+static uint64_t BitsOf(double x) {
+  uint64_t u;
+  std::memcpy(&u, &x, 8);
+  return u;
+}
+
+void GroupPlan::Begin(uint32_t n_, uint32_t mode) {
+  n = n_;
+  score_mode = mode == kModeScore;
+  df_mode = mode == kModeTextDf;
+  page_mode = mode == kModeDocPage;
+  dq.clear();
+  leaves.clear();
+  prog.clear();
+  score.clear();
+  expl.clear();
+  max_limit = max_needed = 1;
+  route.clear();
+  fastq.clear();
+  wave_tables.clear();
+  cand_driver.clear();
+  items.clear();
+  list_begin.clear();
+  item_begin.clear();
+  block.clear();
+  wave.clear();
+  wave_lists.clear();
+  for (auto& f : fast) f.clear();
+  cand.clear();
+  merge.clear();
+  has_seed.clear();
+}
+
+int LayOutQueries(const std::vector<uint32_t>& qids, const std::vector<QuerySpec>& specs, GroupPlan& p, QueryMaxima* m,
+                  uint64_t* list_bytes) {
+  std::vector<DevLeaf>& leaves = p.leaves;
+  std::vector<uint32_t>& expl = p.expl;
+  p.dq.resize(p.n);
+  uint32_t max_leaves = 0, max_lds_leaves = 0, max_score = 0, max_stack = 0, max_instr = 0, max_cap = 64;
+  for (uint32_t i = 0; i < p.n; ++i) {
+    const QuerySpec& s = specs[qids[i]];
+    DevQuery& q = p.dq[i];
+    std::memset(&q, 0, sizeof(q));
+    q.leaf_begin = static_cast<uint32_t>(leaves.size());
+    q.n_leaves = static_cast<uint32_t>(s.leaves.size());
+    q.prog_begin = static_cast<uint32_t>(p.prog.size());
+    q.n_instr = static_cast<uint32_t>(s.prog.size());
+    q.score_begin = static_cast<uint32_t>(p.score.size());
+    q.n_score = static_cast<uint32_t>(s.score.size());
+    q.mode = s.mode;
+    q.limit = s.limit;
+    q.offset = s.offset;
+    q.needed = static_cast<uint32_t>(std::min<uint64_t>(static_cast<uint64_t>(s.offset) + s.limit, 0xFFFFFFFFull));
+    uint32_t cap = 64;
+    if (s.mode == kModeScore)
+      while (cap < q.needed && cap < (1u << 30)) cap <<= 1;
+    q.cap = cap;
+    q.descending = s.reverse;
+    q.stack_depth = s.stack_depth;
+    q.out_slot = i;
+    q.pat_off = s.pat_off;
+    q.pat_len = s.pat_len;
+    q.vt_begin = s.vt_begin;
+    q.vt_count = static_cast<uint32_t>(s.verify_patterns.size());
+    q.fz_distance = s.fz_distance;
+    q.vp_begin = s.vp_begin;
+    q.k1 = s.k1;
+    q.b = s.b;
+    q.one_minus_b = 1.0 - s.b;
+    q.k1_plus_1 = s.k1 + 1.0;
+    q.avgdl_clamped = std::max(s.avgdl, 1.0);
+    const uint32_t ebase = static_cast<uint32_t>(expl.size());
+    uint32_t n_lds = 0;
+    for (size_t li = 0; li < s.leaves.size(); ++li) {
+      DevLeaf lf = s.leaves[li];
+      if (lf.kind == kLeafExplicit) lf.a += ebase;
+      bool resident = lf.kind == kLeafList || lf.kind == kLeafExplicit;
+      for (const DevScoreTerm& st : s.score) resident = resident || st.leaf == li;
+      lf.lds = resident ? n_lds++ : kNoRow;
+      leaves.push_back(lf);
+    }
+    if (n_lds > kMaxLdsLeaves)
+      return Fail(MGX_ERR_NOT_IMPLEMENTED,
+                  "query " + std::to_string(qids[i]) + ": more than 64 sorted-list / scored operands in one query");
+    max_lds_leaves = std::max(max_lds_leaves, n_lds);
+    p.prog.insert(p.prog.end(), s.prog.begin(), s.prog.end());
+    p.score.insert(p.score.end(), s.score.begin(), s.score.end());
+    expl.insert(expl.end(), s.explicit_ids.begin(), s.explicit_ids.end());
+    while (expl.size() % 4) expl.push_back(0xFFFFFFFFu);
+    max_leaves = std::max(max_leaves, q.n_leaves);
+    max_score = std::max(max_score, q.n_score);
+    max_stack = std::max(max_stack, q.stack_depth);
+    max_instr = std::max(max_instr, q.n_instr);
+    max_cap = std::max(max_cap, q.cap);
+    p.max_limit = std::max(p.max_limit, q.limit);
+    p.max_needed = std::max(p.max_needed, q.needed);
+    if (!p.df_mode) *list_bytes += 4 * s.list_postings;
+  }
+  *m = QueryMaxima{max_leaves, max_lds_leaves, max_score, max_stack, max_instr, max_cap};
+  return MGX_OK;
+}
+
+bool ResolveFast(const PlanView& v, const QuerySpec& s, const DevQuery& q, DevFastQuery* out, BlockMaxMemo* memo) {
+  DevFastQuery& f = *out;
+  for (uint32_t ins : s.prog) {
+    const uint32_t op = ins >> 24, arg = ins & 0xFFFFFFu;
+    if (op == kOpCount) {
+      if (f.n_ops == 0) return false;
+      f.ops[f.n_ops - 1].code |= arg << 8;
+      continue;
+    }
+    const DevLeaf& lf = s.leaves[arg];
+    if (f.n_ops == static_cast<uint32_t>(kFastMaxOps) || (op == kOpLoad) != (f.n_ops == 0)) return false;
+    FastOp o{};
+    uint64_t stride = 0;
+    if (lf.kind == kLeafGramBitmap) {
+      o.base = v.gram_bitmaps + static_cast<uint64_t>(lf.b) * v.gb_row_stride * 8;
+      stride = v.gb_tile_stride * 8;
+    } else if (lf.kind == kLeafFilterBitmap) {
+      o.base = static_cast<uint64_t>(lf.b) * v.fb_row_stride * 8;
+      stride = v.fb_tile_stride * 8;
+      o.code |= 16u;
+    } else if (lf.kind == kLeafCondBitmap) {
+      o.base = v.cond_arena + static_cast<uint64_t>(lf.b) * v.fb_row_stride * 8;
+      stride = v.fb_tile_stride * 8;
+    } else {
+      return false;
+    }
+    if (stride > 0xFFFFFFFFull) return false;
+    o.tile_stride = static_cast<uint32_t>(stride);
+    o.code |= (op == kOpLoad || op == kOpOr) ? kFastOr : op == kOpAnd ? kFastAnd : kFastAndNot;
+    f.ops[f.n_ops++] = o;
+  }
+  if (f.n_ops == 0) return false;
+  for (size_t t = 0; t < s.score.size(); ++t) {
+    const DevLeaf& lf = s.leaves[s.score[t].leaf];
+    if (lf.kind != kLeafGramBitmap) return false;
+    FastScore& fs = f.score[t];
+    fs.nib = v.tfnib + static_cast<uint64_t>(lf.b) * v.nib_row_stride;
+    fs.idf = s.score[t].idf;
+    fs.gram = lf.a;
+    fs.skip_row = lf.row;
+  }
+  if (s.reverse != 0) {
+    double step = 0.0;
+    BlockMaxMemo local;
+    BlockMaxMemo& bm = memo ? *memo : local;
+    if (!bm.valid || bm.k1 != BitsOf(s.k1) || bm.b != BitsOf(s.b) || bm.avgdl != BitsOf(s.avgdl)) {
+      bm.valid = true;
+      bm.k1 = BitsOf(s.k1);
+      bm.b = BitsOf(s.b);
+      bm.avgdl = BitsOf(s.avgdl);
+      bm.step = 0.0;
+      bm.fine = nullptr;
+      bm.coarse = v.block_max ? v.block_max(v.block_max_user, s.k1, s.b, s.avgdl, &bm.step, &bm.fine) : nullptr;
+    }
+    step = bm.step;
+    f.blockmax = bm.coarse;
+    f.blockmax_fine = bm.fine;
+    if (f.blockmax) {
+      f.bm_tile_stride = v.n_bitmap_rows * 256u;
+      f.bmf_tile_stride = v.n_fine_rows * 1024u;
+      double idf_max = 0.0;
+      for (size_t t = 0; t < s.score.size(); ++t) idf_max = std::max(idf_max, s.score[t].idf);
+      const double wunit = idf_max > 0.0 ? idf_max * (1.0 + 0x1p-40) / 255.0 : 1.0;
+      f.bm_inv_unit = 1.0 / (wunit * step);
+      f.bm_wpack = f.bm_w4 = f.bm_cint = 0;
+      for (size_t t = 0; t < s.score.size(); ++t) {
+        const uint32_t w = static_cast<uint32_t>(std::min(255.0, std::ceil(s.score[t].idf / wunit)));
+        if (t < 4) f.bm_wpack |= w << (8 * t); else f.bm_w4 = w;
+      }
+      for (size_t t = 0; t < s.score.size(); ++t) {
+        const DevLeaf& lf = s.leaves[s.score[t].leaf];
+        FastScore& fs = f.score[t];
+        const uint32_t frow = f.blockmax_fine ? v.fine_map[lf.b] : kNoRow;
+        fs.bm_mode = frow != kNoRow ? 2u : 1u;
+        fs.bm_off = frow != kNoRow ? frow * 1024u : lf.b * 256u;
+      }
+    }
+  }
+  f.n_score = static_cast<uint32_t>(s.score.size());
+  f.needed = q.needed;
+  f.cap = q.cap;
+  f.descending = q.descending;
+  f.k1 = q.k1;
+  f.b = q.b;
+  f.one_minus_b = q.one_minus_b;
+  f.k1_plus_1 = q.k1_plus_1;
+  f.avgdl_clamped = q.avgdl_clamped;
+  return true;
+}
+
+bool ChooseFastRoutes(const PlanView& v, const std::vector<uint32_t>& qids, const std::vector<QuerySpec>& specs, bool enabled,
+                      GroupPlan& p, uint32_t* fcap_out, double params[3]) {
+  p.route.assign(p.n, Route::kBlock);
+  if (!p.score_mode) return false;
+  uint32_t fcap = 64;
+  bool have_params = false;
+  double pk1 = 0, pb = 0, pavg = 0;
+  BlockMaxMemo memo;
+  for (uint32_t i = 0; enabled && i < p.n; ++i) {
+    const QuerySpec& s = specs[qids[i]];
+    if (!s.flat || !s.fast_score_ok || s.score.empty() || s.score.size() > static_cast<size_t>(kFastMaxScore)) continue;
+    if (p.dq[i].cap > 128) continue;
+    if (have_params && (BitsOf(s.k1) != BitsOf(pk1) || BitsOf(s.b) != BitsOf(pb) || BitsOf(s.avgdl) != BitsOf(pavg))) continue;
+    DevFastQuery f{};
+    if (!ResolveFast(v, s, p.dq[i], &f, &memo)) continue;
+    if (!have_params) {
+      pk1 = s.k1;
+      pb = s.b;
+      pavg = s.avgdl;
+      have_params = true;
+    }
+    if (p.fastq.empty()) p.fastq.resize(p.n);
+    p.fastq[i] = f;
+    p.route[i] = Route::kFast;
+    fcap = std::max(fcap, f.cap);
+  }
+  *fcap_out = fcap;
+  params[0] = pk1;
+  params[1] = pb;
+  params[2] = pavg;
+  return have_params;
+}
+
+void CutItems(const PlanView& v, const std::vector<uint32_t>& qids, const std::vector<QuerySpec>& specs, GroupPlan& p) {
+  static const double kMatchesPerUnit = std::getenv("MGX_ITEM_MATCHES") ? atof(std::getenv("MGX_ITEM_MATCHES")) : 256.0;
+  static const double kItemCost = std::getenv("MGX_ITEM_COST") ? atof(std::getenv("MGX_ITEM_COST")) : 192.0;
+  static const uint32_t kMaxTiles = std::getenv("MGX_MAX_ITEM_TILES") ? static_cast<uint32_t>(atoi(std::getenv("MGX_MAX_ITEM_TILES"))) : static_cast<uint32_t>(kMaxTilesPerItem);
+  static const uint64_t want_items = std::getenv("MGX_WANT_ITEMS") ? static_cast<uint64_t>(atoll(std::getenv("MGX_WANT_ITEMS"))) : 4ull * 768ull;
+  static const uint32_t kSeedTiles = std::getenv("MGX_SEED_TILES") ? static_cast<uint32_t>(atoi(std::getenv("MGX_SEED_TILES"))) : 16u;
+  const uint32_t n = p.n, n_tiles = v.n_tiles;
+  p.list_begin.assign(n + 1, 0);
+  p.item_begin.assign(n + 1, 0);
+  uint32_t n_lists = 0;
+  for (uint32_t i = 0; i < n; ++i) {
+    const QuerySpec& s = specs[qids[i]];
+    const Route route = p.route[i];
+    p.item_begin[i] = static_cast<uint32_t>(p.items.size());
+    const bool fast = route == Route::kFast;
+    const double per_tile = 1.0 + (p.score_mode || p.df_mode ? s.est_density * kTileDocs / (fast ? kMatchesPerUnit / 2 : kMatchesPerUnit) : 0.0);
+    const double fast_scale = std::min(4.0, std::max(2.0, static_cast<double>(n_tiles) / 150.0));
+    uint32_t tiles = static_cast<uint32_t>((fast ? fast_scale * kItemCost : kItemCost) / per_tile);
+    tiles = std::max<uint32_t>(8, std::min<uint32_t>(tiles, fast ? 2 * kMaxTiles : kMaxTiles)) & ~7u;
+    if (p.score_mode) {
+      const uint64_t cap = std::max<uint64_t>(8, (static_cast<uint64_t>(n_tiles) * n / want_items + 7) & ~7ull);
+      tiles = static_cast<uint32_t>(std::min<uint64_t>(tiles, cap));
+    }
+    if (p.score_mode && route == Route::kBlock) tiles = 8;
+    p.list_begin[i] = n_lists;
+    if (route == Route::kCand) {
+      p.items.push_back(DevItem{i, p.cand_driver[i], 0, n_lists++});
+      continue;
+    }
+    uint32_t t0 = 0;
+    const uint32_t seed_tiles = std::min<uint32_t>(kSeedTiles, (n_tiles / 8) & ~7u);
+    if (fast && seed_tiles && n_tiles > 4 * seed_tiles) {
+      p.items.push_back(DevItem{i, 0, seed_tiles, n_lists++});
+      t0 = seed_tiles;
+    }
+    for (uint32_t t = t0; t < n_tiles; t += tiles) {
+      DevItem it{i, t, std::min(tiles, n_tiles - t), n_lists++};
+      p.items.push_back(it);
+    }
+  }
+  p.list_begin[n] = n_lists;
+  p.item_begin[n] = static_cast<uint32_t>(p.items.size());
+}
+
+void ScheduleItems(const PlanView& v, const std::vector<uint32_t>& qids, const std::vector<QuerySpec>& specs, GroupPlan& p,
+                   uint32_t n_seed_fast[kFastMaxScore], uint32_t* seed_k, uint64_t* seed_table_docs) {
+  static const uint32_t kSortTiles = std::getenv("MGX_SORT_TILES") ? static_cast<uint32_t>(atoi(std::getenv("MGX_SORT_TILES"))) : 16u;
+  static const bool kXcdAffinity = std::getenv("MGX_XCD_AFFINITY") ? atoi(std::getenv("MGX_XCD_AFFINITY")) != 0 : true;
+  static const double kHeavyDensity = std::getenv("MGX_HEAVY_DENSITY") ? atof(std::getenv("MGX_HEAVY_DENSITY")) : 0.05;
+  static const double kSqueezeEnv = std::getenv("MGX_HEAVY_SQUEEZE") ? atof(std::getenv("MGX_HEAVY_SQUEEZE")) : -1.0;
+  const uint32_t n = p.n, n_tiles = v.n_tiles;
+  const bool deal = kXcdAffinity && p.score_mode;
+  std::vector<uint32_t>& order = p.order;
+  order.resize(n);
+  if (deal) {
+    p.keys.resize(n);
+    for (uint32_t i = 0; i < n; ++i) {
+      uint64_t best = 0;
+      uint32_t heavy = 0;
+      for (const DevLeaf& lf : specs[qids[i]].leaves) {
+        if (lf.kind != kLeafGramBitmap && lf.kind != kLeafList) continue;
+        const uint64_t sz = v.offsets[lf.a + 1] - v.offsets[lf.a];
+        if (sz > best) {
+          best = sz;
+          heavy = lf.a;
+        }
+      }
+      p.keys[i] = static_cast<uint64_t>(heavy) << 32 | i;
+    }
+    std::sort(p.keys.begin(), p.keys.end());
+    for (uint32_t i = 0; i < n; ++i) order[i] = static_cast<uint32_t>(p.keys[i]);
+  } else {
+    for (uint32_t i = 0; i < n; ++i) order[i] = i;
+  }
+  const uint32_t n_bands = n_tiles / kSortTiles + 1;
+  const double kHeavySqueeze = kSqueezeEnv >= 0.0 ? kSqueezeEnv : 0.6 + 0.4 * std::min(1.0, n_tiles / 600.0);
+  p.band_rule.resize(n);
+  p.dest.resize(n);
+  p.seed_ok.resize(n);
+  for (uint32_t i = 0; i < n; ++i) {
+    const Route route = p.route[i];
+    p.band_rule[i] = route == Route::kCand ? 2
+                     : p.score_mode && route == Route::kFast && specs[qids[i]].est_density >= kHeavyDensity ? 1 : 0;
+    p.dest[i] = route == Route::kBlock ? 0 : route == Route::kWave ? 1 : route == Route::kWaveLists ? 2
+                : route == Route::kCand ? 3 : route == Route::kMerge ? 4
+                : static_cast<uint8_t>(5 + p.fastq[i].n_score - 1);
+    p.seed_ok[i] = route == Route::kFast && p.list_begin[i + 1] - p.list_begin[i] > 1 ? (p.fastq[i].blockmax != 0 ? 2 : 1) : 0;
+  }
+  const size_t n_items = p.items.size();
+  p.band.resize(n_items);
+  std::vector<uint32_t>& band_at = p.band_at;
+  band_at.assign(n_bands + 1, 0);
+  for (size_t k = 0; k < n_items; ++k) {
+    const DevItem& it = p.items[k];
+    const uint8_t rule = p.band_rule[it.query];
+    uint32_t band = rule == 2 ? 0u : it.tile_begin / kSortTiles;
+    if (rule == 1) band = static_cast<uint32_t>(band * kHeavySqueeze);
+    p.band[k] = band;
+    band_at[band + 1]++;
+  }
+  for (uint32_t k = 0; k < n_bands; ++k) band_at[k + 1] += band_at[k];
+  std::vector<DevItem>& sorted = p.sorted;
+  sorted.resize(n_items);
+  {
+    p.cur.assign(band_at.begin(), band_at.end() - 1);
+    for (uint32_t oi = 0; oi < n; ++oi) {
+      const uint32_t i = order[oi];
+      for (uint32_t k = p.item_begin[i]; k < p.item_begin[i + 1]; ++k) sorted[p.cur[p.band[k]]++] = p.items[k];
+    }
+  }
+  if (deal) {
+    for (uint32_t k = 0; k < n_bands; ++k) {
+      const size_t lo = band_at[k], m = band_at[k + 1] - lo, per = (m + 7) / 8;
+      size_t w = lo;
+      for (size_t r = 0; r < per; ++r)
+        for (size_t x = 0; x < 8; ++x)
+          if (x * per + r < m) p.items[w++] = sorted[lo + x * per + r];
+    }
+  } else {
+    p.items.swap(sorted);
+  }
+  p.has_seed.assign(n, 0);
+  std::vector<DevItem>* const dest[5 + kFastMaxScore] = {&p.block, &p.wave, &p.wave_lists, &p.cand, &p.merge,
+                                                         &p.fast[0], &p.fast[1], &p.fast[2], &p.fast[3], &p.fast[4]};
+  auto is_seed = [&](const DevItem& it) {
+    return it.tile_begin == 0 && it.n_tiles <= 16 && p.seed_ok[it.query] != 0 && it.list == p.list_begin[it.query];
+  };
+  for (const DevItem& it : p.items) {
+    if (!is_seed(it)) continue;
+    dest[p.dest[it.query]]->push_back(it);
+    if (p.seed_ok[it.query] == 2) p.has_seed[it.query] = 1;
+  }
+  for (int t = 0; t < kFastMaxScore; ++t) n_seed_fast[t] = static_cast<uint32_t>(p.fast[t].size());
+  for (const DevItem& it : p.items)
+    if (!is_seed(it)) dest[p.dest[it.query]]->push_back(it);
+  *seed_k = 0;
+  *seed_table_docs = 0;
+  for (uint32_t i = 0; p.score_mode && i < n; ++i) {
+    const QuerySpec& sp = specs[qids[i]];
+    if (sp.reverse != 0 && p.dq[i].needed != 0 && p.dq[i].needed <= 128u) {
+      *seed_k = std::max(*seed_k, p.dq[i].needed);
+      *seed_table_docs = std::max<uint64_t>(*seed_table_docs, sp.total_docs);
+    }
+  }
+}
+
+}
diff --git a/mygram-db_amd/csrc/mgx_plan.hpp b/mygram-db_amd/csrc/mgx_plan.hpp
--- /dev/null
+++ b/mygram-db_amd/csrc/mgx_plan.hpp
@@ -0,0 +1,84 @@
+#pragma once
+
+#include <cstdint>
+#include <vector>
+
+#include "mgx_compile.hpp"
+#include "mgx_internal.hpp"
+
+namespace mgx {
+
+using BlockMaxFn = const uint8_t* (*)(void* user, double k1, double b, double avgdl, double* step, const uint8_t** fine);
+
+struct PlanView {
+  const uint64_t* offsets = nullptr;
+  const uint32_t* fine_map = nullptr;
+  uint32_t n_tiles = 0;
+  uint64_t gram_bitmaps = 0, gb_row_stride = 0, gb_tile_stride = 0;
+  uint64_t fb_row_stride = 0, fb_tile_stride = 0;
+  uint64_t tfnib = 0, nib_row_stride = 0;
+  uint64_t cond_arena = 0;
+  uint32_t n_bitmap_rows = 0, n_fine_rows = 0;
+  BlockMaxFn block_max = nullptr;
+  void* block_max_user = nullptr;
+};
+
+enum class Route : uint8_t {
+  kBlock,
+  kWave,
+  kWaveLists,
+  kFast,
+  kCand,
+  kMerge,
+};
+
+struct GroupPlan {
+  void Begin(uint32_t n_, uint32_t mode);
+  uint32_t n = 0;
+  bool score_mode = false, df_mode = false, page_mode = false;
+  std::vector<DevQuery> dq;
+  std::vector<DevLeaf> leaves;
+  std::vector<uint32_t> prog;
+  std::vector<DevScoreTerm> score;
+  std::vector<uint32_t> expl;
+  uint32_t max_limit = 1, max_needed = 1;
+  std::vector<Route> route;
+  std::vector<DevFastQuery> fastq;
+  std::vector<uint64_t> wave_tables;
+  std::vector<uint32_t> cand_driver;
+  std::vector<DevItem> items;
+  std::vector<uint32_t> list_begin, item_begin;
+  std::vector<DevItem> block, wave, wave_lists, fast[kFastMaxScore], cand, merge;
+  std::vector<uint8_t> has_seed;
+  std::vector<uint32_t> order, band_at, cur, band;
+  std::vector<uint64_t> keys;
+  std::vector<uint8_t> band_rule, dest, seed_ok;
+  std::vector<DevItem> sorted;
+};
+
+struct QueryMaxima {
+  uint32_t leaves = 0, lds_leaves = 0, score = 0, stack = 0, instr = 0, cap = 64;
+};
+
+int LayOutQueries(const std::vector<uint32_t>& qids, const std::vector<QuerySpec>& specs, GroupPlan& p, QueryMaxima* m,
+                  uint64_t* list_bytes);
+
+struct BlockMaxMemo {
+  bool valid = false;
+  uint64_t k1 = 0, b = 0, avgdl = 0;
+  const uint8_t* coarse = nullptr;
+  const uint8_t* fine = nullptr;
+  double step = 0.0;
+};
+
+bool ResolveFast(const PlanView& v, const QuerySpec& s, const DevQuery& q, DevFastQuery* out, BlockMaxMemo* memo = nullptr);
+
+bool ChooseFastRoutes(const PlanView& v, const std::vector<uint32_t>& qids, const std::vector<QuerySpec>& specs, bool enabled,
+                      GroupPlan& p, uint32_t* fcap, double params[3]);
+
+void CutItems(const PlanView& v, const std::vector<uint32_t>& qids, const std::vector<QuerySpec>& specs, GroupPlan& p);
+
+void ScheduleItems(const PlanView& v, const std::vector<uint32_t>& qids, const std::vector<QuerySpec>& specs, GroupPlan& p,
+                   uint32_t n_seed_fast[kFastMaxScore], uint32_t* seed_k, uint64_t* seed_table_docs);
+
+}
diff --git a/mygram-db_amd/csrc/shim/mygram_shim.cpp b/mygram-db_amd/csrc/shim/mygram_shim.cpp
--- a/mygram-db_amd/csrc/shim/mygram_shim.cpp
+++ b/mygram-db_amd/csrc/shim/mygram_shim.cpp
@@ -2683,6 +2683,8 @@
   struct Slot {
     mgx_batch* batch = nullptr;
     std::vector<BatchQuery> queries;
+    BatchExecutor::FlatTerms flat;
+    bool from_flat = false;
     std::vector<PlannedQuery> plans;
     std::vector<mgx_query> mq;
     std::shared_ptr<index::Index::Impl::Handles> handles;
@@ -2849,6 +2851,26 @@
     enqueuing = false;
   }
 
+  static void QueryFromFlat(const BatchExecutor::FlatTerms& f, size_t i, BatchQuery* out) {
+    BatchQuery& q = *out;
+    const uint32_t t0 = i ? f.query_end[i - 1] : 0, t1 = f.query_end[i];
+    q.terms.resize(t1 - t0);
+    for (uint32_t t = t0; t < t1; ++t) {
+      const uint32_t b0 = t ? f.term_end[t - 1] : 0;
+      q.terms[t - t0].assign(f.bytes.data() + b0, f.term_end[t] - b0);
+    }
+    q.ast.reset();
+    q.not_terms.clear();
+    q.filters.clear();
+    q.fuzzy_max_distance = 0;
+    q.verify_text = false;
+    q.bm25 = index::BM25Params{};
+    q.sort_by_score = f.sort_by_score;
+    q.order = f.descending ? query::SortOrder::DESC : query::SortOrder::ASC;
+    q.limit = f.limit;
+    q.offset = f.offset;
+  }
+
   void Work() {
     std::unique_lock<std::mutex> lock(mu);
     for (;;) {
@@ -2858,6 +2880,7 @@
       chunks.pop_front();
       lock.unlock();
       for (size_t i = c.begin; i < c.end; ++i) {
+        if (c.slot->from_flat) QueryFromFlat(c.slot->flat, i, &c.slot->queries[i]);
         c.slot->plans[i].Reset();
         PlanQuery(index, c.slot->queries[i], c.slot->total_docs, c.slot->avgdl, &c.slot->plans[i]);
         if (c.slot->delta) {
@@ -2944,7 +2967,11 @@
   }
 }
 
-Expected<uint64_t, Error> BatchExecutor::Submit(std::vector<BatchQuery>&& queries) {
+Expected<uint64_t, Error> BatchExecutor::Submit(std::vector<BatchQuery>&& queries) { return SubmitAny(&queries, nullptr); }
+
+Expected<uint64_t, Error> BatchExecutor::Submit(FlatTerms&& terms) { return SubmitAny(nullptr, &terms); }
+
+Expected<uint64_t, Error> BatchExecutor::SubmitAny(std::vector<BatchQuery>* queries_in, FlatTerms* flat) {
   index::Index::Impl* im = impl_->index.impl();
   if (!im->dev) return MakeUnexpected(MakeError(ErrorCode::kInternalError, im->last_error));
   index::MutationStep step;
@@ -2973,7 +3000,7 @@
     impl_->total_docs = impl_->index.Bm25DocCount();
     impl_->avgdl = impl_->index.Bm25AvgDocLength();
   }
-  if (impl_->opt.comm && AnyHighlight(queries))
+  if (impl_->opt.comm && queries_in && AnyHighlight(*queries_in))
     return MakeUnexpected(MakeError(ErrorCode::kNotImplemented,
                                     "highlight on a sharded table (Options::comm) is not implemented: the page's texts "
                                     "live on other ranks"));
@@ -2990,7 +3017,13 @@
                                       "BatchExecutor: every slot holds an unfetched batch (Wait for one first)"));
     slot->state = Impl::kFilling;
   }
-  slot->queries.swap(queries);
+  slot->from_flat = flat != nullptr;
+  if (flat) {
+    std::swap(slot->flat, *flat);
+    slot->queries.resize(slot->flat.query_end.size());
+  } else {
+    slot->queries.swap(*queries_in);
+  }
   slot->plans.resize(slot->queries.size());
   slot->total_docs = impl_->total_docs;
   slot->avgdl = impl_->avgdl;
diff --git a/mygram-db_amd/csrc/shim/mygram_shim.hpp b/mygram-db_amd/csrc/shim/mygram_shim.hpp
--- a/mygram-db_amd/csrc/shim/mygram_shim.hpp
+++ b/mygram-db_amd/csrc/shim/mygram_shim.hpp
@@ -338,12 +338,20 @@
   BatchExecutor& operator=(const BatchExecutor&) = delete;
   mygram::utils::Expected<uint64_t, mygram::utils::Error> Submit(const std::vector<BatchQuery>& queries);
   mygram::utils::Expected<uint64_t, mygram::utils::Error> Submit(std::vector<BatchQuery>&& queries);
+  struct FlatTerms {
+    std::vector<char> bytes;
+    std::vector<uint32_t> term_end, query_end;
+    uint32_t limit = 0, offset = 0;
+    bool sort_by_score = false, descending = true;
+  };
+  mygram::utils::Expected<uint64_t, mygram::utils::Error> Submit(FlatTerms&& terms);
   mygram::utils::Expected<std::vector<BatchResult>, mygram::utils::Error> Wait(uint64_t ticket, Timing* timing = nullptr);
   mygram::utils::Error Warm(const std::vector<BatchQuery>& sample, int rounds = 2);
   mygram::utils::Error WaitInto(uint64_t ticket, std::vector<BatchResult>* results, Timing* timing = nullptr);
 
  private:
   struct Impl;
+  mygram::utils::Expected<uint64_t, mygram::utils::Error> SubmitAny(std::vector<BatchQuery>* queries, FlatTerms* flat);
   std::unique_ptr<Impl> impl_;
 };
 
diff --git a/mygram-db_amd/csrc/shim/shim_capi.cpp b/mygram-db_amd/csrc/shim/shim_capi.cpp
--- a/mygram-db_amd/csrc/shim/shim_capi.cpp
+++ b/mygram-db_amd/csrc/shim/shim_capi.cpp
@@ -20,7 +20,7 @@
 };
 struct mgxs_executor {
   std::unique_ptr<BatchExecutor> ex;
-  std::vector<BatchQuery> queries;
+  BatchExecutor::FlatTerms flat;
   std::vector<mygramdb::search_pipeline::BatchResult> results;
   std::mutex limits_mu;
   std::unordered_map<uint64_t, uint32_t> limits;
@@ -192,8 +192,24 @@
   if (!ex || !ticket || (n_queries && (!n_terms || !terms)))
     return Fail(MGX_ERR_INVALID_ARGUMENT, "mgxs_submit: null argument");
   try {
-    FillQueries(&ex->queries, n_queries, n_terms, terms, limit, offset, sort_by_score, descending);
-    auto r = ex->ex->Submit(std::move(ex->queries));
+    BatchExecutor::FlatTerms& f = ex->flat;
+    f.bytes.clear();
+    f.term_end.clear();
+    f.query_end.clear();
+    size_t at = 0;
+    for (uint32_t i = 0; i < n_queries; ++i) {
+      for (uint32_t t = 0; t < n_terms[i]; ++t) {
+        const char* term = terms[at++];
+        f.bytes.insert(f.bytes.end(), term, term + std::strlen(term));
+        f.term_end.push_back(static_cast<uint32_t>(f.bytes.size()));
+      }
+      f.query_end.push_back(static_cast<uint32_t>(f.term_end.size()));
+    }
+    f.limit = limit;
+    f.offset = offset;
+    f.sort_by_score = sort_by_score != 0;
+    f.descending = descending != 0;
+    auto r = ex->ex->Submit(std::move(f));
     if (!r) return Fail(static_cast<int>(r.error().code()), r.error().message());
     *ticket = *r;
     {
```

After: 1.042 million. 0.98x the previous value.
